# rasd3/TODA

Hardware: NVIDIA B200
Metric: frames/s voxelize+VoxelResBackBone8x fwd+bwd (higher is better)
Workload: dtype bf16

## Files before the change

include/toda_b200.h:

```cpp
#ifndef TODA_B200_H
#define TODA_B200_H

#include <stddef.h>
#include <stdint.h>

#ifdef __cplusplus
extern "C" {
#endif

#define TODA_OK 0
#define TODA_ERR_INVALID (-1)
#define TODA_ERR_CUDA (-2)
#define TODA_ERR_WORKSPACE (-3)
#define TODA_ERR_UNSUPPORTED (-4)

#define TODA_ORDER_FIRST_APPEARANCE 0
#define TODA_ORDER_CANONICAL 1

const char *toda_last_error(void);
int toda_version(void);
long long toda_launch_count(void);
int toda_device_info(int *sm_count_host, int *cc_major_host, int *cc_minor_host);

size_t toda_index_bytes(int batch, int D, int H, int W);
int toda_index_insert(void *index, int batch, int D, int H, int W, const int32_t *coords, int n, void *stream);
int toda_index_insert_strided(void *index_out, int batch, int oD, int oH, int oW, const int32_t *in_coords, int n_in,
                              const int *ksize_host, const int *stride_host, const int *pad_host, void *stream);
int toda_index_build(void *index, int batch, int D, int H, int W, int32_t *out_coords, int cap, int32_t *n_out,
                     void *stream);
int toda_index_rows(const void *index, int batch, int D, int H, int W, const int32_t *coords, int n, int32_t *rows,
                    void *stream);
int toda_index_release(void *index, int batch, int D, int H, int W, const int32_t *coords, int n, void *stream);

#define TODA_SELECT_RANGE_XY 0
#define TODA_SELECT_RECT_XY 1
#define TODA_SELECT_SECTOR 2
#define TODA_SELECT_BOXES 3
size_t toda_points_select_workspace_bytes(int n);
int toda_points_select(const float *points, int n, int stride, int x_col, const int32_t *frame_offsets, int batch, int mode,
                       const double *params_host, int invert, int add_batch_col, float *out, int32_t *out_offsets,
                       void *workspace, size_t workspace_bytes, void *stream);

size_t toda_voxelize_workspace_bytes(int64_t n_points, int batch, const int *grid_host, int max_points,
                                     int max_voxels);
int toda_voxelize_hard(const float *points, int64_t n_points, int point_stride, int xyz_col, int feat_col,
                       int num_features, const int32_t *frame_offsets, int batch, const float *range_host,
                       const float *vsize_host, const int *grid_host, int max_points, int max_voxels, int order,
                       float *voxels, int32_t *coords, int32_t *num_points, int32_t *voxel_counts, void *workspace,
                       size_t workspace_bytes, void *stream);

int toda_mean_vfe_fwd(const float *voxels, const void *num_points, int num_is_float, int n_voxels, int max_points,
                      int num_features, float *voxel_features, void *stream);
int toda_mean_vfe_bwd(const float *d_voxel_features, const void *num_points, int num_is_float, int n_voxels,
                      int max_points, int num_features, float *d_voxels, void *stream);

int toda_rulebook_subm(const void *index, int batch, int D, int H, int W, const int32_t *coords, int n,
                       const int *ksize_host, int32_t *nbr, void *stream);
int toda_rulebook_sparse(const void *index_in, int iD, int iH, int iW, const void *index_out, int oD, int oH, int oW,
                         int batch, const int32_t *in_coords, int n_in, const int32_t *out_coords, int n_out,
                         const int *ksize_host, const int *stride_host, const int *pad_host, int32_t *nbr_fwd,
                         int32_t *nbr_bwd, void *stream);

size_t toda_parity_order_workspace_bytes(int n);
int toda_parity_order(const int32_t *coords, int n, const int *stride_host, const int *pad_host, int32_t *order,
                      int32_t *pos_of_row, void *workspace, size_t workspace_bytes, void *stream);

#define TODA_CONV_FP32 0
#define TODA_CONV_BF16 1
#define TODA_CONV_BF16X3 2
int toda_weight_repack(const float *w_param, int kvol, int cin, int cout, int transpose, int mirror_k, float *w_out,
                       void *stream);
size_t toda_spconv_fwd_workspace_bytes(int n_in, int cin, int cout, int kvol, int precision);
int toda_table_tile_masks(const int32_t *nbr, int n_out, int kvol, uint32_t *masks, void *stream);
int toda_spconv_uses_tensor_cores(int cin, int cout, int kvol, int precision);
int toda_spconv_wgrad_uses_tensor_cores(int cin, int cout, int kvol, int precision);
int toda_spconv_fwd(const float *x, const void *x_bf16, int n_in, int cin, const int32_t *nbr, int n_out, int kvol,
                    const float *w, int cout, const float *bias, float *y, const int32_t *out_rows,
                    const uint32_t *tile_masks, double *bn_sums, int precision, void *workspace, size_t workspace_bytes,
                    void *stream);
int toda_tile_plan_capacity(int channels);
int toda_table_tile_plan(const int32_t *nbr, int n_out, int kvol, int ngroups, int cap, uint16_t *lidx, int32_t *rows,
                         int32_t *cnt, void *stream);
int toda_spconv_fwd_plan(const float *x, const void *x_bf16, int n_in, int cin, const int32_t *nbr, int n_out, int kvol,
                         const float *w, int cout, const float *bias, const float *addend, float *y,
                         const int32_t *out_rows, const uint32_t *tile_masks, const uint16_t *plan_lidx,
                         const int32_t *plan_rows, const int32_t *plan_cnt, int plan_groups, int plan_cap, double *bn_sums,
                         const void *w_bf16, int precision, void *workspace, size_t workspace_bytes, void *stream);
int toda_weight_kmajor_bf16(const float *w, int kvol, int cin, int cout, void *w_bf16, void *stream);
size_t toda_spconv_wgrad_workspace_bytes(int n_in, int n_out, int kvol, int cin, int cout, int precision);
int toda_spconv_wgrad(const float *x, const void *x_bf16, int n_in, int cin, const int32_t *nbr, int n_out, int kvol,
                      const float *dy, const void *dy_bf16, int cout, float *dw_param, void *workspace,
                      size_t workspace_bytes, int precision, void *stream);

size_t toda_bn_workspace_bytes(int channels);
int toda_bn_stats(const float *y, int n, int channels, const float *gamma, const float *beta, float eps,
                  float momentum, float *running_mean, float *running_var, float *scale, float *shift,
                  float *save_mean, float *save_rstd, void *workspace, size_t workspace_bytes, void *stream);
int toda_bn_finalize_sums(const double *sums, int n, int channels, const float *gamma, const float *beta, float eps,
                          float momentum, float *running_mean, float *running_var, float *scale, float *shift,
                          float *save_mean, float *save_rstd, void *stream);
int toda_bn_eval_coeffs(const float *gamma, const float *beta, const float *running_mean, const float *running_var,
                        float eps, int channels, float *scale, float *shift, void *stream);
int toda_bn_apply(const float *y, int n, int channels, const float *scale, const float *shift, const float *residual,
                  int relu, float *a, void *a_bf16, void *stream);
int toda_bn_apply_sums(const float *y, int n, int channels, const double *sums, const float *gamma, const float *beta,
                       float eps, float momentum, float *running_mean, float *running_var, float *scale, float *shift,
                       float *save_mean, float *save_rstd, const float *residual, int relu, float *a, void *a_bf16,
                       void *stream);
int toda_bn_bwd(const float *da, const float *a, const float *y, int n, int channels, const float *gamma,
                const float *save_mean, const float *save_rstd, int relu, int training, float *dy, void *dy_bf16,
                float *dresidual, float *dgamma, float *dbeta, void *workspace, size_t workspace_bytes, void *stream);
int toda_col_sum(const float *dy, int n, int channels, float *out, void *workspace, size_t workspace_bytes,
                 void *stream);

typedef struct {
    const float *x; const void *x_bf16; int n_in, cin; const int32_t *nbr; int n_out, kvol;
    const float *w; const void *w_bf16 ; int cout; const float *bias ;
    const uint32_t *tile_masks ;
    const uint16_t *plan_lidx ; const int32_t *plan_rows; const int32_t *plan_cnt; int plan_groups, plan_cap;
    int precision; void *conv_ws; size_t conv_ws_bytes;
    const float *gamma; const float *beta; float eps, momentum; float *running_mean; float *running_var; int training;
    const float *residual ; int relu;
    float *y; double *sums; float *stats; float *a; void *a_bf16 ;
    void *bn_ws; size_t bn_ws_bytes;
} toda_layer_fwd_args;
typedef struct {
    const float *da; const float *a_mask; const float *y; int n_out, cout; const float *gamma; const float *mean; const float *rstd;
    int relu, training; float *dy; void *dy_bf16 ; float *dres ; float *dgamma; float *dbeta;
    void *bn_ws; size_t bn_ws_bytes;
    const float *x; const void *x_bf16 ; int n_in, cin, kvol;
    int need_dx; const int32_t *dgrad_nbr; const float *wt; const void *wt_bf16 ;
    const int32_t *dgrad_out_rows ; const uint32_t *dgrad_masks ;
    const uint16_t *dplan_lidx ; const int32_t *dplan_rows; const int32_t *dplan_cnt; int dplan_groups, dplan_cap;
    const float *addend ; float *dx;
    int need_dw; const int32_t *nbr_fwd; float *dw; void *wgrad_ws; size_t wgrad_ws_bytes;
    int need_db; float *db;
    int precision; void *conv_ws; size_t conv_ws_bytes;
} toda_layer_bwd_args;
int toda_layer_fwd(const toda_layer_fwd_args *args, void *stream);
int toda_layer_bwd(const toda_layer_bwd_args *args, void *stream);

int toda_bev_scatter_fwd(const float *features, const int32_t *coords, int n, int channels, int batch, int D, int H,
                         int W, float *out, void *stream);
int toda_bev_scatter_bwd(const float *d_out, const int32_t *coords, int n, int channels, int batch, int D, int H,
                         int W, float *d_features, void *stream);

int toda_gather_rows(const float *in, const int32_t *rows, int n, int channels, float *out, void *stream);

#ifdef __cplusplus
}
#endif
#endif
```

toda_b200/_C.py:

```python
import ctypes
import os

_HERE = os.path.dirname(os.path.abspath(__file__))
LIB_PATH = os.path.join(_HERE, "lib", "libtoda_b200.so")

c_int, c_i64, c_f32, c_vp, c_sz = ctypes.c_int, ctypes.c_int64, ctypes.c_float, ctypes.c_void_p, ctypes.c_size_t
_IP = ctypes.POINTER(ctypes.c_int)
_FP = ctypes.POINTER(ctypes.c_float)

SIGNATURES = {
    "toda_last_error": (ctypes.c_char_p, []),
    "toda_version": (c_int, []),
    "toda_launch_count": (ctypes.c_longlong, []),
    "toda_device_info": (c_int, [_IP, _IP, _IP]),
    "toda_index_bytes": (c_sz, [c_int] * 4),
    "toda_index_insert": (c_int, [c_vp, c_int, c_int, c_int, c_int, c_vp, c_int, c_vp]),
    "toda_index_insert_strided": (c_int, [c_vp, c_int, c_int, c_int, c_int, c_vp, c_int, _IP, _IP, _IP, c_vp]),
    "toda_index_build": (c_int, [c_vp, c_int, c_int, c_int, c_int, c_vp, c_int, c_vp, c_vp]),
    "toda_index_rows": (c_int, [c_vp, c_int, c_int, c_int, c_int, c_vp, c_int, c_vp, c_vp]),
    "toda_index_release": (c_int, [c_vp, c_int, c_int, c_int, c_int, c_vp, c_int, c_vp]),
    "toda_points_select_workspace_bytes": (c_sz, [c_int]),
    "toda_points_select": (c_int, [c_vp, c_int, c_int, c_int, c_vp, c_int, c_int, ctypes.POINTER(ctypes.c_double), c_int, c_int,
                                   c_vp, c_vp, c_vp, c_sz, c_vp]),
    "toda_voxelize_workspace_bytes": (c_sz, [c_i64, c_int, _IP, c_int, c_int]),
    "toda_voxelize_hard": (c_int, [c_vp, c_i64, c_int, c_int, c_int, c_int, c_vp, c_int, _FP, _FP, _IP, c_int, c_int,
                                   c_int, c_vp, c_vp, c_vp, c_vp, c_vp, c_sz, c_vp]),
    "toda_mean_vfe_fwd": (c_int, [c_vp, c_vp, c_int, c_int, c_int, c_int, c_vp, c_vp]),
    "toda_mean_vfe_bwd": (c_int, [c_vp, c_vp, c_int, c_int, c_int, c_int, c_vp, c_vp]),
    "toda_rulebook_subm": (c_int, [c_vp, c_int, c_int, c_int, c_int, c_vp, c_int, _IP, c_vp, c_vp]),
    "toda_rulebook_sparse": (c_int, [c_vp, c_int, c_int, c_int, c_vp, c_int, c_int, c_int, c_int, c_vp, c_int, c_vp,
                                     c_int, _IP, _IP, _IP, c_vp, c_vp, c_vp]),
    "toda_weight_repack": (c_int, [c_vp, c_int, c_int, c_int, c_int, c_int, c_vp, c_vp]),
    "toda_spconv_fwd_workspace_bytes": (c_sz, [c_int] * 5),
    "toda_spconv_uses_tensor_cores": (c_int, [c_int] * 4),
    "toda_spconv_wgrad_uses_tensor_cores": (c_int, [c_int] * 4),
    "toda_parity_order_workspace_bytes": (c_sz, [c_int]),
    "toda_parity_order": (c_int, [c_vp, c_int, _IP, _IP, c_vp, c_vp, c_vp, c_sz, c_vp]),
    "toda_table_tile_masks": (c_int, [c_vp, c_int, c_int, c_vp, c_vp]),
    "toda_spconv_fwd": (c_int, [c_vp, c_vp, c_int, c_int, c_vp, c_int, c_int, c_vp, c_int, c_vp, c_vp, c_vp, c_vp, c_vp, c_int, c_vp,
                                c_sz, c_vp]),
    "toda_tile_plan_capacity": (c_int, [c_int]),
    "toda_table_tile_plan": (c_int, [c_vp, c_int, c_int, c_int, c_int, c_vp, c_vp, c_vp, c_vp]),
    "toda_spconv_fwd_plan": (c_int, [c_vp, c_vp, c_int, c_int, c_vp, c_int, c_int, c_vp, c_int, c_vp, c_vp, c_vp, c_vp, c_vp, c_vp,
                                     c_vp, c_vp, c_int, c_int, c_vp, c_vp, c_int, c_vp, c_sz, c_vp]),
    "toda_weight_kmajor_bf16": (c_int, [c_vp, c_int, c_int, c_int, c_vp, c_vp]),
    "toda_layer_fwd": (c_int, [c_vp, c_vp]),
    "toda_layer_bwd": (c_int, [c_vp, c_vp]),
    "toda_spconv_wgrad_workspace_bytes": (c_sz, [c_int] * 6),
    "toda_spconv_wgrad": (c_int, [c_vp, c_vp, c_int, c_int, c_vp, c_int, c_int, c_vp, c_vp, c_int, c_vp, c_vp, c_sz, c_int, c_vp]),
    "toda_bn_workspace_bytes": (c_sz, [c_int]),
    "toda_bn_stats": (c_int, [c_vp, c_int, c_int, c_vp, c_vp, c_f32, c_f32, c_vp, c_vp, c_vp, c_vp, c_vp, c_vp, c_vp,
                              c_sz, c_vp]),
    "toda_bn_finalize_sums": (c_int, [c_vp, c_int, c_int, c_vp, c_vp, c_f32, c_f32, c_vp, c_vp, c_vp, c_vp, c_vp, c_vp, c_vp]),
    "toda_bn_eval_coeffs": (c_int, [c_vp, c_vp, c_vp, c_vp, c_f32, c_int, c_vp, c_vp, c_vp]),
    "toda_bn_apply": (c_int, [c_vp, c_int, c_int, c_vp, c_vp, c_vp, c_int, c_vp, c_vp, c_vp]),
    "toda_bn_apply_sums": (c_int, [c_vp, c_int, c_int, c_vp, c_vp, c_vp, c_f32, c_f32, c_vp, c_vp, c_vp, c_vp, c_vp, c_vp, c_vp,
                                   c_int, c_vp, c_vp, c_vp]),
    "toda_bn_bwd": (c_int, [c_vp, c_vp, c_vp, c_int, c_int, c_vp, c_vp, c_vp, c_int, c_int, c_vp, c_vp, c_vp, c_vp, c_vp,
                            c_vp, c_sz, c_vp]),
    "toda_col_sum": (c_int, [c_vp, c_int, c_int, c_vp, c_vp, c_sz, c_vp]),
    "toda_bev_scatter_fwd": (c_int, [c_vp, c_vp, c_int, c_int, c_int, c_int, c_int, c_int, c_vp, c_vp]),
    "toda_bev_scatter_bwd": (c_int, [c_vp, c_vp, c_int, c_int, c_int, c_int, c_int, c_int, c_vp, c_vp]),
    "toda_gather_rows": (c_int, [c_vp, c_vp, c_int, c_int, c_vp, c_vp]),
}



class LayerFwdArgs(ctypes.Structure):
    _fields_ = [("x", c_vp), ("x_bf16", c_vp), ("n_in", c_int), ("cin", c_int), ("nbr", c_vp), ("n_out", c_int), ("kvol", c_int),
                ("w", c_vp), ("w_bf16", c_vp), ("cout", c_int), ("bias", c_vp), ("tile_masks", c_vp),
                ("plan_lidx", c_vp), ("plan_rows", c_vp), ("plan_cnt", c_vp), ("plan_groups", c_int), ("plan_cap", c_int),
                ("precision", c_int), ("conv_ws", c_vp), ("conv_ws_bytes", c_sz),
                ("gamma", c_vp), ("beta", c_vp), ("eps", c_f32), ("momentum", c_f32), ("running_mean", c_vp), ("running_var", c_vp),
                ("training", c_int), ("residual", c_vp), ("relu", c_int),
                ("y", c_vp), ("sums", c_vp), ("stats", c_vp), ("a", c_vp), ("a_bf16", c_vp), ("bn_ws", c_vp), ("bn_ws_bytes", c_sz)]


class LayerBwdArgs(ctypes.Structure):
    _fields_ = [("da", c_vp), ("a_mask", c_vp), ("y", c_vp), ("n_out", c_int), ("cout", c_int), ("gamma", c_vp), ("mean", c_vp),
                ("rstd", c_vp), ("relu", c_int), ("training", c_int), ("dy", c_vp), ("dy_bf16", c_vp), ("dres", c_vp), ("dgamma", c_vp),
                ("dbeta", c_vp), ("bn_ws", c_vp), ("bn_ws_bytes", c_sz),
                ("x", c_vp), ("x_bf16", c_vp), ("n_in", c_int), ("cin", c_int), ("kvol", c_int),
                ("need_dx", c_int), ("dgrad_nbr", c_vp), ("wt", c_vp), ("wt_bf16", c_vp), ("dgrad_out_rows", c_vp), ("dgrad_masks", c_vp),
                ("dplan_lidx", c_vp), ("dplan_rows", c_vp), ("dplan_cnt", c_vp), ("dplan_groups", c_int), ("dplan_cap", c_int),
                ("addend", c_vp), ("dx", c_vp),
                ("need_dw", c_int), ("nbr_fwd", c_vp), ("dw", c_vp), ("wgrad_ws", c_vp), ("wgrad_ws_bytes", c_sz),
                ("need_db", c_int), ("db", c_vp),
                ("precision", c_int), ("conv_ws", c_vp), ("conv_ws_bytes", c_sz)]


_lib = None


def lib():
    global _lib
    if _lib is None:
        if not os.path.exists(LIB_PATH):
            raise RuntimeError(
                f"{LIB_PATH} is missing: build it with `python -c 'import __graft_entry__ as g; g.build()'` "
                "(nvcc, sm_100a).  toda_b200 has no CPU fallback.")
        L = ctypes.CDLL(LIB_PATH)
        for name, (res, args) in SIGNATURES.items():
            fn = getattr(L, name)
            fn.restype = res
            fn.argtypes = args
        _lib = L
    return _lib


def check(rc, what=""):
    if rc != 0:
        msg = lib().toda_last_error().decode("utf-8", "replace")
        raise RuntimeError(f"libtoda_b200 {what} failed (code {rc}): {msg}")


def ints(vals):
    return (ctypes.c_int * len(vals))(*[int(v) for v in vals])


def doubles(vals):
    return (ctypes.c_double * len(vals))(*[float(v) for v in vals])


def floats(vals):
    return (ctypes.c_float * len(vals))(*[float(v) for v in vals])
```

toda_b200/csrc/conv_simt.cu:

```cuda
#include "common.cuh"
#include "conv_ts.cuh"

int conv_tc_fwd(const float *x, const void *x_bf16, int n_in, int cin, const int32_t *nbr, int n_out, int kvol, const float *w,
                int cout, const float *bias, float *y, const int32_t *out_rows, const uint32_t *tile_masks, double *bn_sums,
                void *workspace, size_t workspace_bytes,
                cudaStream_t st, const TilePlan *plan, const float *addend, const void *w_bf16);
size_t conv_tc_fwd_workspace_bytes(int n_in, int cin, int cout, int kvol);
int conv_tc_wgrad(const float *x, const void *x_bf16, int n_in, int cin, const int32_t *nbr, int n_out, int kvol,
                  const float *dy, const void *dy_bf16, int cout, float *dw_param, void *workspace, size_t workspace_bytes,
                  cudaStream_t st);
bool conv_tc_supported(int cin, int cout, int kvol);
size_t conv_x3_fwd_workspace_bytes(int n_in, int cin, int cout, int kvol);
int conv_x3_fwd(const float *x, int n_in, int cin, const int32_t *nbr, int n_out, int kvol, const float *w, int cout, const float *bias,
                float *y, const int32_t *out_rows, const uint32_t *tile_masks, double *bn_sums, void *workspace, size_t workspace_bytes,
                cudaStream_t st, const TilePlan *plan, const float *addend);
size_t conv_x3_wgrad_workspace_bytes(int n_in, int n_out, int kvol, int cin, int cout);
int conv_x3_wgrad(const float *x, int n_in, int cin, const int32_t *nbr, int n_out, int kvol, const float *dy, int cout, float *dw_param,
                  void *workspace, size_t workspace_bytes, cudaStream_t st);
bool conv_tc_wgrad_supported(int cin, int cout, int kvol);
size_t conv_tc_wgrad_workspace_bytes(int n_in, int n_out, int kvol, int cin, int cout);

namespace {

constexpr int kThreads = 256;
constexpr int BK = 16;

template <int BM, int BN>
__global__ void __launch_bounds__(kThreads) conv_fwd_f32_kernel(const float *__restrict__ x, int cin,
                                                                const int *__restrict__ nbr, int n_out, int kvol,
                                                                const float *__restrict__ w, int cout,
                                                                const float *__restrict__ bias, float *__restrict__ y,
                                                                const int *__restrict__ out_rows ,
                                                                const float *__restrict__ addend ) {
    static_assert((BM / 4) * (BN / 4) == kThreads, "4x4 micro-tiles must cover the CTA tile");
    __shared__ __align__(16) float As[BK][BM + 4];
    __shared__ __align__(16) float Bs[BK][BN + 4];
    __shared__ int rows[BM];
    const int tid = threadIdx.x;
    const int tx = tid % (BN / 4), ty = tid / (BN / 4);
    const int row0 = blockIdx.x * BM, col0 = blockIdx.y * BN;
    const bool vec = (cin % 4) == 0;
    float acc[4][4];
#pragma unroll
    for (int i = 0; i < 4; ++i)
#pragma unroll
        for (int j = 0; j < 4; ++j) acc[i][j] = 0.f;

    for (int k = 0; k < kvol; ++k) {
        int any = 0;
        for (int m = tid; m < BM; m += kThreads) {
            int r = row0 + m;
            int src = (r < n_out) ? __ldg(nbr + (size_t)k * n_out + r) : -1;
            rows[m] = src;
            any |= (src >= 0);
        }
        any = __syncthreads_or(any);
        if (!any) continue;
        for (int c0 = 0; c0 < cin; c0 += BK) {
            if (vec) {
                for (int e = tid; e < BM * (BK / 4); e += kThreads) {
                    int m = e / (BK / 4), q = e % (BK / 4);
                    int src = rows[m];
                    float4 v = make_float4(0.f, 0.f, 0.f, 0.f);
                    if (src >= 0 && c0 + q * 4 < cin) v = __ldg((const float4 *)(x + (size_t)src * cin + c0 + q * 4));
                    As[q * 4 + 0][m] = v.x; As[q * 4 + 1][m] = v.y; As[q * 4 + 2][m] = v.z; As[q * 4 + 3][m] = v.w;
                }
            } else {
                for (int e = tid; e < BM * BK; e += kThreads) {
                    int m = e / BK, kk = e % BK;
                    int src = rows[m];
                    As[kk][m] = (src >= 0 && c0 + kk < cin) ? __ldg(x + (size_t)src * cin + c0 + kk) : 0.f;
                }
            }
            for (int e = tid; e < BK * BN; e += kThreads) {
                int kk = e / BN, nn = e % BN;
                Bs[kk][nn] = (c0 + kk < cin && col0 + nn < cout) ? __ldg(w + ((size_t)k * cin + c0 + kk) * cout + col0 + nn) : 0.f;
            }
            __syncthreads();
#pragma unroll
            for (int kk = 0; kk < BK; ++kk) {
                float4 a = *(const float4 *)&As[kk][ty * 4];
                float4 b = *(const float4 *)&Bs[kk][tx * 4];
                float av[4] = {a.x, a.y, a.z, a.w}, bv[4] = {b.x, b.y, b.z, b.w};
#pragma unroll
                for (int i = 0; i < 4; ++i)
#pragma unroll
                    for (int j = 0; j < 4; ++j) acc[i][j] = fmaf(av[i], bv[j], acc[i][j]);
            }
            __syncthreads();
        }
    }
#pragma unroll
    for (int i = 0; i < 4; ++i) {
        int r = row0 + ty * 4 + i;
        if (r >= n_out) continue;
        const int orow = out_rows ? __ldg(out_rows + r) : r;
#pragma unroll
        for (int j = 0; j < 4; ++j) {
            int c = col0 + tx * 4 + j;
            if (c < cout) y[(size_t)orow * cout + c] = acc[i][j] + (bias ? __ldg(bias + c) : 0.f) + (addend ? __ldg(addend + (size_t)orow * cout + c) : 0.f);
        }
    }
}

constexpr int WT = 64;
__global__ void __launch_bounds__(kThreads) conv_wgrad_f32_kernel(const float *__restrict__ x, int cin,
                                                                  const int *__restrict__ nbr, int n_out, int kvol,
                                                                  const float *__restrict__ dy, int cout, int rows_per_split,
                                                                  float *__restrict__ partial) {
    __shared__ __align__(16) float As[BK][WT + 4];
    __shared__ __align__(16) float Bs[BK][WT + 4];
    __shared__ int pin[kThreads], pout[kThreads];
    __shared__ int warp_cnt[kThreads / 32];
    const int tid = threadIdx.x, lane = tid & 31, warp = tid >> 5;
    const int tx = tid % (WT / 4), ty = tid / (WT / 4);
    const int ci_tiles = (cin + WT - 1) / WT, co_tiles = (cout + WT - 1) / WT;
    int bx = blockIdx.x;
    const int co_t = bx % co_tiles; bx /= co_tiles;
    const int ci_t = bx % ci_tiles; bx /= ci_tiles;
    const int k = bx;
    const int split = blockIdx.y;
    const int ci0 = ci_t * WT, co0 = co_t * WT;
    const int r_begin = split * rows_per_split;
    const int r_end = min(n_out, r_begin + rows_per_split);
    float acc[4][4];
#pragma unroll
    for (int i = 0; i < 4; ++i)
#pragma unroll
        for (int j = 0; j < 4; ++j) acc[i][j] = 0.f;

    for (int r0 = r_begin; r0 < r_end; r0 += kThreads) {
        int r = r0 + tid;
        int src = (r < r_end) ? __ldg(nbr + (size_t)k * n_out + r) : -1;
        unsigned bal = __ballot_sync(0xffffffffu, src >= 0);
        if (lane == 0) warp_cnt[warp] = __popc(bal);
        __syncthreads();
        int woff = 0, total = 0;
#pragma unroll
        for (int wi = 0; wi < kThreads / 32; ++wi) {
            int c = warp_cnt[wi];
            if (wi < warp) woff += c;
            total += c;
        }
        if (src >= 0) {
            int pos = woff + __popc(bal & ((1u << lane) - 1u));
            pin[pos] = src;
            pout[pos] = r;
        }
        __syncthreads();
        for (int g0 = 0; g0 < total; g0 += BK) {
            for (int e = tid; e < BK * WT; e += kThreads) {
                int kk = e / WT, c = e % WT;
                bool ok = g0 + kk < total;
                As[kk][c] = (ok && ci0 + c < cin) ? __ldg(x + (size_t)pin[ok ? g0 + kk : 0] * cin + ci0 + c) : 0.f;
                Bs[kk][c] = (ok && co0 + c < cout) ? __ldg(dy + (size_t)pout[ok ? g0 + kk : 0] * cout + co0 + c) : 0.f;
            }
            __syncthreads();
#pragma unroll
            for (int kk = 0; kk < BK; ++kk) {
                float4 a = *(const float4 *)&As[kk][ty * 4];
                float4 b = *(const float4 *)&Bs[kk][tx * 4];
                float av[4] = {a.x, a.y, a.z, a.w}, bv[4] = {b.x, b.y, b.z, b.w};
#pragma unroll
                for (int i = 0; i < 4; ++i)
#pragma unroll
                    for (int j = 0; j < 4; ++j) acc[i][j] = fmaf(av[i], bv[j], acc[i][j]);
            }
            __syncthreads();
        }
    }
    float *dst = partial + ((size_t)split * kvol + k) * cin * cout;
#pragma unroll
    for (int i = 0; i < 4; ++i) {
        int ci = ci0 + ty * 4 + i;
        if (ci >= cin) continue;
#pragma unroll
        for (int j = 0; j < 4; ++j) {
            int co = co0 + tx * 4 + j;
            if (co < cout) dst[(size_t)ci * cout + co] = acc[i][j];
        }
    }
}

__global__ void wgrad_reduce_kernel(const float *__restrict__ partial, int splits, int kvol, int cin, int cout,
                                    float *__restrict__ dw_param) {
    size_t per = (size_t)kvol * cin * cout;
    const int sub = threadIdx.x & 7;
    for (size_t e = (blockIdx.x * (size_t)blockDim.x + threadIdx.x) >> 3; e < ((per + 31) & ~(size_t)31);
         e += ((size_t)gridDim.x * blockDim.x) >> 3) {
        float s = 0.f;
        if (e < per) {
            int ci = (int)(e % cin);
            size_t t = e / cin;
            int k = (int)(t % kvol);
            int co = (int)(t / kvol);
            size_t src = ((size_t)k * cin + ci) * cout + co;
            for (int sp = sub; sp < splits; sp += 8) s += partial[sp * per + src];
        }
        s += __shfl_xor_sync(0xffffffffu, s, 1);
        s += __shfl_xor_sync(0xffffffffu, s, 2);
        s += __shfl_xor_sync(0xffffffffu, s, 4);
        if (e < per && sub == 0) dw_param[e] = s;
    }
}

__global__ void weight_repack_kernel(const float *__restrict__ w_param, int kvol, int cin, int cout, int transpose,
                                     int mirror, float *__restrict__ w_out) {
    size_t per = (size_t)kvol * cin * cout;
    for (size_t e = blockIdx.x * (size_t)blockDim.x + threadIdx.x; e < per; e += (size_t)gridDim.x * blockDim.x) {
        int inner = (int)(e % (transpose ? cin : cout));
        size_t t = e / (transpose ? cin : cout);
        int mid = (int)(t % (transpose ? cout : cin));
        int k = (int)(t / (transpose ? cout : cin));
        int ci = transpose ? inner : mid, co = transpose ? mid : inner;
        int ks = mirror ? kvol - 1 - k : k;
        w_out[e] = __ldg(w_param + ((size_t)co * kvol + ks) * cin + ci);
    }
}

__global__ void gather_rows_kernel(const float *__restrict__ in, const int *__restrict__ rows, long long total, int c,
                                   float *__restrict__ out) {
    for (long long e = blockIdx.x * (long long)blockDim.x + threadIdx.x; e < total; e += (long long)gridDim.x * blockDim.x) {
        long long i = e / c;
        int r = __ldg(rows + i);
        out[e] = r >= 0 ? __ldg(in + (long long)r * c + (e - i * c)) : 0.f;
    }
}

int wgrad_splits(int n_out, int kvol, int cin, int cout) {
    int tiles = kvol * ((cin + WT - 1) / WT) * ((cout + WT - 1) / WT);
    int want = (4 * kNumSMs + tiles - 1) / tiles;
    int max_by_rows = (n_out + 4 * kThreads - 1) / (4 * kThreads);
    int s = want < max_by_rows ? want : max_by_rows;
    return s < 1 ? 1 : s;
}

}

extern "C" int toda_weight_repack(const float *w_param, int kvol, int cin, int cout, int transpose, int mirror_k,
                                  float *w_out, void *stream) {
    TODA_CHECK_ARG(w_param && w_out && kvol > 0 && cin > 0 && cout > 0, "weight_repack: bad args");
    size_t per = (size_t)kvol * cin * cout;
    weight_repack_kernel<<<wave_grid(per, 256), 256, 0, (cudaStream_t)stream>>>(w_param, kvol, cin, cout, transpose,
                                                                              mirror_k, w_out);
    TODA_LAUNCH_OK();
    return TODA_OK;
}

extern "C" int toda_spconv_uses_tensor_cores(int cin, int cout, int kvol, int precision) {
    return (precision == TODA_CONV_BF16 || precision == TODA_CONV_BF16X3) && conv_tc_supported(cin, cout, kvol) ? 1 : 0;
}

extern "C" int toda_spconv_wgrad_uses_tensor_cores(int cin, int cout, int kvol, int precision) {
    return (precision == TODA_CONV_BF16 || precision == TODA_CONV_BF16X3) && conv_tc_wgrad_supported(cin, cout, kvol) ? 1 : 0;
}

extern "C" size_t toda_spconv_fwd_workspace_bytes(int n_in, int cin, int cout, int kvol, int precision) {
    if (precision == TODA_CONV_BF16 && n_in >= 0 && cin > 0 && cout > 0 && kvol > 0 && conv_tc_supported(cin, cout, kvol))
        return conv_tc_fwd_workspace_bytes(n_in, cin, cout, kvol);
    if (precision == TODA_CONV_BF16X3 && n_in >= 0 && cin > 0 && cout > 0 && kvol > 0 && conv_tc_supported(cin, cout, kvol))
        return conv_x3_fwd_workspace_bytes(n_in, cin, cout, kvol);
    return 0;
}

static int spconv_fwd_impl(const float *x, const void *x_bf16, int n_in, int cin, const int32_t *nbr, int n_out, int kvol,
                           const float *w, int cout, const float *bias, float *y, const int32_t *out_rows,
                           const uint32_t *tile_masks, double *bn_sums, int precision, void *workspace, size_t workspace_bytes,
                           void *stream, const TilePlan *plan, const float *addend, const void *w_bf16);

extern "C" int toda_spconv_fwd(const float *x, const void *x_bf16, int n_in, int cin, const int32_t *nbr, int n_out, int kvol,
                               const float *w, int cout, const float *bias, float *y, const int32_t *out_rows,
                               const uint32_t *tile_masks, double *bn_sums, int precision,
                               void *workspace, size_t workspace_bytes, void *stream) {
    return spconv_fwd_impl(x, x_bf16, n_in, cin, nbr, n_out, kvol, w, cout, bias, y, out_rows, tile_masks, bn_sums, precision, workspace,
                           workspace_bytes, stream, nullptr, nullptr, nullptr);
}

extern "C" int toda_spconv_fwd_plan(const float *x, const void *x_bf16, int n_in, int cin, const int32_t *nbr, int n_out, int kvol,
                                    const float *w, int cout, const float *bias, const float *addend, float *y,
                                    const int32_t *out_rows, const uint32_t *tile_masks, const uint16_t *plan_lidx,
                                    const int32_t *plan_rows, const int32_t *plan_cnt, int plan_groups, int plan_cap, double *bn_sums,
                                    const void *w_bf16, int precision, void *workspace, size_t workspace_bytes, void *stream) {
    TilePlan plan{plan_lidx, plan_rows, plan_cnt, plan_groups, plan_cap};
    return spconv_fwd_impl(x, x_bf16, n_in, cin, nbr, n_out, kvol, w, cout, bias, y, out_rows, tile_masks, bn_sums, precision, workspace,
                           workspace_bytes, stream, plan_lidx ? &plan : nullptr, addend, w_bf16);
}

static int spconv_fwd_impl(const float *x, const void *x_bf16, int n_in, int cin, const int32_t *nbr, int n_out, int kvol,
                           const float *w, int cout, const float *bias, float *y, const int32_t *out_rows,
                           const uint32_t *tile_masks, double *bn_sums, int precision, void *workspace, size_t workspace_bytes,
                           void *stream, const TilePlan *plan, const float *addend, const void *w_bf16) {
    TODA_CHECK_ARG(n_in >= 0 && n_out >= 0 && cin > 0 && cout > 0 && kvol > 0, "spconv_fwd: bad sizes");
    if (n_out == 0) return TODA_OK;
    TODA_CHECK_ARG(x && nbr && w && y, "spconv_fwd: null pointer");
    cudaStream_t st = (cudaStream_t)stream;
    TODA_CHECK_ARG(precision == TODA_CONV_FP32 || precision == TODA_CONV_BF16 || precision == TODA_CONV_BF16X3,
                   "spconv_fwd: unknown precision %d", precision);
    if (precision == TODA_CONV_BF16X3 && conv_tc_supported(cin, cout, kvol))
        return conv_x3_fwd(x, n_in, cin, nbr, n_out, kvol, w, cout, bias, y, out_rows, tile_masks, bn_sums, workspace, workspace_bytes, st,
                           plan, addend);
    if (precision == TODA_CONV_BF16 && conv_tc_supported(cin, cout, kvol))
        return conv_tc_fwd(x, x_bf16, n_in, cin, nbr, n_out, kvol, w, cout, bias, y, out_rows, tile_masks, bn_sums, workspace,
                           workspace_bytes, st, plan, addend, w_bf16);
    TODA_CHECK_ARG(!bn_sums, "spconv_fwd: fused BatchNorm statistics need the tensor-core kernel for this shape");
    if (cout <= 16) {
        dim3 grid(ceil_div(n_out, 256), ceil_div(cout, 16));
        conv_fwd_f32_kernel<256, 16><<<grid, kThreads, 0, st>>>(x, cin, nbr, n_out, kvol, w, cout, bias, y, out_rows, addend);
    } else if (cout <= 32) {
        dim3 grid(ceil_div(n_out, 128), ceil_div(cout, 32));
        conv_fwd_f32_kernel<128, 32><<<grid, kThreads, 0, st>>>(x, cin, nbr, n_out, kvol, w, cout, bias, y, out_rows, addend);
    } else {
        dim3 grid(ceil_div(n_out, 64), ceil_div(cout, 64));
        conv_fwd_f32_kernel<64, 64><<<grid, kThreads, 0, st>>>(x, cin, nbr, n_out, kvol, w, cout, bias, y, out_rows, addend);
    }
    TODA_LAUNCH_OK();
    return TODA_OK;
}

extern "C" size_t toda_spconv_wgrad_workspace_bytes(int n_in, int n_out, int kvol, int cin, int cout, int precision) {
    if (n_in < 0 || n_out < 0 || kvol <= 0 || cin <= 0 || cout <= 0) return 0;
    if (precision == TODA_CONV_BF16 && conv_tc_wgrad_supported(cin, cout, kvol))
        return conv_tc_wgrad_workspace_bytes(n_in, n_out, kvol, cin, cout);
    if (precision == TODA_CONV_BF16X3 && conv_tc_wgrad_supported(cin, cout, kvol))
        return conv_x3_wgrad_workspace_bytes(n_in, n_out, kvol, cin, cout);
    int splits = wgrad_splits(n_out, kvol, cin, cout);
    return align_up((size_t)splits * kvol * cin * cout * sizeof(float), 256);
}

extern "C" int toda_spconv_wgrad(const float *x, const void *x_bf16, int n_in, int cin, const int32_t *nbr, int n_out,
                                 int kvol, const float *dy, const void *dy_bf16, int cout, float *dw_param, void *workspace,
                                 size_t workspace_bytes, int precision, void *stream) {
    TODA_CHECK_ARG(n_in >= 0 && n_out >= 0 && cin > 0 && cout > 0 && kvol > 0, "spconv_wgrad: bad sizes");
    TODA_CHECK_ARG(dw_param, "spconv_wgrad: null dw");
    cudaStream_t st = (cudaStream_t)stream;
    if (n_out == 0) {
        TODA_CUDA_OK(cudaMemsetAsync(dw_param, 0, (size_t)kvol * cin * cout * sizeof(float), st));
        return TODA_OK;
    }
    TODA_CHECK_ARG(x && nbr && dy && workspace, "spconv_wgrad: null pointer");
    TODA_CHECK_ARG(precision == TODA_CONV_FP32 || precision == TODA_CONV_BF16 || precision == TODA_CONV_BF16X3,
                   "spconv_wgrad: unknown precision %d", precision);
    if (precision == TODA_CONV_BF16X3 && conv_tc_wgrad_supported(cin, cout, kvol))
        return conv_x3_wgrad(x, n_in, cin, nbr, n_out, kvol, dy, cout, dw_param, workspace, workspace_bytes, st);
    if (precision == TODA_CONV_BF16 && conv_tc_wgrad_supported(cin, cout, kvol))
        return conv_tc_wgrad(x, x_bf16, n_in, cin, nbr, n_out, kvol, dy, dy_bf16, cout, dw_param, workspace, workspace_bytes, st);
    int splits = wgrad_splits(n_out, kvol, cin, cout);
    size_t need = (size_t)splits * kvol * cin * cout * sizeof(float);
    if (workspace_bytes < need) {
        toda_set_error("spconv_wgrad: workspace %zu < required %zu bytes", workspace_bytes, need);
        return TODA_ERR_WORKSPACE;
    }
    int rows_per_split = ceil_div(n_out, splits);
    rows_per_split = ceil_div(rows_per_split, kThreads) * kThreads;
    int tiles = kvol * ((cin + WT - 1) / WT) * ((cout + WT - 1) / WT);
    dim3 grid(tiles, splits);
    conv_wgrad_f32_kernel<<<grid, kThreads, 0, st>>>(x, cin, nbr, n_out, kvol, dy, cout, rows_per_split, (float *)workspace);
    TODA_LAUNCH_OK();
    size_t per = (size_t)kvol * cin * cout;
    wgrad_reduce_kernel<<<wave_grid(per * 8, 256), 256, 0, st>>>((const float *)workspace, splits, kvol, cin, cout, dw_param);
    TODA_LAUNCH_OK();
    return TODA_OK;
}

extern "C" int toda_gather_rows(const float *in, const int32_t *rows, int n, int channels, float *out, void *stream) {
    TODA_CHECK_ARG(n >= 0 && channels > 0, "gather_rows: bad sizes");
    if (n == 0) return TODA_OK;
    TODA_CHECK_ARG(in && rows && out, "gather_rows: null pointer");
    long long total = (long long)n * channels;
    gather_rows_kernel<<<wave_grid(total, 256), 256, 0, (cudaStream_t)stream>>>(in, rows, total, channels, out);
    TODA_LAUNCH_OK();
    return TODA_OK;
}
```

toda_b200/csrc/conv_tc.cu:

```cuda
#include <cuda.h>
#include <cuda_bf16.h>
#include <stdlib.h>

#include "common.cuh"
#include "conv_ts.cuh"
#include "epilogue.cuh"
#include "table_slice.cuh"

namespace {

constexpr int kTileM = 128;
constexpr int kChunkK = 64;
constexpr int kStages = 3;
constexpr int kProducers = 128;
constexpr int kThreadsTC = kProducers + 32;
constexpr int kABytes = kTileM * kChunkK * 2;
constexpr int kBBytesMax = 128 * kChunkK * 2;
constexpr int kStageBytes = kABytes + kBBytesMax;
constexpr int kMaxKvol = 27;
constexpr int kIdxBytes = kMaxKvol * kTileM * 4;

__device__ __forceinline__ uint32_t smem_u32(const void *p) { return (uint32_t)__cvta_generic_to_shared(p); }

__device__ __forceinline__ void mbar_init(uint32_t bar, uint32_t count) {
    asm volatile("mbarrier.init.shared::cta.b64 [%0], %1;" ::"r"(bar), "r"(count) : "memory");
}
__device__ __forceinline__ void mbar_wait(uint32_t bar, uint32_t parity) {
    uint32_t done = 0;
    uint32_t spins = 0;
    while (!done) {
        asm volatile(
            "{\n\t.reg .pred p;\n\t"
            "mbarrier.try_wait.parity.shared::cta.b64 p, [%1], %2;\n\t"
            "selp.u32 %0, 1, 0, p;\n\t}"
            : "=r"(done)
            : "r"(bar), "r"(parity)
            : "memory");
        if (!done && ++spins > (1u << 24)) __trap();
    }
}
__device__ __forceinline__ uint32_t mbar_test(uint32_t bar, uint32_t parity) {
    uint32_t done;
    asm volatile(
        "{\n\t.reg .pred p;\n\t"
        "mbarrier.test_wait.parity.shared::cta.b64 p, [%1], %2;\n\t"
        "selp.u32 %0, 1, 0, p;\n\t}"
        : "=r"(done)
        : "r"(bar), "r"(parity)
        : "memory");
    return done;
}
__device__ __forceinline__ bool elect_one() {
    uint32_t pred;
    asm volatile(
        "{\n\t.reg .pred p;\n\t"
        "elect.sync _|p, 0xffffffff;\n\t"
        "selp.u32 %0, 1, 0, p;\n\t}"
        : "=r"(pred));
    return pred != 0;
}
__device__ __forceinline__ void cp_async_16(uint32_t dst, const void *src, uint32_t src_bytes) {
    asm volatile("cp.async.cg.shared.global [%0], [%1], 16, %2;" ::"r"(dst), "l"(src), "r"(src_bytes) : "memory");
}
__device__ __forceinline__ void mbar_arrive_expect_tx(uint32_t bar, uint32_t bytes) {
    asm volatile("mbarrier.arrive.expect_tx.shared::cta.b64 _, [%0], %1;" ::"r"(bar), "r"(bytes) : "memory");
}
__device__ __forceinline__ void tma_load_2d(uint32_t dst, const CUtensorMap *map, int c0, int c1, uint32_t bar) {
    asm volatile(
        "cp.async.bulk.tensor.2d.shared::cluster.global.mbarrier::complete_tx::bytes [%0], [%1, {%2, %3}], [%4];"
        ::"r"(dst), "l"(map), "r"(c0), "r"(c1), "r"(bar)
        : "memory");
}
__device__ __forceinline__ void st_shared_zero16(uint32_t dst) {
    asm volatile("st.shared.v4.b32 [%0], {%1, %1, %1, %1};" ::"r"(dst), "r"(0u) : "memory");
}
__device__ __forceinline__ void cp_async_arrive_noinc(uint32_t bar) {
    asm volatile("cp.async.mbarrier.arrive.noinc.shared::cta.b64 [%0];" ::"r"(bar) : "memory");
}
__device__ __forceinline__ void umma_commit(uint32_t bar) {
    asm volatile("tcgen05.commit.cta_group::1.mbarrier::arrive::one.shared::cluster.b64 [%0];" ::"r"(bar) : "memory");
}
__device__ __forceinline__ void umma_bf16(uint32_t tmem_d, uint64_t adesc, uint64_t bdesc, uint32_t idesc, uint32_t accumulate) {
    asm volatile(
        "{\n\t.reg .pred p;\n\t"
        "setp.ne.b32 p, %4, 0;\n\t"
        "tcgen05.mma.cta_group::1.kind::f16 [%0], %1, %2, %3, p;\n\t}"
        ::"r"(tmem_d), "l"(adesc), "l"(bdesc), "r"(idesc), "r"(accumulate)
        : "memory");
}

__device__ __forceinline__ uint64_t make_desc_k_sw128(uint32_t smem_addr) {
    uint64_t d = 0;
    d |= (uint64_t)((smem_addr >> 4) & 0x3fff);
    d |= (uint64_t)1 << 16;
    d |= (uint64_t)(1024 >> 4) << 32;
    d |= (uint64_t)1 << 46;
    d |= (uint64_t)2 << 61;
    return d;
}

__host__ __device__ constexpr uint32_t make_idesc_bf16(int m, int n) {
    return (1u << 4) | (1u << 7) | (1u << 10) | ((uint32_t)(n >> 3) << 17) | ((uint32_t)(m >> 4) << 24);
}

__device__ __forceinline__ uint32_t sw128_offset(int r, int p) { return (uint32_t)(r * 128 + ((p ^ (r & 7)) << 4)); }

constexpr int kProdThreads = 256;
constexpr int kFwdThreads = kProdThreads + 32 + 128 + 32;
constexpr int kFwdSmemBudget = 200 * 1024;
template <int COUT, int KB> struct FwdCfg {
    static constexpr int kABlock = kTileM * kChunkK * 2;
    static constexpr int kBBlock = COUT * kChunkK * 2;
    static constexpr int kATile = KB * kABlock, kBTile = KB * kBBlock;
    static constexpr int kStage = kATile + kBTile;
    static constexpr int kStagesRaw = (kFwdSmemBudget - 2 * kIdxBytes) / kStage;
    static constexpr int kStages = kStagesRaw > 8 ? 8 : kStagesRaw;
    static constexpr int kSmem = kStages * kStage + 1024 + 256 + 2 * kIdxBytes;
    static constexpr int kTmemCols = 2 * COUT < 32 ? 32 : 2 * COUT;
    static_assert(kStages >= 3, "need at least 3 stages");
};

__device__ __forceinline__ void mbar_arrive(uint32_t bar) {
    asm volatile("mbarrier.arrive.shared::cta.b64 _, [%0];" ::"r"(bar) : "memory");
}
__device__ __forceinline__ void cp_async_4(uint32_t dst, const void *src) {
    asm volatile("cp.async.ca.shared.global [%0], [%1], 4;" ::"r"(dst), "l"(src) : "memory");
}

template <int CIN, int COUT, int KB>
__global__ void __launch_bounds__(kFwdThreads, 1) conv_tc_fwd_kernel(const __nv_bfloat16 *__restrict__ xb,
                                                                     const int *__restrict__ nbr, int n_out, int kvol,
                                                                     const __grid_constant__ CUtensorMap map_w ,
                                                                     const float *__restrict__ bias, const float *__restrict__ addend ,
                                                                     float *__restrict__ y,
                                                                     const int *__restrict__ out_rows ,
                                                                     const uint32_t *__restrict__ tile_masks ,
                                                                     double *__restrict__ bn_sums, int num_tiles,
                                                                     long long *__restrict__ dbg) {
    static_assert(COUT % 16 == 0 && COUT >= 16 && COUT <= 128, "UMMA N");
    static_assert(CIN == 16 || CIN == 32 || CIN == 64 || CIN == 128, "row = 32..256 bytes of bf16");
    using C = FwdCfg<COUT, KB>;
    constexpr int S = C::kStages;
    constexpr int kChunkElems = KB * kChunkK;
    extern __shared__ uint8_t smem_raw[];
    const uint32_t raw = smem_u32(smem_raw);
    const uint32_t base = (raw + 1023u) & ~1023u;
    const uint32_t bar_base = base + S * C::kStage;
    const uint32_t full_bar = bar_base, empty_bar = bar_base + 8 * S;
    const uint32_t acc_full = bar_base + 16 * S, acc_empty = acc_full + 16;
    const uint32_t idx_full = acc_full + 32, idx_empty = acc_full + 48;
    const uint32_t tmem_slot = acc_full + 64;
    const uint32_t idx_base = bar_base + 256;
    volatile uint32_t *tmem_slot_ptr = (volatile uint32_t *)(smem_raw + (tmem_slot - raw));

    const int tid = threadIdx.x, warp = tid >> 5, lane = tid & 31;
    const int ktot = kvol * CIN;
    const int nchunks = (ktot + kChunkElems - 1) / kChunkElems;
    auto chunk_mask_of = [&](int t) -> unsigned long long {
        if (!tile_masks) return nchunks >= 64 ? ~0ull : ((1ull << nchunks) - 1ull);
        const uint32_t om = __ldg(tile_masks + t);
        unsigned long long cm = 0ull;
        if (CIN <= kChunkElems) {
            constexpr int kOpc = CIN <= kChunkElems ? kChunkElems / CIN : 1;
            for (int c = 0; c < nchunks; ++c)
                if ((om >> (c * kOpc)) & ((1u << kOpc) - 1u)) cm |= 1ull << c;
        } else {
            constexpr int kCpo = CIN > kChunkElems ? CIN / kChunkElems : 1;
            for (int c = 0; c < nchunks; ++c)
                if ((om >> (c / kCpo)) & 1u) cm |= 1ull << c;
        }
        return cm ? cm : 1ull;
    };

    if (tid == 0) {
        for (int s = 0; s < S; ++s) {
            mbar_init(full_bar + 8 * s, kProdThreads / 32 + 1);
            mbar_init(empty_bar + 8 * s, 1);
        }
        for (int b = 0; b < 2; ++b) {
            mbar_init(acc_full + 8 * b, 1);
            mbar_init(acc_empty + 8 * b, 128);
            mbar_init(idx_full + 8 * b, 64);
            mbar_init(idx_empty + 8 * b, kProdThreads);
        }
        asm volatile("fence.mbarrier_init.release.cluster;" ::: "memory");
    }
    if (warp == 8) {
        asm volatile("tcgen05.alloc.cta_group::1.sync.aligned.shared::cta.b32 [%0], %1;" ::"r"(tmem_slot), "n"(C::kTmemCols) : "memory");
        asm volatile("tcgen05.relinquish_alloc_permit.cta_group::1.sync.aligned;" ::: "memory");
    }
    asm volatile("tcgen05.fence::before_thread_sync;" ::: "memory");
    __syncthreads();
    asm volatile("tcgen05.fence::after_thread_sync;" ::: "memory");
    const uint32_t tmem_base = *tmem_slot_ptr;

    if (warp < 8) {
        const int p = tid & 7;
        const int rbase = tid >> 3;
        const uint32_t piece_off = (uint32_t)(rbase * 128 + ((p ^ (rbase & 7)) << 4));
        constexpr int kOffsPerChunk = CIN >= 64 ? 1 : 64 / CIN;
        const int k_sub = CIN >= 64 ? 0 : p / (CIN / 8);
        const int ci_lo = CIN >= 64 ? p * 8 : (p % (CIN / 8)) * 8;
        const char *xbytes = (const char *)xb + ci_lo * 2;
        const uint32_t idx_lane = idx_base + 4 * rbase;
        constexpr int kLag = S - 2;
        int g = 0, it = 0;
        for (int t = blockIdx.x; t < num_tiles; t += gridDim.x, ++it) {
            const int ib = it & 1;
            if (dbg && blockIdx.x == 0 && tid == 0 && it < 256) dbg[0 * 256 + it] = clock64();
            mbar_wait(idx_full + 8 * ib, (it >> 1) & 1);
            if (dbg && blockIdx.x == 0 && tid == 0 && it < 256) dbg[1 * 256 + it] = clock64();
            if (dbg && blockIdx.x == 0 && tid == 0 && it < 255) dbg[7 * 256 + it] = g;
            const uint32_t idx_tile = idx_lane + ib * kIdxBytes;
            for (unsigned long long cm = chunk_mask_of(t); cm; cm &= cm - 1, ++g) {
                const int c = __ffsll((long long)cm) - 1;
                const int s = g % S, use = g / S;
                if (use > 0) mbar_wait(empty_bar + 8 * s, (use - 1) & 1);
                const uint32_t a_dst0 = base + s * C::kStage + piece_off;
#pragma unroll
                for (int kb = 0; kb < KB; ++kb) {
                    const int cb = c * KB + kb;
                    const uint32_t a_dst = a_dst0 + kb * C::kABlock;
                    const int k = CIN == 128 ? (cb >> 1) : cb * kOffsPerChunk + k_sub;
                    const bool k_ok = k < kvol;
                    const int ci_hi = CIN == 128 ? (cb & 1) * 64 : 0;
                    int src[4];
#pragma unroll
                    for (int i = 0; i < 4; ++i) {
                        src[i] = -1;
                        if (k_ok) asm volatile("ld.shared.b32 %0, [%1];" : "=r"(src[i]) : "r"(idx_tile + 4 * (k * kTileM + 32 * i)));
                    }
#pragma unroll
                    for (int i = 0; i < 4; ++i) {
                        if (src[i] >= 0) cp_async_16(a_dst + i * 4096, xbytes + ((size_t)(unsigned)src[i] * CIN + ci_hi) * 2, 16u);
                        else st_shared_zero16(a_dst + i * 4096);
                    }
                }
                if (tid == 0) {
                    const int left = ktot - c * kChunkElems;
                    const int nblk = left >= kChunkElems ? KB : (left + kChunkK - 1) / kChunkK;
                    mbar_arrive_expect_tx(full_bar + 8 * s, nblk * C::kBBlock);
                    const uint32_t b_tile = base + s * C::kStage + C::kATile;
                    for (int kb = 0; kb < nblk; ++kb)
                        tma_load_2d(b_tile + kb * C::kBBlock, &map_w, (c * KB + kb) * kChunkK, 0, full_bar + 8 * s);
                }
                asm volatile("cp.async.commit_group;" ::: "memory");
                if (g >= kLag) {
                    asm volatile("cp.async.wait_group %0;" ::"n"(kLag) : "memory");
                    asm volatile("fence.proxy.async.shared::cta;" ::: "memory");
                    __syncwarp();
                    if (lane == 0) mbar_arrive(full_bar + 8 * ((g - kLag) % S));
                }
                if (dbg && blockIdx.x == 0 && tid == 0 && g < 256) dbg[3 * 256 + g] = clock64();
            }
            mbar_arrive(idx_empty + 8 * ib);
        }
        asm volatile("cp.async.wait_group 0;" ::: "memory");
        asm volatile("fence.proxy.async.shared::cta;" ::: "memory");
        __syncwarp();
        if (lane == 0)
            for (int j = (g > kLag ? g - kLag : 0); j < g; ++j) mbar_arrive(full_bar + 8 * (j % S));
    } else if (warp == 8) {
        {
            constexpr uint32_t idesc = make_idesc_bf16(kTileM, COUT);
            int g = 0, it = 0;
            uint32_t ready = 0;
            for (int t = blockIdx.x; t < num_tiles; t += gridDim.x, ++it) {
                const int ab = it & 1, ause = it >> 1;
                if (ause > 0) mbar_wait(acc_empty + 8 * ab, (ause - 1) & 1);
                const uint32_t d_tmem = tmem_base + ab * COUT;
                uint32_t accumulate = 0;
                for (unsigned long long cm = chunk_mask_of(t); cm; cm &= cm - 1, ++g) {
                    const int c = __ffsll((long long)cm) - 1;
                    const int s = g % S, use = g / S;
                    if (dbg && blockIdx.x == 0 && lane == 0 && g < 256) dbg[4 * 256 + g] = clock64();
                    if (!ready) mbar_wait(full_bar + 8 * s, use & 1);
                    if (dbg && blockIdx.x == 0 && lane == 0 && g < 256) dbg[5 * 256 + g] = clock64();
                    const int sn = (g + 1) % S, usen = (g + 1) / S;
                    ready = mbar_test(full_bar + 8 * sn, usen & 1);
                    asm volatile("tcgen05.fence::after_thread_sync;" ::: "memory");
                    const uint32_t a_tile = base + s * C::kStage, b_tile = a_tile + C::kATile;
                    const int ksteps = min(kChunkElems, ktot - c * kChunkElems) / 16;
                    if (elect_one()) {
                        const uint64_t ad0 = make_desc_k_sw128(a_tile), bd0 = make_desc_k_sw128(b_tile);
                        umma_bf16(d_tmem, ad0, bd0, idesc, accumulate);
                        for (int j = 1; j < ksteps; ++j) {
                            const uint32_t blk = j >> 2, st = j & 3;
                            umma_bf16(d_tmem, ad0 + blk * (C::kABlock >> 4) + 2 * st, bd0 + blk * (C::kBBlock >> 4) + 2 * st, idesc, 1u);
                        }
                        umma_commit(empty_bar + 8 * s);
                    }
                    accumulate = 1u;
                    __syncwarp();
                    if (dbg && blockIdx.x == 0 && lane == 0 && g < 256) dbg[6 * 256 + g] = clock64();
                }
                if (elect_one()) umma_commit(acc_full + 8 * ab);
                __syncwarp();
            }
        }
    } else if (warp < 13) {
        const int q = warp & 3;
        float acc_s[COUT / 16], acc_q[COUT / 16];
#pragma unroll
        for (int i = 0; i < COUT / 16; ++i) acc_s[i] = acc_q[i] = 0.f;
        int it = 0;
        for (int t = blockIdx.x; t < num_tiles; t += gridDim.x, ++it) {
            const int ab = it & 1;
            mbar_wait(acc_full + 8 * ab, (it >> 1) & 1);
            asm volatile("tcgen05.fence::after_thread_sync;" ::: "memory");
            const int row = t * kTileM + q * 32 + lane;
            const int orow = (out_rows && row < n_out) ? __ldg(out_rows + row) : row;
            const uint32_t taddr = tmem_base + ((uint32_t)(q * 32) << 16) + ab * COUT;
#pragma unroll
            for (int n0 = 0; n0 < COUT; n0 += 16) {
                uint32_t v[16];
                asm volatile(
                    "tcgen05.ld.sync.aligned.32x32b.x16.b32 {%0,%1,%2,%3,%4,%5,%6,%7,%8,%9,%10,%11,%12,%13,%14,%15}, [%16];"
                    : "=r"(v[0]), "=r"(v[1]), "=r"(v[2]), "=r"(v[3]), "=r"(v[4]), "=r"(v[5]), "=r"(v[6]), "=r"(v[7]), "=r"(v[8]),
                      "=r"(v[9]), "=r"(v[10]), "=r"(v[11]), "=r"(v[12]), "=r"(v[13]), "=r"(v[14]), "=r"(v[15])
                    : "r"(taddr + n0));
                asm volatile("tcgen05.wait::ld.sync.aligned;" ::: "memory");
                float o[16];
#pragma unroll
                for (int j = 0; j < 16; ++j) o[j] = __uint_as_float(v[j]) + (bias ? __ldg(bias + n0 + j) : 0.f);
                if (row < n_out) {
                    if (addend) {
                        const float4 *ad = (const float4 *)(addend + (size_t)orow * COUT + n0);
#pragma unroll
                        for (int qq = 0; qq < 4; ++qq) {
                            const float4 a4 = __ldg(ad + qq);
                            o[4 * qq] += a4.x; o[4 * qq + 1] += a4.y; o[4 * qq + 2] += a4.z; o[4 * qq + 3] += a4.w;
                        }
                    }
                    float4 *dst = (float4 *)(y + (size_t)orow * COUT + n0);
#pragma unroll
                    for (int qq = 0; qq < 4; ++qq) dst[qq] = make_float4(o[4 * qq], o[4 * qq + 1], o[4 * qq + 2], o[4 * qq + 3]);
                }
                if (bn_sums) {
                    float sq[16];
#pragma unroll
                    for (int j = 0; j < 16; ++j) {
                        o[j] = row < n_out ? o[j] : 0.f;
                        sq[j] = o[j] * o[j];
                    }
                    acc_s[n0 / 16] += warp_colsum16(o, lane);
                    acc_q[n0 / 16] += warp_colsum16(sq, lane);
                }
            }
            asm volatile("tcgen05.fence::before_thread_sync;" ::: "memory");
            mbar_arrive(acc_empty + 8 * ab);
            if (dbg && blockIdx.x == 0 && q == 1 && lane == 0 && it < 256) dbg[2 * 256 + it] = clock64();
        }
        if (bn_sums && !(lane & 1)) {
            const int col = (lane >> 1) & 15;
#pragma unroll
            for (int i = 0; i < COUT / 16; ++i) {
                atomicAdd(bn_sums + i * 16 + col, (double)acc_s[i]);
                atomicAdd(bn_sums + COUT + i * 16 + col, (double)acc_q[i]);
            }
        }
    } else {
        int it = 0;
        for (int t = blockIdx.x; t < num_tiles; t += gridDim.x, ++it) {
            const int ib = it & 1, use = it >> 1;
            if (use > 0) mbar_wait(idx_empty + 8 * ib, (use - 1) & 1);
            const uint32_t dst0 = idx_base + ib * kIdxBytes;
            const int row0 = t * kTileM;
            load_table_slice<kTileM>(dst0, nbr, n_out, row0, n_out, kvol, lane);
            cp_async_arrive_noinc(idx_full + 8 * ib);
            mbar_arrive(idx_full + 8 * ib);
        }
    }
    __syncthreads();
    if (warp == 8) {
        asm volatile("tcgen05.fence::after_thread_sync;" ::: "memory");
        asm volatile("tcgen05.dealloc.cta_group::1.sync.aligned.b32 %0, %1;" ::"r"(tmem_base), "n"(C::kTmemCols) : "memory");
    }
}

__global__ void f32_to_bf16_kernel(const float *__restrict__ in, long long n4, __nv_bfloat16 *__restrict__ out) {
    for (long long i = blockIdx.x * (long long)blockDim.x + threadIdx.x; i < n4; i += (long long)gridDim.x * blockDim.x) {
        float4 v = __ldg((const float4 *)in + i);
        __nv_bfloat162 lo = __floats2bfloat162_rn(v.x, v.y), hi = __floats2bfloat162_rn(v.z, v.w);
        uint2 o;
        o.x = *(uint32_t *)&lo;
        o.y = *(uint32_t *)&hi;
        ((uint2 *)out)[i] = o;
    }
}

__global__ void f32_to_bf16_pad_kernel(const float *__restrict__ in, long long n, int cin, int cpad,
                                       __nv_bfloat16 *__restrict__ out) {
    long long total = n * cpad;
    for (long long e = blockIdx.x * (long long)blockDim.x + threadIdx.x; e < total; e += (long long)gridDim.x * blockDim.x) {
        long long r = e / cpad;
        int c = (int)(e - r * cpad);
        out[e] = __float2bfloat16_rn(c < cin ? __ldg(in + r * cin + c) : 0.f);
    }
}

__global__ void weight_to_kmajor_bf16_kernel(const float *__restrict__ w, int kvol, int cin, int cpad, int cout,
                                             __nv_bfloat16 *__restrict__ wb) {
    size_t per = (size_t)kvol * cpad * cout;
    for (size_t e = blockIdx.x * (size_t)blockDim.x + threadIdx.x; e < per; e += (size_t)gridDim.x * blockDim.x) {
        size_t kc = e % ((size_t)kvol * cpad);
        int co = (int)(e / ((size_t)kvol * cpad));
        int k = (int)(kc / cpad), ci = (int)(kc % cpad);
        wb[e] = __float2bfloat16_rn(ci < cin ? __ldg(w + ((size_t)k * cin + ci) * cout + co) : 0.f);
    }
}

__global__ void table_tile_masks_kernel(const int *__restrict__ nbr, int n_out, int kvol, int num_tiles, uint32_t *__restrict__ masks) {
    const int t = (blockIdx.x * blockDim.x + threadIdx.x) >> 5, lane = threadIdx.x & 31;
    if (t >= num_tiles) return;
    const int row0 = t * kTileM;
    uint32_t m = 0;
    for (int k = 0; k < kvol; ++k) {
        const int *src = nbr + (size_t)k * n_out + row0;
        int any = 0;
#pragma unroll
        for (int j = 0; j < kTileM / 32; ++j) {
            const int r = lane + 32 * j;
            if (row0 + r < n_out) any |= (__ldg(src + r) >= 0);
        }
        if (__any_sync(0xffffffffu, any)) m |= 1u << k;
    }
    if (lane == 0) masks[t] = m;
}

}

extern "C" int toda_table_tile_masks(const int32_t *nbr, int n_out, int kvol, uint32_t *masks, void *stream) {
    TODA_CHECK_ARG(n_out >= 0 && kvol > 0 && kvol <= 32, "table_tile_masks: bad sizes n_out=%d kvol=%d", n_out, kvol);
    if (n_out == 0) return TODA_OK;
    TODA_CHECK_ARG(nbr && masks, "table_tile_masks: null pointer");
    const int num_tiles = ceil_div(n_out, kTileM);
    table_tile_masks_kernel<<<ceil_div(num_tiles * 32, 256), 256, 0, (cudaStream_t)stream>>>(nbr, n_out, kvol, num_tiles, masks);
    TODA_LAUNCH_OK();
    return TODA_OK;
}

static inline int pad16(int c) { return c < 16 ? 16 : c; }

int conv_tma_fwd(const void *xb, int n_in, int cin, const int32_t *nbr, int n_out, int kvol, const void *wb, int cout,
                 const float *bias, const float *addend, float *y, const int32_t *out_rows, const uint32_t *tile_masks, double *bn_sums,
                 cudaStream_t st);

static long long *g_dbg_timeline = nullptr;
extern "C" void toda_debug_set_timeline(long long *buf) { g_dbg_timeline = buf; }
long long *conv_tc_debug_timeline() { return g_dbg_timeline; }
static int g_dbg_mode = 0;
extern "C" void toda_debug_set_mode(int m) { g_dbg_mode = m; }
int conv_tc_debug_mode() { return g_dbg_mode; }

extern "C" int toda_weight_kmajor_bf16(const float *w, int kvol, int cin, int cout, void *w_bf16, void *stream) {
    TODA_CHECK_ARG(w && w_bf16 && kvol > 0 && cin > 0 && cout > 0, "weight_kmajor_bf16: bad args");
    const int cp = cin < 16 ? 16 : cin;
    weight_to_kmajor_bf16_kernel<<<wave_grid((int64_t)kvol * cp * cout, 256), 256, 0, (cudaStream_t)stream>>>(w, kvol, cin, cp, cout,
                                                                                                            (__nv_bfloat16 *)w_bf16);
    TODA_LAUNCH_OK();
    return TODA_OK;
}

bool conv_tc_supported(int cin, int cout, int kvol) {
    bool cin_ok = (cin >= 1 && cin < 16) || cin == 16 || cin == 32 || cin == 64 || cin == 128;
    return cin_ok && kvol <= kMaxKvol && (cout == 16 || cout == 32 || cout == 64 || cout == 128);
}

size_t conv_tc_fwd_workspace_bytes(int n_in, int cin, int cout, int kvol) {
    int cp = pad16(cin);
    return align_up((size_t)n_in * cp * 2 + 16, 256) + align_up((size_t)kvol * cp * cout * 2, 256) + 256;
}

int conv_tc_fwd(const float *x, const void *x_bf16, int n_in, int cin, const int32_t *nbr, int n_out, int kvol, const float *w,
                int cout, const float *bias, float *y, const int32_t *out_rows, const uint32_t *tile_masks, double *bn_sums,
                void *workspace, size_t workspace_bytes,
                cudaStream_t st, const TilePlan *plan, const float *addend, const void *w_bf16) {
    size_t need = conv_tc_fwd_workspace_bytes(n_in, cin, cout, kvol);
    if (!workspace || workspace_bytes < need) {
        toda_set_error("spconv_fwd(bf16): workspace %zu < required %zu bytes", workspace_bytes, need);
        return TODA_ERR_WORKSPACE;
    }
    const int cp = pad16(cin);
    __nv_bfloat16 *xb = (__nv_bfloat16 *)workspace;
    __nv_bfloat16 *wb = (__nv_bfloat16 *)((char *)workspace + align_up((size_t)n_in * cp * 2 + 16, 256));
    if (cp == cin && x_bf16) {
        xb = (__nv_bfloat16 *)x_bf16;
    } else if (cp == cin) {
        long long n4 = (long long)n_in * cin / 4;
        if (n4 > 0) {
            f32_to_bf16_kernel<<<wave_grid(n4, 256), 256, 0, st>>>(x, n4, xb);
            TODA_LAUNCH_OK();
        }
    } else if (n_in > 0) {
        f32_to_bf16_pad_kernel<<<wave_grid((int64_t)n_in * cp, 256), 256, 0, st>>>(x, n_in, cin, cp, xb);
        TODA_LAUNCH_OK();
    }
    if (w_bf16) {
        wb = (__nv_bfloat16 *)w_bf16;
    } else {
        weight_to_kmajor_bf16_kernel<<<wave_grid((int64_t)kvol * cp * cout, 256), 256, 0, st>>>(w, kvol, cin, cp, cout, wb);
        TODA_LAUNCH_OK();
    }
    cin = cp;
    if (bn_sums) TODA_CUDA_OK(cudaMemsetAsync(bn_sums, 0, 2 * (size_t)cout * sizeof(double), st));
    static int feed = -1;
    if (feed < 0) { const char *e = getenv("TODA_TC_FEED"); feed = !e ? 2 : (e[0] == 'c' ? 0 : (e[0] == 't' && e[1] == 'm' ? 1 : 2)); }
    if (feed == 2 && conv_ts_supported(cin, cout, kvol, plan))
        return conv_ts_fwd(xb, n_in, cin, nbr, n_out, kvol, *plan, wb, cout, bias, addend, y, out_rows, tile_masks, bn_sums, st);
    if (feed == 1 || (feed == 2 && cin == 128 && cout == 128))
        {
        return conv_tma_fwd(xb, n_in, cin, nbr, n_out, kvol, wb, cout, bias, addend, y, out_rows, out_rows ? tile_masks : nullptr, bn_sums, st);
    }
    int num_tiles = ceil_div(n_out, kTileM);
    int grid = num_tiles < kNumSMs ? num_tiles : kNumSMs;
    CUtensorMap map_w;
    if (int rc = conv_tma_make_map(&map_w, wb, (uint64_t)cout, (uint64_t)kvol * cin, (uint32_t)cout, kChunkK)) return rc;
#define LAUNCH_TC(CI, CO)                                                                                                    \
    do {                                                                                                                     \
        constexpr int KB_ = (CO) <= 64 ? 2 : 1;                                                                              \
        constexpr int smem = FwdCfg<CO, KB_>::kSmem;                                                                         \
        static bool attr_set = false;                                                                                        \
        if (!attr_set) {                                                                                                     \
            TODA_CUDA_OK(cudaFuncSetAttribute(conv_tc_fwd_kernel<CI, CO, KB_>, cudaFuncAttributeMaxDynamicSharedMemorySize, smem)); \
            attr_set = true;                                                                                                 \
        }                                                                                                                    \
        conv_tc_fwd_kernel<CI, CO, KB_><<<grid, kFwdThreads, smem, st>>>(xb, nbr, n_out, kvol, map_w, bias, addend, y, out_rows, tile_masks, bn_sums, num_tiles, g_dbg_timeline); \
    } while (0)
#define LAUNCH_TC_CO(CI)                                                                                 \
    switch (cout) {                                                                                      \
        case 16: LAUNCH_TC(CI, 16); break;                                                               \
        case 32: LAUNCH_TC(CI, 32); break;                                                               \
        case 64: LAUNCH_TC(CI, 64); break;                                                               \
        case 128: LAUNCH_TC(CI, 128); break;                                                             \
        default: toda_set_error("conv_tc_fwd: unsupported cout %d", cout); return TODA_ERR_UNSUPPORTED;  \
    }
    switch (cin) {
        case 16: LAUNCH_TC_CO(16); break;
        case 32: LAUNCH_TC_CO(32); break;
        case 64: LAUNCH_TC_CO(64); break;
        case 128: LAUNCH_TC_CO(128); break;
        default: toda_set_error("conv_tc_fwd: unsupported cin %d", cin); return TODA_ERR_UNSUPPORTED;
    }
#undef LAUNCH_TC_CO
#undef LAUNCH_TC
    TODA_LAUNCH_OK();
    return TODA_OK;
}

namespace {

template <int NPAD, int ROWS> struct WCfg {
    static constexpr int kATile = 2 * ROWS * 128;
    static constexpr int kBTile = (NPAD / 64) * ROWS * 128;
    static constexpr int kIdx = 32 * ROWS * 4;
    static constexpr int kBBufs = ROWS == 128 ? 2 : 3;
    static constexpr int kStages = ROWS == 128 ? 4 : 8;
    static constexpr int kLag = ROWS == 128 ? 2 : 3;
    static constexpr int kSmem = kStages * kATile + kBBufs * kBTile + 2 * kIdx + 1024 + 256;
};
constexpr int kWgradThreads = kProdThreads + 32 + 128 + 32;

__device__ __forceinline__ uint64_t make_desc_mn_sw128(uint32_t smem_addr, uint32_t lbo_bytes) {
    uint64_t d = 0;
    d |= (uint64_t)((smem_addr >> 4) & 0x3fff);
    d |= (uint64_t)((lbo_bytes >> 4) & 0x3fff) << 16;
    d |= (uint64_t)(1024 >> 4) << 32;
    d |= (uint64_t)1 << 46;
    d |= (uint64_t)2 << 61;
    return d;
}

template <int CIN, int NPAD, int ROWS>
__global__ void __launch_bounds__(kWgradThreads, 1) conv_tc_wgrad_kernel(const __nv_bfloat16 *__restrict__ xb,
                                                                         const int *__restrict__ nbr, int n_out, int kvol,
                                                                         const __nv_bfloat16 *__restrict__ dyb, int cout,
                                                                         int rows_per_split, int passes_per_cta,
                                                                         float *__restrict__ partial) {
    using W = WCfg<NPAD, ROWS>;
    constexpr int kOffsPerPass = 128 / CIN;
    constexpr int S = W::kStages;
    constexpr int kRowsW = ROWS, kATileW = W::kATile, kBTileW = W::kBTile, kIdxW = W::kIdx, kBBufsW = W::kBBufs;
    constexpr int kRowIters = ROWS / 32;
    extern __shared__ uint8_t smem_raw[];
    const uint32_t raw = smem_u32(smem_raw);
    const uint32_t base = (raw + 1023u) & ~1023u;
    const uint32_t b_base = base + S * kATileW;
    const uint32_t idx_base = b_base + kBBufsW * kBTileW;
    const uint32_t bar_base = idx_base + 2 * kIdxW;
    const uint32_t a_full = bar_base, a_empty = bar_base + 8 * S;
    const uint32_t b_full = bar_base + 16 * S, b_empty = b_full + 32;
    const uint32_t idx_full = b_full + 64, idx_empty = b_full + 80;
    const uint32_t accum_bar = b_full + 96, tmem_slot = b_full + 104;
    volatile uint32_t *tmem_slot_ptr = (volatile uint32_t *)(smem_raw + (tmem_slot - raw));

    const int tid = threadIdx.x, warp = tid >> 5, lane = tid & 31;
    const int split = blockIdx.x, group = blockIdx.y;
    const int total_passes = (kvol + kOffsPerPass - 1) / kOffsPerPass;
    const int pass0 = group * passes_per_cta;
    const int npass = min(passes_per_cta, total_passes - pass0);
    const int k0 = pass0 * kOffsPerPass;
    const int noffs = min(npass * kOffsPerPass, kvol - k0);
    const int r_begin = split * rows_per_split;
    const int r_end = min(n_out, r_begin + rows_per_split);
    const int nchunks = r_end > r_begin ? (r_end - r_begin + kRowsW - 1) / kRowsW : 0;

    if (tid == 0) {
        for (int s = 0; s < S; ++s) {
            mbar_init(a_full + 8 * s, kProdThreads / 32);
            mbar_init(a_empty + 8 * s, 1);
        }
        for (int b = 0; b < kBBufsW; ++b) {
            mbar_init(b_full + 8 * b, kProdThreads / 32);
            mbar_init(b_empty + 8 * b, 1);
        }
        for (int b = 0; b < 2; ++b) {
            mbar_init(idx_full + 8 * b, 64);
            mbar_init(idx_empty + 8 * b, kProdThreads);
        }
        mbar_init(accum_bar, 1);
        asm volatile("fence.mbarrier_init.release.cluster;" ::: "memory");
    }
    uint32_t tmem_cols = 32;
    while ((int)tmem_cols < passes_per_cta * NPAD) tmem_cols <<= 1;
    if (warp == 8) {
        asm volatile("tcgen05.alloc.cta_group::1.sync.aligned.shared::cta.b32 [%0], %1;" ::"r"(tmem_slot), "r"(tmem_cols) : "memory");
        asm volatile("tcgen05.relinquish_alloc_permit.cta_group::1.sync.aligned;" ::: "memory");
    }
    asm volatile("tcgen05.fence::before_thread_sync;" ::: "memory");
    __syncthreads();
    asm volatile("tcgen05.fence::after_thread_sync;" ::: "memory");
    const uint32_t tmem_base = *tmem_slot_ptr;

    if (warp < 8) {
        const int p = tid & 7, rbase = tid >> 3;
        const uint32_t piece_off = (uint32_t)(rbase * 128 + ((p ^ (rbase & 7)) << 4));
        const int off_lo = CIN >= 64 ? 0 : p / (CIN / 8);
        const int ci_lo = CIN >= 64 ? p * 8 : (p % (CIN / 8)) * 8;
        constexpr int kLagW = W::kLag;
        int g = 0, signalled = 0;
        for (int rc = 0; rc < nchunks; ++rc) {
            const int ib = rc & 1, use_i = rc >> 1;
            const int bb = rc % kBBufsW, use_b = rc / kBBufsW;
            const int row_base = r_begin + rc * kRowsW;
            if (npass < kLagW) {
                asm volatile("cp.async.wait_group 0;" ::: "memory");
                asm volatile("fence.proxy.async.shared::cta;" ::: "memory");
                __syncwarp();
                if (lane == 0)
                    for (; signalled < g; ++signalled) {
                        if (signalled % npass == 0) mbar_arrive(b_full + 8 * ((signalled / npass) % kBBufsW));
                        mbar_arrive(a_full + 8 * (signalled % S));
                    }
                signalled = g;
            }
            if (use_b > 0) mbar_wait(b_empty + 8 * bb, (use_b - 1) & 1);
            {
                const uint32_t b_dst = b_base + bb * kBTileW + piece_off;
#pragma unroll
                for (int nb = 0; nb < NPAD / 64; ++nb) {
                    const int co = nb * 64 + p * 8;
#pragma unroll
                    for (int i = 0; i < kRowIters; ++i) {
                        const int row = row_base + rbase + 32 * i;
                        const uint32_t dst = b_dst + nb * (kRowsW * 128) + i * 4096;
                        if (row < r_end && co < cout) cp_async_16(dst, dyb + (size_t)row * cout + co, 16u);
                        else st_shared_zero16(dst);
                    }
                }
            }
            mbar_wait(idx_full + 8 * ib, use_i & 1);
            const uint32_t idx_tile = idx_base + ib * kIdxW + 4 * rbase;
            for (int ps = 0; ps < npass; ++ps, ++g) {
                const int s = g % S, use = g / S;
                if (use > 0) mbar_wait(a_empty + 8 * s, (use - 1) & 1);
                const uint32_t a_dst = base + s * kATileW + piece_off;
#pragma unroll
                for (int mb = 0; mb < 2; ++mb) {
                    const int koff = ps * kOffsPerPass + (CIN == 128 ? 0 : (CIN == 64 ? mb : mb * (kOffsPerPass / 2) + off_lo));
                    const int ci = CIN == 128 ? mb * 64 + ci_lo : ci_lo;
                    const bool k_ok = koff < noffs;
                    int src[kRowIters];
#pragma unroll
                    for (int i = 0; i < kRowIters; ++i) {
                        src[i] = -1;
                        if (k_ok) asm volatile("ld.shared.b32 %0, [%1];" : "=r"(src[i]) : "r"(idx_tile + 4 * (koff * kRowsW + 32 * i)));
                    }
#pragma unroll
                    for (int i = 0; i < kRowIters; ++i) {
                        const uint32_t dst = a_dst + mb * (kRowsW * 128) + i * 4096;
                        if (src[i] >= 0) cp_async_16(dst, xb + (size_t)(unsigned)src[i] * CIN + ci, 16u);
                        else st_shared_zero16(dst);
                    }
                }
                asm volatile("cp.async.commit_group;" ::: "memory");
                if (g - signalled >= kLagW) {
                    asm volatile("cp.async.wait_group %0;" ::"n"(kLagW) : "memory");
                    asm volatile("fence.proxy.async.shared::cta;" ::: "memory");
                    __syncwarp();
                    const int j = signalled;
                    if (lane == 0) {
                        if (j % npass == 0) mbar_arrive(b_full + 8 * ((j / npass) % kBBufsW));
                        mbar_arrive(a_full + 8 * (j % S));
                    }
                    ++signalled;
                }
            }
            mbar_arrive(idx_empty + 8 * ib);
        }
        asm volatile("cp.async.wait_group 0;" ::: "memory");
        asm volatile("fence.proxy.async.shared::cta;" ::: "memory");
        __syncwarp();
        if (lane == 0)
            for (int j = signalled; j < g; ++j) {
                if (j % npass == 0) mbar_arrive(b_full + 8 * ((j / npass) % kBBufsW));
                mbar_arrive(a_full + 8 * (j % S));
            }
    } else if (warp == 8) {
        if (nchunks > 0) {
            constexpr uint32_t idesc = make_idesc_bf16(128, NPAD) | (1u << 15) | (1u << 16);
            int g = 0;
            uint32_t ready = 0;
            for (int rc = 0; rc < nchunks; ++rc) {
                const int ib = rc % kBBufsW;
                mbar_wait(b_full + 8 * ib, (rc / kBBufsW) & 1);
                const uint32_t b_tile = b_base + ib * kBTileW;
                for (int ps = 0; ps < npass; ++ps, ++g) {
                    const int s = g % S, use = g / S;
                    if (!ready) mbar_wait(a_full + 8 * s, use & 1);
                    ready = mbar_test(a_full + 8 * ((g + 1) % S), ((g + 1) / S) & 1);
                    asm volatile("tcgen05.fence::after_thread_sync;" ::: "memory");
                    const uint32_t a_tile = base + s * kATileW;
                    if (elect_one()) {
#pragma unroll
                        const uint64_t ad0 = make_desc_mn_sw128(a_tile, kRowsW * 128), bd0 = make_desc_mn_sw128(b_tile, kRowsW * 128);
                        umma_bf16(tmem_base + ps * NPAD, ad0, bd0, idesc, rc != 0);
                        for (int j = 1; j < kRowsW / 16; ++j)
                            umma_bf16(tmem_base + ps * NPAD, ad0 + 128 * j, bd0 + 128 * j, idesc, 1u);
                        umma_commit(a_empty + 8 * s);
                    }
                    __syncwarp();
                }
                if (elect_one()) umma_commit(b_empty + 8 * ib);
                __syncwarp();
            }
            if (elect_one()) umma_commit(accum_bar);
            __syncwarp();
        }
    } else if (warp < 13) {
        const int q = warp & 3;
        if (nchunks > 0) {
            mbar_wait(accum_bar, 0);
            asm volatile("tcgen05.fence::after_thread_sync;" ::: "memory");
        }
        const int m = q * 32 + lane;
        for (int ps = 0; ps < npass; ++ps) {
            const int k = (pass0 + ps) * kOffsPerPass + m / CIN, ci = m % CIN;
            float *dst = partial + (((size_t)split * kvol + k) * CIN + ci) * cout;
            const uint32_t taddr = tmem_base + ((uint32_t)(q * 32) << 16) + ps * NPAD;
            for (int n0 = 0; n0 < cout; n0 += 16) {
                uint32_t v[16];
                if (nchunks > 0) {
                    asm volatile(
                        "tcgen05.ld.sync.aligned.32x32b.x16.b32 {%0,%1,%2,%3,%4,%5,%6,%7,%8,%9,%10,%11,%12,%13,%14,%15}, [%16];"
                        : "=r"(v[0]), "=r"(v[1]), "=r"(v[2]), "=r"(v[3]), "=r"(v[4]), "=r"(v[5]), "=r"(v[6]), "=r"(v[7]),
                          "=r"(v[8]), "=r"(v[9]), "=r"(v[10]), "=r"(v[11]), "=r"(v[12]), "=r"(v[13]), "=r"(v[14]), "=r"(v[15])
                        : "r"(taddr + n0));
                    asm volatile("tcgen05.wait::ld.sync.aligned;" ::: "memory");
                } else {
#pragma unroll
                    for (int qq = 0; qq < 16; ++qq) v[qq] = 0u;
                }
                if (k < kvol) {
#pragma unroll
                    for (int qq = 0; qq < 4; ++qq)
                        *(float4 *)(dst + n0 + 4 * qq) = make_float4(__uint_as_float(v[4 * qq]), __uint_as_float(v[4 * qq + 1]),
                                                                     __uint_as_float(v[4 * qq + 2]), __uint_as_float(v[4 * qq + 3]));
                }
            }
        }
        asm volatile("tcgen05.fence::before_thread_sync;" ::: "memory");
    } else {
        for (int rc = 0; rc < nchunks; ++rc) {
            const int ib = rc & 1, use = rc >> 1;
            if (use > 0) mbar_wait(idx_empty + 8 * ib, (use - 1) & 1);
            const uint32_t dst0 = idx_base + ib * kIdxW;
            const int row_base = r_begin + rc * kRowsW;
            load_table_slice<ROWS>(dst0, nbr + (size_t)k0 * n_out, n_out, row_base, r_end, noffs, lane);
            cp_async_arrive_noinc(idx_full + 8 * ib);
            mbar_arrive(idx_full + 8 * ib);
        }
    }
    __syncthreads();
    if (warp == 8) {
        asm volatile("tcgen05.fence::after_thread_sync;" ::: "memory");
        asm volatile("tcgen05.dealloc.cta_group::1.sync.aligned.b32 %0, %1;" ::"r"(tmem_base), "r"(tmem_cols) : "memory");
    }
}

__global__ void __launch_bounds__(256) wgrad_tc_reduce_kernel(const float *__restrict__ partial, int splits, int kvol, int cin,
                                                              int cpad, int cout, float *__restrict__ dw_param) {
    __shared__ float red[8][33];
    const size_t per_pad = (size_t)kvol * cpad * cout;
    const int x = threadIdx.x & 31, y = threadIdx.x >> 5;
    for (size_t e0 = (size_t)blockIdx.x * 32; e0 < per_pad; e0 += (size_t)gridDim.x * 32) {
        const size_t e = e0 + x;
        float s = 0.f;
        if (e < per_pad) {
#pragma unroll 4
            for (int sp = y; sp < splits; sp += 8) s += __ldg(partial + sp * per_pad + e);
        }
        red[y][x] = s;
        __syncthreads();
        if (y == 0 && e < per_pad) {
            s = ((red[0][x] + red[1][x]) + (red[2][x] + red[3][x])) + ((red[4][x] + red[5][x]) + (red[6][x] + red[7][x]));
            const int co = (int)(e % cout);
            const size_t t = e / cout;
            const int ci = (int)(t % cpad), k = (int)(t / cpad);
            if (ci < cin) dw_param[((size_t)co * kvol + k) * cin + ci] = s;
        }
        __syncthreads();
    }
}

struct WgradPlan {
    int passes_per_cta, groups, splits, rows_per_split;
    size_t xb_bytes, dyb_bytes, partial_bytes;
};

WgradPlan wgrad_plan(int n_in, int n_out, int kvol, int cin, int cout) {
    WgradPlan p;
    int npad = cout <= 64 ? 64 : 128;
    const int kRowsW = npad == 64 ? 128 : 64;
    int offs = 128 / cin;
    int total_passes = (kvol + offs - 1) / offs;
    p.passes_per_cta = total_passes < 512 / npad ? total_passes : 512 / npad;
    p.groups = (total_passes + p.passes_per_cta - 1) / p.passes_per_cta;
    int want = kNumSMs / p.groups;
    if (want < 1) want = 1;
    int max_by_rows = (n_out + 4 * kRowsW - 1) / (4 * kRowsW);
    p.splits = want < max_by_rows ? want : max_by_rows;
    if (p.splits < 1) p.splits = 1;
    int rps = (n_out + p.splits - 1) / p.splits;
    p.rows_per_split = (rps + kRowsW - 1) / kRowsW * kRowsW;
    if (p.rows_per_split < kRowsW) p.rows_per_split = kRowsW;
    p.xb_bytes = align_up((size_t)n_in * cin * 2 + 16, 256);
    p.dyb_bytes = align_up((size_t)n_out * cout * 2 + 16, 256);
    p.partial_bytes = align_up((size_t)p.splits * kvol * cin * cout * 4, 256);
    return p;
}

}

bool conv_tc_wgrad_supported(int cin, int cout, int kvol) {
    return kvol <= kMaxKvol && ((cin >= 1 && cin <= 16) || cin == 32 || cin == 64 || cin == 128) && (cout == 16 || cout == 32 || cout == 64 || cout == 128);
}

size_t conv_tc_wgrad_workspace_bytes(int n_in, int n_out, int kvol, int cin, int cout) {
    WgradPlan p = wgrad_plan(n_in, n_out, kvol, pad16(cin), cout);
    return p.xb_bytes + p.dyb_bytes + p.partial_bytes + 256;
}

int conv_tc_wgrad(const float *x, const void *x_bf16, int n_in, int cin, const int32_t *nbr, int n_out, int kvol,
                  const float *dy, const void *dy_bf16, int cout, float *dw_param, void *workspace, size_t workspace_bytes,
                  cudaStream_t st) {
    const int cin_real = cin;
    cin = pad16(cin);
    WgradPlan p = wgrad_plan(n_in, n_out, kvol, cin, cout);
    size_t need = p.xb_bytes + p.dyb_bytes + p.partial_bytes;
    if (!workspace || workspace_bytes < need) {
        toda_set_error("spconv_wgrad(bf16): workspace %zu < required %zu bytes", workspace_bytes, need);
        return TODA_ERR_WORKSPACE;
    }
    __nv_bfloat16 *xb = (__nv_bfloat16 *)workspace;
    __nv_bfloat16 *dyb = (__nv_bfloat16 *)((char *)workspace + p.xb_bytes);
    float *partial = (float *)((char *)workspace + p.xb_bytes + p.dyb_bytes);
    long long n4 = (long long)n_in * cin / 4;
    if (cin_real != cin) {
        if (n_in > 0) {
            f32_to_bf16_pad_kernel<<<wave_grid((int64_t)n_in * cin, 256), 256, 0, st>>>(x, n_in, cin_real, cin, xb);
            TODA_LAUNCH_OK();
        }
    } else if (x_bf16) {
        xb = (__nv_bfloat16 *)x_bf16;
    } else if (n4 > 0) {
        f32_to_bf16_kernel<<<wave_grid(n4, 256), 256, 0, st>>>(x, n4, xb);
        TODA_LAUNCH_OK();
    }
    if (dy_bf16) {
        dyb = (__nv_bfloat16 *)dy_bf16;
    } else {
        n4 = (long long)n_out * cout / 4;
        f32_to_bf16_kernel<<<wave_grid(n4, 256), 256, 0, st>>>(dy, n4, dyb);
        TODA_LAUNCH_OK();
    }
    dim3 grid(p.splits, p.groups);
#define LAUNCH_W(CI, NP, RW)                                                                                              \
    do {                                                                                                                   \
        constexpr int smem = WCfg<NP, RW>::kSmem;                                                                          \
        static bool attr_set = false;                                                                                      \
        if (!attr_set) {                                                                                                   \
            TODA_CUDA_OK(cudaFuncSetAttribute(conv_tc_wgrad_kernel<CI, NP, RW>, cudaFuncAttributeMaxDynamicSharedMemorySize, smem)); \
            attr_set = true;                                                                                               \
        }                                                                                                                  \
        conv_tc_wgrad_kernel<CI, NP, RW><<<grid, kWgradThreads, smem, st>>>(xb, nbr, n_out, kvol, dyb, cout, p.rows_per_split,  \
                                                                           p.passes_per_cta, partial);                      \
    } while (0)
    const bool wide = cout > 64;
    switch (cin) {
        case 16: if (wide) LAUNCH_W(16, 128, 64); else LAUNCH_W(16, 64, 128); break;
        case 32: if (wide) LAUNCH_W(32, 128, 64); else LAUNCH_W(32, 64, 128); break;
        case 64: if (wide) LAUNCH_W(64, 128, 64); else LAUNCH_W(64, 64, 128); break;
        case 128: if (wide) LAUNCH_W(128, 128, 64); else LAUNCH_W(128, 64, 128); break;
        default: toda_set_error("conv_tc_wgrad: unsupported cin %d", cin); return TODA_ERR_UNSUPPORTED;
    }
#undef LAUNCH_W
    TODA_LAUNCH_OK();
    size_t per_pad = (size_t)kvol * cin * cout;
    wgrad_tc_reduce_kernel<<<wave_grid(per_pad * 8, 256), 256, 0, st>>>(partial, p.splits, kvol, cin_real, cin, cout, dw_param);
    TODA_LAUNCH_OK();
    return TODA_OK;
}
```

toda_b200/csrc/conv_x3.cu:

```cuda
#include <cuda_bf16.h>

#include "common.cuh"
#include "conv_ts.cuh"

int conv_tc_fwd(const float *x, const void *x_bf16, int n_in, int cin, const int32_t *nbr, int n_out, int kvol, const float *w,
                int cout, const float *bias, float *y, const int32_t *out_rows, const uint32_t *tile_masks, double *bn_sums,
                void *workspace, size_t workspace_bytes,
                cudaStream_t st, const TilePlan *plan, const float *addend, const void *w_bf16);
size_t conv_tc_fwd_workspace_bytes(int n_in, int cin, int cout, int kvol);
int conv_tc_wgrad(const float *x, const void *x_bf16, int n_in, int cin, const int32_t *nbr, int n_out, int kvol,
                  const float *dy, const void *dy_bf16, int cout, float *dw_param, void *workspace, size_t workspace_bytes,
                  cudaStream_t st);
size_t conv_tc_wgrad_workspace_bytes(int n_in, int n_out, int kvol, int cin, int cout);

namespace {

static inline int pad16(int c) { return c < 16 ? 16 : c; }

__device__ __forceinline__ void split_bf16(float v, __nv_bfloat16 &hi, __nv_bfloat16 &lo) {
    hi = __float2bfloat16_rn(v);
    lo = __float2bfloat16_rn(v - __bfloat162float(hi));
}

__global__ void split_rows_kernel(const float *__restrict__ in, long long n, int cin, int cpad, __nv_bfloat16 *__restrict__ hi,
                                  __nv_bfloat16 *__restrict__ lo) {
    const long long total = n * cpad;
    for (long long e = blockIdx.x * (long long)blockDim.x + threadIdx.x; e < total; e += (long long)gridDim.x * blockDim.x) {
        const long long r = e / cpad;
        const int c = (int)(e - r * cpad);
        __nv_bfloat16 h, l;
        split_bf16(c < cin ? __ldg(in + r * cin + c) : 0.f, h, l);
        hi[e] = h;
        lo[e] = l;
    }
}

__global__ void split_weights_kernel(const float *__restrict__ w, int kvol, int cin, int cpad, int cout, __nv_bfloat16 *__restrict__ hi,
                                     __nv_bfloat16 *__restrict__ lo) {
    const size_t per = (size_t)kvol * cpad * cout;
    for (size_t e = blockIdx.x * (size_t)blockDim.x + threadIdx.x; e < per; e += (size_t)gridDim.x * blockDim.x) {
        const size_t kc = e % ((size_t)kvol * cpad);
        const int co = (int)(e / ((size_t)kvol * cpad));
        const int k = (int)(kc / cpad), ci = (int)(kc % cpad);
        __nv_bfloat16 h, l;
        split_bf16(ci < cin ? __ldg(w + ((size_t)k * cin + ci) * cout + co) : 0.f, h, l);
        hi[e] = h;
        lo[e] = l;
    }
}

__global__ void sum3_unpad_kernel(const float *__restrict__ t1, const float *__restrict__ t2, const float *__restrict__ t3, size_t rows,
                                  int cpad, int cin, float *__restrict__ dw) {
    const size_t total = rows * cin;
    for (size_t e = blockIdx.x * (size_t)blockDim.x + threadIdx.x; e < total; e += (size_t)gridDim.x * blockDim.x) {
        const size_t r = e / cin;
        const int c = (int)(e - r * cin);
        const size_t s = r * cpad + c;
        dw[e] = (t1[s] + t2[s]) + t3[s];
    }
}

struct X3Fwd { size_t x_bytes, w_bytes, inner; };
X3Fwd x3_fwd_layout(int n_in, int cin, int cout, int kvol) {
    const int cp = pad16(cin);
    X3Fwd l;
    l.x_bytes = align_up((size_t)(n_in > 0 ? n_in : 1) * cp * 2 + 16, 256);
    l.w_bytes = align_up((size_t)kvol * cp * cout * 2, 256);
    l.inner = conv_tc_fwd_workspace_bytes(n_in, cp, cout, kvol);
    return l;
}

struct X3Wgrad { size_t x_bytes, dy_bytes, t_bytes, inner; };
X3Wgrad x3_wgrad_layout(int n_in, int n_out, int kvol, int cin, int cout) {
    const int cp = pad16(cin);
    X3Wgrad l;
    l.x_bytes = align_up((size_t)(n_in > 0 ? n_in : 1) * cp * 2 + 16, 256);
    l.dy_bytes = align_up((size_t)(n_out > 0 ? n_out : 1) * cout * 2 + 16, 256);
    l.t_bytes = align_up((size_t)kvol * cp * cout * 4, 256);
    l.inner = conv_tc_wgrad_workspace_bytes(n_in, n_out, kvol, cp, cout);
    return l;
}

}

size_t conv_x3_fwd_workspace_bytes(int n_in, int cin, int cout, int kvol) {
    X3Fwd l = x3_fwd_layout(n_in, cin, cout, kvol);
    return 2 * l.x_bytes + 2 * l.w_bytes + l.inner + 256;
}

int conv_x3_fwd(const float *x, int n_in, int cin, const int32_t *nbr, int n_out, int kvol, const float *w, int cout, const float *bias,
                float *y, const int32_t *out_rows, const uint32_t *tile_masks, double *bn_sums, void *workspace, size_t workspace_bytes,
                cudaStream_t st, const TilePlan *plan, const float *addend) {
    const size_t need = conv_x3_fwd_workspace_bytes(n_in, cin, cout, kvol);
    if (!workspace || workspace_bytes < need) {
        toda_set_error("spconv_fwd(bf16x3): workspace %zu < required %zu bytes", workspace_bytes, need);
        return TODA_ERR_WORKSPACE;
    }
    const int cp = pad16(cin);
    X3Fwd l = x3_fwd_layout(n_in, cin, cout, kvol);
    char *p = (char *)workspace;
    __nv_bfloat16 *xh = (__nv_bfloat16 *)p, *xl = (__nv_bfloat16 *)(p + l.x_bytes);
    __nv_bfloat16 *wh = (__nv_bfloat16 *)(p + 2 * l.x_bytes), *wl = (__nv_bfloat16 *)(p + 2 * l.x_bytes + l.w_bytes);
    void *inner = p + 2 * l.x_bytes + 2 * l.w_bytes;
    if (n_in > 0) {
        split_rows_kernel<<<wave_grid((int64_t)n_in * cp, 256), 256, 0, st>>>(x, n_in, cin, cp, xh, xl);
        TODA_LAUNCH_OK();
    }
    split_weights_kernel<<<wave_grid((int64_t)kvol * cp * cout, 256), 256, 0, st>>>(w, kvol, cin, cp, cout, wh, wl);
    TODA_LAUNCH_OK();
    int rc = conv_tc_fwd(x, xh, n_in, cp, nbr, n_out, kvol, w, cout, bias, y, out_rows, tile_masks, nullptr, inner, l.inner, st, plan, addend, wh);
    if (rc) return rc;
    rc = conv_tc_fwd(x, xh, n_in, cp, nbr, n_out, kvol, w, cout, nullptr, y, out_rows, tile_masks, nullptr, inner, l.inner, st, plan, y, wl);
    if (rc) return rc;
    return conv_tc_fwd(x, xl, n_in, cp, nbr, n_out, kvol, w, cout, nullptr, y, out_rows, tile_masks, bn_sums, inner, l.inner, st, plan, y, wh);
}

size_t conv_x3_wgrad_workspace_bytes(int n_in, int n_out, int kvol, int cin, int cout) {
    X3Wgrad l = x3_wgrad_layout(n_in, n_out, kvol, cin, cout);
    return 2 * l.x_bytes + 2 * l.dy_bytes + 3 * l.t_bytes + l.inner + 256;
}

int conv_x3_wgrad(const float *x, int n_in, int cin, const int32_t *nbr, int n_out, int kvol, const float *dy, int cout, float *dw_param,
                  void *workspace, size_t workspace_bytes, cudaStream_t st) {
    const size_t need = conv_x3_wgrad_workspace_bytes(n_in, n_out, kvol, cin, cout);
    if (!workspace || workspace_bytes < need) {
        toda_set_error("spconv_wgrad(bf16x3): workspace %zu < required %zu bytes", workspace_bytes, need);
        return TODA_ERR_WORKSPACE;
    }
    const int cp = pad16(cin);
    X3Wgrad l = x3_wgrad_layout(n_in, n_out, kvol, cin, cout);
    char *p = (char *)workspace;
    __nv_bfloat16 *xh = (__nv_bfloat16 *)p, *xl = (__nv_bfloat16 *)(p + l.x_bytes);
    __nv_bfloat16 *dh = (__nv_bfloat16 *)(p + 2 * l.x_bytes), *dl = (__nv_bfloat16 *)(p + 2 * l.x_bytes + l.dy_bytes);
    float *t1 = (float *)(p + 2 * l.x_bytes + 2 * l.dy_bytes), *t2 = (float *)((char *)t1 + l.t_bytes), *t3 = (float *)((char *)t2 + l.t_bytes);
    void *inner = (char *)t3 + l.t_bytes;
    split_rows_kernel<<<wave_grid((int64_t)n_in * cp, 256), 256, 0, st>>>(x, n_in, cin, cp, xh, xl);
    TODA_LAUNCH_OK();
    split_rows_kernel<<<wave_grid((int64_t)n_out * cout, 256), 256, 0, st>>>(dy, n_out, cout, cout, dh, dl);
    TODA_LAUNCH_OK();
    int rc = conv_tc_wgrad(x, xh, n_in, cp, nbr, n_out, kvol, dy, dh, cout, t1, inner, l.inner, st);
    if (rc) return rc;
    rc = conv_tc_wgrad(x, xh, n_in, cp, nbr, n_out, kvol, dy, dl, cout, t2, inner, l.inner, st);
    if (rc) return rc;
    rc = conv_tc_wgrad(x, xl, n_in, cp, nbr, n_out, kvol, dy, dh, cout, t3, inner, l.inner, st);
    if (rc) return rc;
    const size_t rows = (size_t)cout * kvol;
    sum3_unpad_kernel<<<wave_grid((int64_t)rows * cin, 256), 256, 0, st>>>(t1, t2, t3, rows, cp, cin, dw_param);
    TODA_LAUNCH_OK();
    return TODA_OK;
}
```

toda_b200/csrc/layer.cu:

```cuda
#include "common.cuh"

extern "C" int toda_layer_fwd(const toda_layer_fwd_args *p, void *stream) {
    TODA_CHECK_ARG(p, "layer_fwd: null args");
    const int c = p->cout, n = p->n_out;
    TODA_CHECK_ARG(c > 0 && n >= 0 && p->stats && (n == 0 || (p->y && p->a)), "layer_fwd: bad sizes / null outputs");
    float *scale = p->stats, *shift = p->stats + c, *mean = p->stats + 2 * c, *rstd = p->stats + 3 * c;
    const bool tc = p->training && n > 0 && p->sums && toda_spconv_uses_tensor_cores(p->cin, c, p->kvol, p->precision);
    int rc = toda_spconv_fwd_plan(p->x, p->x_bf16, p->n_in, p->cin, p->nbr, n, p->kvol, p->w, c, p->bias, nullptr, p->y, nullptr,
                                  p->tile_masks, p->plan_lidx, p->plan_rows, p->plan_cnt, p->plan_groups, p->plan_cap,
                                  tc ? p->sums : nullptr, p->w_bf16, p->precision, p->conv_ws, p->conv_ws_bytes, stream);
    if (rc) return rc;
    if (n == 0) return TODA_OK;
    if (tc)
        return toda_bn_apply_sums(p->y, n, c, p->sums, p->gamma, p->beta, p->eps, p->momentum, p->running_mean, p->running_var, scale,
                                  shift, mean, rstd, p->residual, p->relu, p->a, p->a_bf16, stream);
    if (p->training)
        rc = toda_bn_stats(p->y, n, c, p->gamma, p->beta, p->eps, p->momentum, p->running_mean, p->running_var, scale, shift, mean, rstd,
                           p->bn_ws, p->bn_ws_bytes, stream);
    else
        rc = toda_bn_eval_coeffs(p->gamma, p->beta, p->running_mean, p->running_var, p->eps, c, scale, shift, stream);
    if (rc) return rc;
    return toda_bn_apply(p->y, n, c, scale, shift, p->residual, p->relu, p->a, p->a_bf16, stream);
}

extern "C" int toda_layer_bwd(const toda_layer_bwd_args *p, void *stream) {
    TODA_CHECK_ARG(p, "layer_bwd: null args");
    const int c = p->cout, n = p->n_out;
    TODA_CHECK_ARG(c > 0 && n >= 0, "layer_bwd: bad sizes");
    if (n == 0) {
        cudaStream_t st = (cudaStream_t)stream;
        if (p->dgamma) TODA_CUDA_OK(cudaMemsetAsync(p->dgamma, 0, sizeof(float) * c, st));
        if (p->dbeta) TODA_CUDA_OK(cudaMemsetAsync(p->dbeta, 0, sizeof(float) * c, st));
        if (p->need_db && p->db) TODA_CUDA_OK(cudaMemsetAsync(p->db, 0, sizeof(float) * c, st));
        if (p->need_dw && p->dw) TODA_CUDA_OK(cudaMemsetAsync(p->dw, 0, sizeof(float) * (size_t)p->kvol * p->cin * c, st));
        if (p->need_dx && p->dx && p->n_in > 0) {
            if (p->addend) TODA_CUDA_OK(cudaMemcpyAsync(p->dx, p->addend, sizeof(float) * (size_t)p->n_in * p->cin, cudaMemcpyDeviceToDevice, st));
            else TODA_CUDA_OK(cudaMemsetAsync(p->dx, 0, sizeof(float) * (size_t)p->n_in * p->cin, st));
        }
        return TODA_OK;
    }
    const bool dy_f32_read = p->need_db || !p->dy_bf16 || p->precision != TODA_CONV_BF16 ||
                             (p->need_dx && !toda_spconv_uses_tensor_cores(c, p->cin, p->kvol, p->precision)) ||
                             (p->need_dw && !toda_spconv_wgrad_uses_tensor_cores(p->cin, c, p->kvol, p->precision));
    int rc = toda_bn_bwd(p->da, p->a_mask, p->y, n, c, p->gamma, p->mean, p->rstd, p->relu, p->training, dy_f32_read ? p->dy : nullptr,
                         p->dy_bf16, p->dres, p->dgamma, p->dbeta, p->bn_ws, p->bn_ws_bytes, stream);
    if (rc) return rc;
    if (p->need_dx) {
        rc = toda_spconv_fwd_plan(p->dy, p->dy_bf16, n, c, p->dgrad_nbr, p->n_in, p->kvol, p->wt, p->cin, nullptr, p->addend, p->dx,
                                  p->dgrad_out_rows, p->dgrad_masks, p->dplan_lidx, p->dplan_rows, p->dplan_cnt, p->dplan_groups,
                                  p->dplan_cap, nullptr, p->wt_bf16, p->precision, p->conv_ws, p->conv_ws_bytes, stream);
        if (rc) return rc;
    }
    if (p->need_dw) {
        rc = toda_spconv_wgrad(p->x, p->x_bf16, p->n_in, p->cin, p->nbr_fwd, n, p->kvol, p->dy, p->dy_bf16, c, p->dw, p->wgrad_ws,
                               p->wgrad_ws_bytes, p->precision, stream);
        if (rc) return rc;
    }
    if (p->need_db) {
        rc = toda_col_sum(p->dy, n, c, p->db, p->bn_ws, p->bn_ws_bytes, stream);
        if (rc) return rc;
    }
    return TODA_OK;
}
```

toda_b200/csrc/table_slice.cuh:

```cuda
#pragma once
#include <cstdint>

template <int ROWS>
__device__ __forceinline__ void load_table_slice(uint32_t dst0, const int *__restrict__ nbr_k0, int n_out, int row_base, int r_end,
                                                 int noffs, int lane) {
    const int *src = nbr_k0 + row_base + lane;
    uint32_t dst = dst0 + 4u * lane;
    if (row_base + ROWS <= r_end) {
#pragma unroll 3
        for (int k = 0; k < noffs; ++k, src += n_out, dst += 4u * ROWS) {
#pragma unroll
            for (int j = 0; j < ROWS / 32; ++j)
                asm volatile("cp.async.ca.shared.global [%0], [%1], 4;" ::"r"(dst + 128u * j), "l"(src + 32 * j) : "memory");
        }
    } else {
        for (int k = 0; k < noffs; ++k, src += n_out, dst += 4u * ROWS) {
#pragma unroll
            for (int j = 0; j < ROWS / 32; ++j) {
                if (row_base + lane + 32 * j < r_end)
                    asm volatile("cp.async.ca.shared.global [%0], [%1], 4;" ::"r"(dst + 128u * j), "l"(src + 32 * j) : "memory");
                else
                    asm volatile("st.shared.b32 [%0], %1;" ::"r"(dst + 128u * j), "r"(-1) : "memory");
            }
        }
    }
}
```

toda_b200/ops.py:

```python
import ctypes
import weakref
from dataclasses import dataclass
from typing import List, Optional

import numpy as np
import torch

from . import _C

ORDER_FIRST_APPEARANCE = 0
ORDER_CANONICAL = 1
CONV_FP32 = 0
CONV_BF16 = 1
CONV_BF16X3 = 2
_TC_PRECISIONS = (CONV_BF16, CONV_BF16X3)

_launch_base = 0


def launches():
    return int(_C.lib().toda_launch_count()) - _launch_base


def reset_launches():
    global _launch_base
    _launch_base = int(_C.lib().toda_launch_count())


def _count(n):
    pass


_prof = None


def profile_begin():
    global _prof
    _prof = []


def profile_end():
    global _prof
    rec, _prof = _prof, None
    torch.cuda.synchronize()
    return [dict(name=n, ms=a.elapsed_time(b), **m) for (n, m, a, b) in rec]


class _Timed:
    def __init__(self, name, meta):
        self.name, self.meta = name, meta

    def __enter__(self):
        self.a = torch.cuda.Event(enable_timing=True)
        self.a.record()
        return self

    def __exit__(self, *exc):
        b = torch.cuda.Event(enable_timing=True)
        b.record()
        _prof.append((self.name, self.meta, self.a, b))
        return False


class _NoTimer:
    def __enter__(self):
        return self

    def __exit__(self, *exc):
        return False


_NO_TIMER = _NoTimer()


def _timed(name, **meta):
    return _Timed(name, meta) if _prof is not None else _NO_TIMER


_raw_stream = torch._C._cuda_getCurrentRawStream


def _stream_id(device=None):
    return _raw_stream(torch.cuda.current_device() if device is None or device.index is None else device.index)


def _stream():
    return ctypes.c_void_p(_raw_stream(torch.cuda.current_device()))


def _p(t: Optional[torch.Tensor]):
    return ctypes.c_void_p(t.data_ptr()) if t is not None else None


def _need(t, dtype, name):
    if not t.is_cuda:
        raise RuntimeError(f"{name} must be a CUDA tensor (toda_b200 has no CPU path)")
    if t.dtype != dtype:
        raise TypeError(f"{name} must be {dtype}, got {t.dtype}")
    if not t.is_contiguous():
        raise ValueError(f"{name} must be contiguous")
    return t


_workspaces = {}


def _workspace(tag, nbytes, device, zero=False):
    key = (tag, device.index, _stream_id(device))
    buf = _workspaces.get(key)
    if buf is None or buf.numel() < nbytes:
        buf = (torch.zeros if zero else torch.empty)(int(nbytes * 1.25) + 256, dtype=torch.uint8, device=device)
        _workspaces[key] = buf
    return buf


SELECT_RANGE_XY, SELECT_RECT_XY, SELECT_SECTOR, SELECT_BOXES = 0, 1, 2, 3
SELECT_MAX_BOXES = 96


def points_select(points, frame_offsets, mode, params, invert=False, add_batch_col=False, x_col=0, trim=True):
    points = _need(points, torch.float32, "points")
    assert points.dim() == 2
    n, stride = points.shape
    dev = points.device
    batch = 0
    if frame_offsets is not None:
        frame_offsets = _need(frame_offsets, torch.int32, "frame_offsets")
        batch = frame_offsets.numel() - 1
    L = _C.lib()
    ws = _workspace("select", L.toda_points_select_workspace_bytes(n), dev)
    out = torch.empty((n, stride + (1 if add_batch_col else 0)), dtype=torch.float32, device=dev)
    out_offsets = torch.empty((batch + 1,), dtype=torch.int32, device=dev)
    p = list(params) + [0.0] * (4 - len(params))
    with _timed("points_select", n=n, stride=stride, mode=int(mode)):
        _C.check(L.toda_points_select(_p(points), n, stride, int(x_col), _p(frame_offsets), batch, int(mode), _C.doubles(p),
                                      int(bool(invert)), int(bool(add_batch_col)), _p(out), _p(out_offsets), _p(ws),
                                      ws.numel(), _stream()), "toda_points_select")
    _count(2)
    if trim:
        return out[:int(out_offsets[-1].item())], out_offsets
    return out, out_offsets


def gather_point_rows(points, rows):
    points = _need(points, torch.float32, "points")
    rows = _need(rows, torch.int32, "rows")
    n, c = rows.shape[0], points.shape[1]
    out = torch.empty((n, c), dtype=torch.float32, device=points.device)
    _C.check(_C.lib().toda_gather_rows(_p(points), _p(rows), n, c, _p(out), _stream()), "toda_gather_rows")
    _count(1)
    return out


def grid_size_xyz(pc_range, voxel_size):
    r = np.asarray(pc_range, dtype=np.float64)
    return np.round((r[3:6] - r[0:3]) / np.asarray(voxel_size, dtype=np.float64)).astype(np.int64)


def voxelize(points, frame_offsets, pc_range, voxel_size, max_points, max_voxels, num_features=None, xyz_col=0,
             feat_col=0, order=ORDER_FIRST_APPEARANCE, grid=None, trim=True):
    points = _need(points, torch.float32, "points")
    assert points.dim() == 2
    n, stride = points.shape
    dev = points.device
    if not torch.is_tensor(frame_offsets):
        frame_offsets = torch.tensor(list(frame_offsets), dtype=torch.int32, device=dev)
    frame_offsets = _need(frame_offsets, torch.int32, "frame_offsets")
    batch = frame_offsets.numel() - 1
    f = int(num_features) if num_features is not None else stride - feat_col
    grid = grid_size_xyz(pc_range, voxel_size) if grid is None else np.asarray(grid)
    grid_c = _C.ints(grid)
    L = _C.lib()
    ws_bytes = L.toda_voxelize_workspace_bytes(n, batch, grid_c, max_points, max_voxels)
    if ws_bytes == 0:
        raise RuntimeError("toda_voxelize_workspace_bytes rejected the arguments")
    ws = _workspace("vox", ws_bytes, dev)
    cap = batch * max_voxels
    voxels = torch.empty((cap, max_points, f), dtype=torch.float32, device=dev)
    coords = torch.empty((cap, 4), dtype=torch.int32, device=dev)
    num = torch.empty((cap,), dtype=torch.int32, device=dev)
    counts = torch.empty((batch + 1,), dtype=torch.int32, device=dev)
    with _timed("voxelize", n_points=n, batch=batch, K=max_points, F=f):
        rc = L.toda_voxelize_hard(_p(points), n, stride, xyz_col, feat_col, f, _p(frame_offsets), batch,
                                  _C.floats(np.asarray(pc_range, dtype=np.float32)),
                                  _C.floats(np.asarray(voxel_size, dtype=np.float32)), grid_c, max_points, max_voxels,
                                  order, _p(voxels), _p(coords), _p(num), _p(counts), _p(ws), ws.numel(), _stream())
    _C.check(rc, "toda_voxelize_hard")
    _count(16 if order == ORDER_FIRST_APPEARANCE else 19)
    if trim:
        v = int(counts[batch].item())
        return voxels[:v], coords[:v], num[:v], counts
    return voxels, coords, num, counts


class _MeanVFE(torch.autograd.Function):
    @staticmethod
    def forward(ctx, voxels, num_points):
        voxels = _need(voxels, torch.float32, "voxels")
        v, k, f = voxels.shape
        is_float = num_points.dtype == torch.float32
        if not is_float:
            num_points = _need(num_points, torch.int32, "voxel_num_points")
        num_points = num_points.contiguous()
        out = torch.empty((v, f), dtype=torch.float32, device=voxels.device)
        with _timed("mean_vfe_fwd", V=v, K=k, F=f):
            _C.check(_C.lib().toda_mean_vfe_fwd(_p(voxels), _p(num_points), int(is_float), v, k, f, _p(out), _stream()),
                     "toda_mean_vfe_fwd")
        _count(1)
        ctx.save_for_backward(num_points)
        ctx.shape = (v, k, f, is_float)
        return out

    @staticmethod
    def backward(ctx, dout):
        (num_points,) = ctx.saved_tensors
        v, k, f, is_float = ctx.shape
        dout = dout.contiguous()
        dv = torch.empty((v, k, f), dtype=torch.float32, device=dout.device)
        _C.check(_C.lib().toda_mean_vfe_bwd(_p(dout), _p(num_points), int(is_float), v, k, f, _p(dv), _stream()),
                 "toda_mean_vfe_bwd")
        _count(1)
        return dv, None


def mean_vfe(voxels, num_points):
    return _MeanVFE.apply(voxels, num_points)


_index_occupant = {}


class OccupancyIndex:

    def __init__(self, batch, shape, device, tag):
        self.batch = int(batch)
        self.shape = [int(s) for s in shape]
        d, h, w = self.shape
        nbytes = _C.lib().toda_index_bytes(self.batch, d, h, w)
        if nbytes == 0:
            raise RuntimeError(f"bad index dims {batch} {shape}")
        self.key = (("index", tag, self.batch, d, h, w), device.index, _stream_id(device))
        self.buf = _workspace(self.key[0], nbytes, device, zero=True)
        self.coords = None
        self.frame_counts = None
        self.n = 0
        self._marked = False

    def _dims(self):
        return (self.batch, *self.shape)

    def _acquire(self):
        prev = _index_occupant.get(self.key)
        if prev is not None and prev is not self and prev.buf.data_ptr() == self.buf.data_ptr():
            prev._unmark()
        _index_occupant[self.key] = self

    def _unmark(self):
        if self.coords is not None and self.n > 0:
            _C.check(_C.lib().toda_index_release(_p(self.buf), *self._dims(), _p(self.coords), self.n, _stream()),
                     "toda_index_release")
            _count(1)
        if _index_occupant.get(self.key) is self:
            del _index_occupant[self.key]

    def insert(self, coords):
        self._acquire()
        coords = _need(coords, torch.int32, "coords")
        _C.check(_C.lib().toda_index_insert(_p(self.buf), *self._dims(), _p(coords), coords.shape[0], _stream()),
                 "toda_index_insert")
        _count(1)

    def insert_strided(self, in_coords, ksize, stride, padding):
        self._acquire()
        in_coords = _need(in_coords, torch.int32, "in_coords")
        _C.check(_C.lib().toda_index_insert_strided(_p(self.buf), *self._dims(), _p(in_coords), in_coords.shape[0],
                                                    _C.ints(ksize), _C.ints(stride), _C.ints(padding), _stream()),
                 "toda_index_insert_strided")
        _count(1)

    def build(self, cap, known_n=None):
        dev = self.buf.device
        coords = torch.empty((max(cap, 1), 4), dtype=torch.int32, device=dev)
        n_out = torch.empty((self.batch + 1,), dtype=torch.int32, device=dev)
        with _timed("index_build", cells=self.batch * self.shape[0] * self.shape[1] * self.shape[2]):
            _C.check(_C.lib().toda_index_build(_p(self.buf), *self._dims(), _p(coords), cap, _p(n_out), _stream()),
                     "toda_index_build")
        _count(5)
        self.n = int(n_out[0].item()) if known_n is None else int(known_n)
        self.coords = coords[:self.n]
        self.frame_counts = n_out
        return self.coords

    def ensure_live(self):
        if _index_occupant.get(self.key) is self:
            return
        if self.coords is None:
            raise RuntimeError("occupancy index was released")
        coords, n = self.coords, self.n
        self.insert(coords)
        self.build(n, known_n=n)

    def rows(self, coords):
        self.ensure_live()
        coords = _need(coords, torch.int32, "coords")
        rows = torch.empty((coords.shape[0],), dtype=torch.int32, device=coords.device)
        _C.check(_C.lib().toda_index_rows(_p(self.buf), *self._dims(), _p(coords), coords.shape[0], _p(rows), _stream()),
                 "toda_index_rows")
        _count(1)
        return rows

    def release(self):
        if _index_occupant.get(self.key) is self:
            self._unmark()
        self.coords = None
        self.n = 0


@dataclass
class Rulebook:
    subm: bool
    ksize: List[int]
    stride: List[int]
    padding: List[int]
    in_shape: List[int]
    out_shape: List[int]
    n_in: int
    n_out: int
    out_coords: torch.Tensor
    nbr_fwd: torch.Tensor
    nbr_bwd: Optional[torch.Tensor]
    dgrad_order: Optional[torch.Tensor] = None
    nbr_bwd_sorted: Optional[torch.Tensor] = None
    dgrad_tile_masks: Optional[torch.Tensor] = None
    tile_masks: Optional[torch.Tensor] = None
    plan: Optional["TilePlan"] = None
    dgrad_plan: Optional["TilePlan"] = None

    @property
    def kvol(self):
        return self.ksize[0] * self.ksize[1] * self.ksize[2]


@dataclass
class TilePlan:
    lidx: torch.Tensor
    rows: torch.Tensor
    cnt: torch.Tensor
    ngroups: int
    cap: int

    def tensors(self):
        return [self.lidx, self.rows, self.cnt]


def table_tile_plan(nbr, ksize, channels):
    kvol, n = nbr.shape
    ngroups = int(ksize[0])
    if n == 0 or kvol > 27 or ngroups > 3 or kvol % ngroups or kvol // ngroups > 9 or not channels:
        return None
    L = _C.lib()
    cap = L.toda_tile_plan_capacity(int(channels))
    if cap <= 0:
        return None
    tiles = (n + 127) // 128
    dev = nbr.device
    lidx = torch.empty((tiles, kvol, 128), dtype=torch.int16, device=dev)
    rows = torch.empty((tiles, ngroups, cap), dtype=torch.int32, device=dev)
    cnt = torch.empty((tiles, ngroups), dtype=torch.int32, device=dev)
    with _timed("tile_plan", n=n, kvol=kvol):
        _C.check(L.toda_table_tile_plan(_p(nbr), n, kvol, ngroups, cap, _p(lidx), _p(rows), _p(cnt), _stream()),
                 "toda_table_tile_plan")
    _count(1)
    return TilePlan(lidx, rows, cnt, ngroups, cap)


def conv_out_size(in_size, k, s, p):
    return (in_size + 2 * p - (k - 1) - 1) // s + 1


def rulebook_subm(index: OccupancyIndex, ksize, channels=None):
    index.ensure_live()
    n = index.n
    kvol = ksize[0] * ksize[1] * ksize[2]
    nbr = torch.empty((kvol, n), dtype=torch.int32, device=index.buf.device)
    with _timed("rulebook_subm", n=n, kvol=kvol):
        _C.check(_C.lib().toda_rulebook_subm(_p(index.buf), index.batch, *index.shape, _p(index.coords), n, _C.ints(ksize),
                                             _p(nbr), _stream()), "toda_rulebook_subm")
    _count(1)
    rb = Rulebook(True, list(ksize), [1, 1, 1], [k // 2 for k in ksize], index.shape, index.shape, n, n, index.coords,
                  nbr, None)
    rb.tile_masks = table_tile_masks(nbr) if (n > 0 and kvol <= 32) else None
    rb.plan = table_tile_plan(nbr, ksize, channels) if _TILE_PLANS else None
    return rb


def rulebook_sparse(index_in: OccupancyIndex, ksize, stride, padding, tag, cin=None, cout=None):
    index_in.ensure_live()
    out_shape = [conv_out_size(index_in.shape[a], ksize[a], stride[a], padding[a]) for a in range(3)]
    index_out = OccupancyIndex(index_in.batch, out_shape, index_in.buf.device, tag)
    if index_out.buf.data_ptr() == index_in.buf.data_ptr():
        index_out = OccupancyIndex(index_in.batch, out_shape, index_in.buf.device, (tag, "alt"))
    assert index_out.buf.data_ptr() != index_in.buf.data_ptr()
    index_out.insert_strided(index_in.coords, ksize, stride, padding)
    per_in = 1
    for a in range(3):
        per_in *= min(ksize[a], (ksize[a] + stride[a] - 1) // stride[a])
    cells = index_in.batch * out_shape[0] * out_shape[1] * out_shape[2]
    cap = int(min(index_in.n * per_in, cells))
    out_coords = index_out.build(cap)
    n_in, n_out = index_in.n, index_out.n
    kvol = ksize[0] * ksize[1] * ksize[2]
    dev = index_in.buf.device
    nbr_fwd = torch.empty((kvol, n_out), dtype=torch.int32, device=dev)
    nbr_bwd = torch.empty((kvol, n_in), dtype=torch.int32, device=dev)
    with _timed("rulebook_sparse", n_in=n_in, n_out=n_out, kvol=kvol):
        _C.check(_C.lib().toda_rulebook_sparse(_p(index_in.buf), *index_in.shape, _p(index_out.buf), *out_shape,
                                               index_in.batch, _p(index_in.coords), n_in, _p(out_coords), n_out,
                                               _C.ints(ksize), _C.ints(stride), _C.ints(padding), _p(nbr_fwd), _p(nbr_bwd),
                                               _stream()), "toda_rulebook_sparse")
    _count(2)
    rb = Rulebook(False, list(ksize), list(stride), list(padding), index_in.shape, out_shape, n_in, n_out, out_coords,
                  nbr_fwd, nbr_bwd)
    rb.tile_masks = table_tile_masks(nbr_fwd) if (n_out > 0 and kvol <= 32) else None
    rb.dgrad_order, rb.nbr_bwd_sorted = (_dgrad_parity_order(index_in.coords, nbr_bwd, stride, padding) if kvol <= 32
                                         else (None, None))
    if rb.dgrad_order is not None:
        rb.dgrad_tile_masks = table_tile_masks(rb.nbr_bwd_sorted)
    if _TILE_PLANS:
        rb.plan = table_tile_plan(nbr_fwd, ksize, cin)
        rb.dgrad_plan = table_tile_plan(rb.nbr_bwd_sorted if rb.dgrad_order is not None else nbr_bwd, ksize, cout)
    return rb, index_out


import os as _os
_TILE_PLANS = _os.environ.get("TODA_TILE_PLANS", "0") == "1"


def set_tile_plans(on):
    global _TILE_PLANS
    _TILE_PLANS = bool(on)


def tile_plans_enabled():
    return _TILE_PLANS


def table_tile_masks(nbr):
    kvol, n = nbr.shape
    masks = torch.empty(((n + 127) // 128,), dtype=torch.int32, device=nbr.device)
    _C.check(_C.lib().toda_table_tile_masks(_p(nbr), n, kvol, _p(masks), _stream()), "toda_table_tile_masks")
    _count(1)
    return masks


def _dgrad_parity_order(in_coords, nbr_bwd, stride, padding):
    if all(s == 1 for s in stride) or in_coords.shape[0] == 0:
        return None, None
    if stride[0] * stride[1] * stride[2] > 8:
        return None, None
    n = in_coords.shape[0]
    L = _C.lib()
    ws = _workspace("parity", L.toda_parity_order_workspace_bytes(n), in_coords.device)
    order = torch.empty((n,), dtype=torch.int32, device=in_coords.device)
    _C.check(L.toda_parity_order(_p(in_coords), n, _C.ints(stride), _C.ints(padding), _p(order), None, _p(ws), ws.numel(),
                                 _stream()), "toda_parity_order")
    _count(2)
    return order, nbr_bwd.index_select(1, order).contiguous()


_repack_cache = {}


def invalidate_weight_cache():
    _repack_cache.clear()


def _repack(weight, transpose, mirror, want_bf16=False):
    key = (id(weight), bool(transpose), bool(mirror))
    hit = _repack_cache.get(key)
    if hit is not None and hit[2]() is weight and hit[0] == weight._version and hit[3] == weight.data_ptr():
        out = hit[1]
    else:
        cout, kvol, cin = weight.shape[0], weight.shape[1] * weight.shape[2] * weight.shape[3], weight.shape[4]
        out = torch.empty((kvol, cout, cin) if transpose else (kvol, cin, cout), dtype=torch.float32, device=weight.device)
        _C.check(_C.lib().toda_weight_repack(_p(weight), kvol, cin, cout, int(transpose), int(mirror), _p(out), _stream()),
                 "toda_weight_repack")
        _count(1)
        if len(_repack_cache) > 512:
            _repack_cache.clear()
        hit = [weight._version, out, weakref.ref(weight), weight.data_ptr(), None]
        _repack_cache[key] = hit
    if not want_bf16:
        return out
    if hit[4] is None:
        kvol, ci, co = out.shape
        wb = torch.empty((co, kvol * max(ci, 16)), dtype=torch.bfloat16, device=out.device)
        _C.check(_C.lib().toda_weight_kmajor_bf16(_p(out), kvol, ci, co, _p(wb), _stream()), "toda_weight_kmajor_bf16")
        _count(1)
        hit[4] = wb
    return out, hit[4]


def _bf16_shadow_of(t):
    tag = getattr(t, "_toda_bf16", None)
    if tag is not None and tag[1] == t._version and tag[0].shape == t.shape:
        return tag[0]
    return None


def _conv_call(x, xb, cin, nbr, n_out, kvol, w, cout, bias, precision, what="conv_fwd", rb=None, bn_sums=None, y=None,
               out_rows=None, tile_masks=None, plan=None, addend=None, w_bf16=None):
    if y is None:
        y = torch.empty((n_out, cout), dtype=torch.float32, device=x.device)
    L = _C.lib()
    ws_bytes = L.toda_spconv_fwd_workspace_bytes(x.shape[0], cin, cout, kvol, precision)
    ws = _workspace("conv", ws_bytes, x.device) if ws_bytes else None
    if precision not in _TC_PRECISIONS:
        plan = None
    with _timed(what, n_in=x.shape[0], n_out=n_out, cin=cin, cout=cout, kvol=kvol, precision=precision, rb=id(rb)):
        if plan is None and addend is None and w_bf16 is None:
            _C.check(L.toda_spconv_fwd(_p(x), _p(xb), x.shape[0], cin, _p(nbr), n_out, kvol, _p(w), cout, _p(bias), _p(y),
                                       _p(out_rows), _p(tile_masks), _p(bn_sums), precision, _p(ws), ws.numel() if ws is not None else 0,
                                       _stream()), "toda_spconv_fwd")
        else:
            pl = plan
            _C.check(L.toda_spconv_fwd_plan(_p(x), _p(xb), x.shape[0], cin, _p(nbr), n_out, kvol, _p(w), cout, _p(bias),
                                            _p(addend), _p(y), _p(out_rows), _p(tile_masks), _p(pl.lidx) if pl else None,
                                            _p(pl.rows) if pl else None, _p(pl.cnt) if pl else None, pl.ngroups if pl else 0,
                                            pl.cap if pl else 0, _p(bn_sums), _p(w_bf16), precision, _p(ws),
                                            ws.numel() if ws is not None else 0, _stream()), "toda_spconv_fwd_plan")
    _count(1)
    return y


def conv_plan_usable(plan, cin, cout, kvol, precision):
    if plan is None or precision not in _TC_PRECISIONS or _os.environ.get("TODA_TC_FEED", "ts")[:1] in ("c",) or \
            _os.environ.get("TODA_TC_FEED", "ts")[:2] == "tm":
        return False
    cp = max(16, cin)
    return (cp in (16, 32, 64, 128) and cout in (16, 32, 64, 128) and kvol <= 27
            and plan.cap <= _C.lib().toda_tile_plan_capacity(cp))


def _conv_forward_impl(x, x_bf16, weight, bias, rb, precision, want_stats):
    x = _need(x.contiguous(), torch.float32, "features")
    weight = _need(weight.contiguous(), torch.float32, "weight")
    cout, cin = weight.shape[0], weight.shape[4]
    assert x.shape == (rb.n_in, cin), (x.shape, rb.n_in, cin)
    if x_bf16 is not None and (precision != CONV_BF16 or x_bf16.shape != x.shape or x_bf16.dtype != torch.bfloat16
                               or not x_bf16.is_contiguous()):
        x_bf16 = None
    w = _repack(weight, False, False)
    b = bias.contiguous() if bias is not None else None
    sums = None
    if want_stats and rb.n_out > 0 and _C.lib().toda_spconv_uses_tensor_cores(cin, cout, rb.kvol, precision):
        sums = torch.empty((2 * cout,), dtype=torch.float64, device=x.device)
    y = _conv_call(x, x_bf16, cin, rb.nbr_fwd, rb.n_out, rb.kvol, w, cout, b, precision, "conv_fwd", rb, sums,
                   tile_masks=rb.tile_masks, plan=rb.plan)
    return y, sums, x, weight, x_bf16


def _conv_backward_impl(dy, dyb, x, weight, xb, rb, precision, need_dx, need_dw, need_db):
    cout, cin = weight.shape[0], weight.shape[4]
    L = _C.lib()
    dx = dw = db = None
    if need_dx:
        wt = _repack(weight, True, rb.subm)
        if rb.subm:
            dx = _conv_call(dy, dyb, cout, rb.nbr_fwd, rb.n_in, rb.kvol, wt, cin, None, precision, "conv_dgrad", rb,
                            tile_masks=rb.tile_masks, plan=rb.plan)
        elif rb.dgrad_order is None:
            dx = _conv_call(dy, dyb, cout, rb.nbr_bwd, rb.n_in, rb.kvol, wt, cin, None, precision, "conv_dgrad", rb,
                            plan=rb.dgrad_plan)
        else:
            dx = _conv_call(dy, dyb, cout, rb.nbr_bwd_sorted, rb.n_in, rb.kvol, wt, cin, None, precision, "conv_dgrad",
                            rb, out_rows=rb.dgrad_order, tile_masks=rb.dgrad_tile_masks, plan=rb.dgrad_plan)
    if need_dw:
        dw = torch.empty_like(weight)
        ws_bytes = L.toda_spconv_wgrad_workspace_bytes(rb.n_in, rb.n_out, rb.kvol, cin, cout, precision)
        ws = _workspace("wgrad", ws_bytes, dy.device)
        with _timed("conv_wgrad", n_in=rb.n_in, n_out=rb.n_out, cin=cin, cout=cout, kvol=rb.kvol, precision=precision,
                    rb=id(rb)):
            _C.check(L.toda_spconv_wgrad(_p(x), _p(xb), rb.n_in, cin, _p(rb.nbr_fwd), rb.n_out, rb.kvol, _p(dy), _p(dyb),
                                         cout, _p(dw), _p(ws), ws.numel(), precision, _stream()), "toda_spconv_wgrad")
        _count(2)
    if need_db:
        db = col_sum(dy)
    return dx, dw, db


class _SparseConv(torch.autograd.Function):
    @staticmethod
    def forward(ctx, x, x_bf16, weight, bias, rb: Rulebook, precision, want_stats):
        y, sums, x, weight, x_bf16 = _conv_forward_impl(x, x_bf16, weight, bias, rb, precision, want_stats)
        ctx.save_for_backward(x, weight, x_bf16)
        ctx.set_materialize_grads(False)
        ctx.rb, ctx.precision, ctx.has_bias = rb, precision, bias is not None
        if sums is not None:
            ctx.mark_non_differentiable(sums)
        return y, sums

    @staticmethod
    def backward(ctx, dy, _dsums=None):
        if dy is None:
            return (None,) * 7
        x, weight, xb = ctx.saved_tensors
        dyb = _bf16_shadow_of(dy) if (ctx.precision == CONV_BF16 and dy.is_contiguous()) else None
        dx, dw, db = _conv_backward_impl(dy.contiguous(), dyb, x, weight, xb, ctx.rb, ctx.precision, ctx.needs_input_grad[0],
                                         ctx.needs_input_grad[2], ctx.has_bias and ctx.needs_input_grad[3])
        return dx, None, dw, db, None, None, None


def sparse_conv(x, weight, bias, rb, precision=CONV_FP32, x_bf16=None, want_stats=False):
    y, sums = _SparseConv.apply(x, x_bf16, weight, bias, rb, precision, want_stats)
    return (y, sums) if want_stats else y


def col_sum(t):
    n, c = t.shape
    out = torch.empty((c,), dtype=torch.float32, device=t.device)
    L = _C.lib()
    ws = _workspace("bn", L.toda_bn_workspace_bytes(c), t.device)
    _C.check(L.toda_col_sum(_p(t), n, c, _p(out), _p(ws), ws.numel(), _stream()), "toda_col_sum")
    _count(2)
    return out


class ReluMaskTape:

    def __init__(self, mode):
        assert mode in ("record", "replay")
        self.mode, self.masks, self.i = mode, [], 0

    def replay(self):
        self.mode, self.i = "replay", 0
        return self


_relu_tape = None


def set_relu_mask_tape(tape):
    global _relu_tape
    _relu_tape = tape


def _bn_forward_impl(y, gamma, beta, running_mean, running_var, eps, momentum, training, residual, relu, want_bf16, sums,
                     need_grad):
    y = _need(y.contiguous(), torch.float32, "bn input")
    n, c = y.shape
    dev = y.device
    L = _C.lib()
    scale = torch.empty((c,), dtype=torch.float32, device=dev)
    shift = torch.empty_like(scale)
    if training and sums is not None:
        mean = torch.empty_like(scale)
        rstd = torch.empty_like(scale)
        _C.check(L.toda_bn_finalize_sums(_p(sums), n, c, _p(gamma), _p(beta), float(eps), float(momentum),
                                         _p(running_mean), _p(running_var), _p(scale), _p(shift), _p(mean), _p(rstd),
                                         _stream()), "toda_bn_finalize_sums")
        _count(1)
    elif training:
        mean = torch.empty_like(scale)
        rstd = torch.empty_like(scale)
        ws = _workspace("bn", L.toda_bn_workspace_bytes(c), dev)
        with _timed("bn_stats", n=n, c=c):
            _C.check(L.toda_bn_stats(_p(y), n, c, _p(gamma), _p(beta), float(eps), float(momentum), _p(running_mean),
                                     _p(running_var), _p(scale), _p(shift), _p(mean), _p(rstd), _p(ws), ws.numel(),
                                     _stream()), "toda_bn_stats")
        _count(2)
    else:
        _C.check(L.toda_bn_eval_coeffs(_p(gamma), _p(beta), _p(running_mean), _p(running_var), float(eps), c, _p(scale),
                                       _p(shift), _stream()), "toda_bn_eval_coeffs")
        _count(1)
        mean = running_mean
        rstd = torch.rsqrt(running_var + eps) if need_grad else None
    res = residual.contiguous() if residual is not None else None
    a = torch.empty_like(y)
    ab = torch.empty(y.shape, dtype=torch.bfloat16, device=dev) if want_bf16 else None
    if _relu_tape is not None and relu:
        _C.check(L.toda_bn_apply(_p(y), n, c, _p(scale), _p(shift), _p(res), 0, _p(a), None, _stream()), "toda_bn_apply")
        _count(1)
        if _relu_tape.mode == "record":
            mask = a > 0
            _relu_tape.masks.append(mask)
        else:
            mask = _relu_tape.masks[_relu_tape.i]
            _relu_tape.i += 1
        a = a * mask
        if want_bf16:
            ab = a.to(torch.bfloat16)
        return a, ab, y, mean, rstd, mask.to(torch.float32)
    with _timed("bn_apply", n=n, c=c, residual=res is not None):
        _C.check(L.toda_bn_apply(_p(y), n, c, _p(scale), _p(shift), _p(res), int(relu), _p(a), _p(ab), _stream()),
                 "toda_bn_apply")
    _count(1)
    return a, ab, y, mean, rstd, a


def _bn_backward_impl(da, y, a, gamma, mean, rstd, training, relu, has_res, want_bf16):
    n, c = y.shape
    da = da.contiguous()
    L = _C.lib()
    dy = torch.empty_like(y)
    dyb = torch.empty(y.shape, dtype=torch.bfloat16, device=y.device) if want_bf16 else None
    dres = torch.empty_like(y) if has_res else None
    dgamma = torch.empty((c,), dtype=torch.float32, device=y.device)
    dbeta = torch.empty_like(dgamma)
    ws = _workspace("bn", L.toda_bn_workspace_bytes(c), y.device)
    with _timed("bn_bwd", n=n, c=c, residual=has_res):
        _C.check(L.toda_bn_bwd(_p(da), _p(a), _p(y), n, c, _p(gamma), _p(mean), _p(rstd), int(relu), int(training),
                               _p(dy), _p(dyb), _p(dres), _p(dgamma), _p(dbeta), _p(ws), ws.numel(), _stream()),
                 "toda_bn_bwd")
    _count(3)
    return dy, dyb, dres, dgamma, dbeta


class _BNAct(torch.autograd.Function):
    @staticmethod
    def forward(ctx, y, gamma, beta, running_mean, running_var, eps, momentum, training, residual, relu, want_bf16, sums):
        a, ab, y, mean, rstd, a_mask = _bn_forward_impl(y, gamma, beta, running_mean, running_var, eps, momentum, training,
                                                        residual, relu, want_bf16, sums, y.requires_grad or gamma.requires_grad)
        ctx.save_for_backward(y, a_mask, gamma, mean, rstd)
        ctx.set_materialize_grads(False)
        ctx.cfg = (bool(training), bool(relu), residual is not None, bool(want_bf16))
        if ab is not None:
            ctx.mark_non_differentiable(ab)
        return a, ab

    @staticmethod
    def backward(ctx, da, _dab=None):
        if da is None:
            return (None,) * 12
        y, a, gamma, mean, rstd = ctx.saved_tensors
        training, relu, has_res, want_bf16 = ctx.cfg
        dy, dyb, dres, dgamma, dbeta = _bn_backward_impl(da, y, a, gamma, mean, rstd, training, relu, has_res, want_bf16)
        if dyb is not None:
            dy._toda_bf16 = (dyb, dy._version)
        return dy, dgamma, dbeta, None, None, None, None, None, dres, None, None, None


def _vp(t):
    return t.data_ptr() if t is not None else None


def _fused_ok(training, need_grad):
    return _prof is None and _relu_tape is None and (training or not need_grad)


def _layer_forward(x, x_bf16, weight, bias, rb, precision, gamma, beta, running_mean, running_var, eps, momentum, training,
                   residual, relu, want_bf16, need_grad=True):
    if not _fused_ok(training, need_grad):
        y, sums, x, weight, x_bf16 = _conv_forward_impl(x, x_bf16, weight, bias, rb, precision, bool(training))
        a, ab, y, mean, rstd, a_mask = _bn_forward_impl(y, gamma, beta, running_mean, running_var, eps, momentum, training,
                                                        residual, relu, want_bf16, sums, need_grad)
        return a, ab, (x, x_bf16, weight, y, a_mask, gamma, mean, rstd)
    x = _need(x.contiguous(), torch.float32, "features")
    weight = _need(weight.contiguous(), torch.float32, "weight")
    cout, cin = weight.shape[0], weight.shape[4]
    assert x.shape == (rb.n_in, cin), (x.shape, rb.n_in, cin)
    if x_bf16 is not None and (precision != CONV_BF16 or x_bf16.shape != x.shape or x_bf16.dtype != torch.bfloat16
                               or not x_bf16.is_contiguous()):
        x_bf16 = None
    L = _C.lib()
    kvol, n_out, dev = rb.kvol, rb.n_out, x.device
    tc = bool(L.toda_spconv_uses_tensor_cores(cin, cout, kvol, precision))
    if tc and precision == CONV_BF16:
        w, wb = _repack(weight, False, False, True)
    else:
        w, wb = _repack(weight, False, False), None
    y = torch.empty((n_out, cout), dtype=torch.float32, device=dev)
    a = torch.empty_like(y)
    ab = torch.empty((n_out, cout), dtype=torch.bfloat16, device=dev) if want_bf16 else None
    small = torch.empty((8 * cout,), dtype=torch.float32, device=dev)
    ws_bytes = L.toda_spconv_fwd_workspace_bytes(x.shape[0], cin, cout, kvol, precision)
    ws = _workspace("conv", ws_bytes, dev) if ws_bytes else None
    bws = _workspace("bn", L.toda_bn_workspace_bytes(cout), dev)
    res = residual.contiguous() if residual is not None else None
    b = bias.contiguous() if bias is not None else None
    pl = rb.plan if precision in _TC_PRECISIONS else None
    sp = small.data_ptr()
    args = _C.LayerFwdArgs(
        x.data_ptr(), _vp(x_bf16), x.shape[0], cin, rb.nbr_fwd.data_ptr(), n_out, kvol, w.data_ptr(), _vp(wb), cout, _vp(b),
        _vp(rb.tile_masks), _vp(pl.lidx) if pl else None, _vp(pl.rows) if pl else None, _vp(pl.cnt) if pl else None,
        pl.ngroups if pl else 0, pl.cap if pl else 0, precision, _vp(ws), ws.numel() if ws is not None else 0,
        gamma.data_ptr(), beta.data_ptr(), float(eps), float(momentum), _vp(running_mean), _vp(running_var), int(bool(training)),
        _vp(res), int(bool(relu)), y.data_ptr(), sp + 16 * cout, sp, a.data_ptr(), _vp(ab), bws.data_ptr(), bws.numel())
    _C.check(L.toda_layer_fwd(ctypes.byref(args), _stream()), "toda_layer_fwd")
    _count(2 if (tc and training and n_out > 0) else (3 if tc else 4))
    mean = small[2 * cout:3 * cout] if training else running_mean
    rstd = small[3 * cout:4 * cout] if training else None
    return a, ab, (x, x_bf16, weight, y, a, gamma, mean, rstd)


def _layer_backward(da, saved, rb, precision, training, relu, has_res, has_bias, need_dx, need_dw, addend=None):
    x, xb, weight, y, a_mask, gamma, mean, rstd = saved
    if not _fused_ok(training, True):
        dy, dyb, dres, dgamma, dbeta = _bn_backward_impl(da, y, a_mask, gamma, mean, rstd, training, relu, has_res,
                                                         precision == CONV_BF16)
        dx, dw, db = _conv_backward_impl(dy, dyb, x, weight, xb, rb, precision, need_dx, need_dw, has_bias)
        if addend is not None and dx is not None:
            dx = dx + addend
        return dx, dw, db, dgamma, dbeta, dres
    L = _C.lib()
    da = da.contiguous()
    n_out, cout = y.shape
    cin, kvol, dev = weight.shape[4], rb.kvol, y.device
    bf16 = precision == CONV_BF16
    dy = torch.empty_like(y)
    dyb = torch.empty(y.shape, dtype=torch.bfloat16, device=dev) if bf16 else None
    dres = torch.empty_like(y) if has_res else None
    small = torch.empty((3 * cout,), dtype=torch.float32, device=dev)
    bws = _workspace("bn", L.toda_bn_workspace_bytes(cout), dev)
    dx = dw = None
    wt = wtb = None
    nbr = out_rows = masks = pl = None
    if need_dx:
        tc = bool(L.toda_spconv_uses_tensor_cores(cout, cin, kvol, precision))
        if tc and precision == CONV_BF16:
            wt, wtb = _repack(weight, True, rb.subm, True)
        else:
            wt = _repack(weight, True, rb.subm)
        if rb.subm:
            nbr, masks, pl = rb.nbr_fwd, rb.tile_masks, rb.plan
        elif rb.dgrad_order is None:
            nbr, pl = rb.nbr_bwd, rb.dgrad_plan
        else:
            nbr, out_rows, masks, pl = rb.nbr_bwd_sorted, rb.dgrad_order, rb.dgrad_tile_masks, rb.dgrad_plan
        if precision not in _TC_PRECISIONS:
            pl = None
        dx = torch.empty((rb.n_in, cin), dtype=torch.float32, device=dev)
        if addend is not None:
            addend = addend.contiguous()
    ws_bytes = L.toda_spconv_fwd_workspace_bytes(n_out, cout, cin, kvol, precision) if need_dx else 0
    ws = _workspace("conv", ws_bytes, dev) if ws_bytes else None
    wws = None
    if need_dw:
        dw = torch.empty_like(weight)
        wws = _workspace("wgrad", L.toda_spconv_wgrad_workspace_bytes(rb.n_in, n_out, kvol, cin, cout, precision), dev)
    sp = small.data_ptr()
    args = _C.LayerBwdArgs(
        da.data_ptr(), a_mask.data_ptr(), y.data_ptr(), n_out, cout, gamma.data_ptr(), _vp(mean), _vp(rstd), int(relu), int(training),
        dy.data_ptr(), _vp(dyb), _vp(dres), sp, sp + 4 * cout, bws.data_ptr(), bws.numel(),
        x.data_ptr(), _vp(xb), rb.n_in, cin, kvol,
        int(bool(need_dx)), _vp(nbr), _vp(wt), _vp(wtb), _vp(out_rows), _vp(masks),
        _vp(pl.lidx) if pl else None, _vp(pl.rows) if pl else None, _vp(pl.cnt) if pl else None, pl.ngroups if pl else 0,
        pl.cap if pl else 0, _vp(addend) if need_dx else None, _vp(dx),
        int(bool(need_dw)), rb.nbr_fwd.data_ptr(), _vp(dw), _vp(wws), wws.numel() if wws is not None else 0,
        int(bool(has_bias)), sp + 8 * cout, precision, _vp(ws), ws.numel() if ws is not None else 0)
    _C.check(L.toda_layer_bwd(ctypes.byref(args), _stream()), "toda_layer_bwd")
    _count(3 + (1 if need_dx else 0) + (2 if need_dw else 0) + (2 if has_bias else 0))
    return dx, dw, (small[2 * cout:] if has_bias else None), small[:cout], small[cout:2 * cout], dres


class _ConvBNAct(torch.autograd.Function):

    @staticmethod
    def forward(ctx, x, x_bf16, weight, bias, rb, precision, gamma, beta, running_mean, running_var, eps, momentum, training,
                residual, relu, want_bf16):
        need_grad = any(ctx.needs_input_grad)
        a, ab, saved = _layer_forward(x, x_bf16, weight, bias, rb, precision, gamma, beta, running_mean, running_var, eps, momentum,
                                      training, residual, relu, want_bf16, need_grad)
        if need_grad:
            ctx.save_for_backward(*saved)
        ctx.set_materialize_grads(False)
        ctx.rb, ctx.precision, ctx.has_bias = rb, precision, bias is not None
        ctx.cfg = (bool(training), bool(relu), residual is not None, bool(want_bf16))
        if ab is not None:
            ctx.mark_non_differentiable(ab)
        return a, ab

    @staticmethod
    def backward(ctx, da, _dab=None):
        if da is None:
            return (None,) * 16
        training, relu, has_res, want_bf16 = ctx.cfg
        dx, dw, db, dgamma, dbeta, dres = _layer_backward(da, ctx.saved_tensors, ctx.rb, ctx.precision, training, relu, has_res,
                                                          ctx.has_bias and ctx.needs_input_grad[3], ctx.needs_input_grad[0],
                                                          ctx.needs_input_grad[2])
        return dx, None, dw, db, None, None, dgamma, dbeta, None, None, None, None, None, dres, None, None


class _ResBlock(torch.autograd.Function):

    @staticmethod
    def forward(ctx, x, x_bf16, w1, b1, g1, be1, rm1, rv1, w2, b2, g2, be2, rm2, rv2, rb, precision, eps, momentum, training, want_bf16):
        need_grad = any(ctx.needs_input_grad)
        h, hb, s1 = _layer_forward(x, x_bf16, w1, b1, rb, precision, g1, be1, rm1, rv1, eps, momentum, training, None, True,
                                   want_bf16, need_grad)
        out, outb, s2 = _layer_forward(h, hb, w2, b2, rb, precision, g2, be2, rm2, rv2, eps, momentum, training, s1[0], True,
                                       want_bf16, need_grad)
        if need_grad:
            ctx.save_for_backward(*s1, *s2)
        ctx.set_materialize_grads(False)
        ctx.rb, ctx.precision, ctx.training = rb, precision, bool(training)
        ctx.has_bias = (b1 is not None, b2 is not None)
        if outb is not None:
            ctx.mark_non_differentiable(outb)
        return out, outb

    @staticmethod
    def backward(ctx, dout, _db=None):
        if dout is None:
            return (None,) * 20
        sv = ctx.saved_tensors
        s1, s2 = sv[:8], sv[8:]
        ng = ctx.needs_input_grad
        dh, dw2, db2, dg2, dbe2, dres = _layer_backward(dout, s2, ctx.rb, ctx.precision, ctx.training, True, True,
                                                        ctx.has_bias[1] and ng[9], True, ng[8])
        dx, dw1, db1, dg1, dbe1, _ = _layer_backward(dh, s1, ctx.rb, ctx.precision, ctx.training, True, False,
                                                     ctx.has_bias[0] and ng[3], ng[0], ng[2], addend=dres if ng[0] else None)
        return (dx, None, dw1, db1, dg1, dbe1, None, None, dw2, db2, dg2, dbe2, None, None, None, None, None, None, None, None)


def res_block(x, x_bf16, conv1_w, conv1_b, bn1, conv2_w, conv2_b, bn2, rb, precision, want_bf16=False):
    training = bn1.training or bn1.running_mean is None
    if training:
        for bn in (bn1, bn2):
            if bn.running_mean is not None and bn.num_batches_tracked is not None:
                bn.num_batches_tracked += 1
    assert bn1.eps == bn2.eps and bn1.momentum == bn2.momentum
    return _ResBlock.apply(x, x_bf16, conv1_w, conv1_b, bn1.weight, bn1.bias, bn1.running_mean, bn1.running_var, conv2_w, conv2_b,
                           bn2.weight, bn2.bias, bn2.running_mean, bn2.running_var, rb, precision, bn1.eps, bn1.momentum, training,
                           want_bf16)


def conv_bn_act(x, weight, bias, rb, precision, bn: torch.nn.BatchNorm1d, residual=None, relu=True, x_bf16=None, want_bf16=False):
    training = bn.training or bn.running_mean is None
    if training and bn.running_mean is not None and bn.num_batches_tracked is not None:
        bn.num_batches_tracked += 1
    return _ConvBNAct.apply(x, x_bf16, weight, bias, rb, precision, bn.weight, bn.bias, bn.running_mean, bn.running_var, bn.eps,
                            bn.momentum, training, residual, relu, want_bf16)


def bn_act(y, bn: torch.nn.BatchNorm1d, residual=None, relu=True, want_bf16=False, sums=None):
    training = bn.training or bn.running_mean is None
    if training and bn.running_mean is not None and bn.num_batches_tracked is not None:
        bn.num_batches_tracked += 1
    a, ab = _BNAct.apply(y, bn.weight, bn.bias, bn.running_mean, bn.running_var, bn.eps, bn.momentum, training, residual,
                         relu, want_bf16, sums if training else None)
    return (a, ab) if want_bf16 else a


class _BEVScatter(torch.autograd.Function):
    @staticmethod
    def forward(ctx, features, coords, batch, d, h, w):
        features = _need(features.contiguous(), torch.float32, "features")
        coords = _need(coords, torch.int32, "indices")
        n, c = features.shape
        out = torch.empty((batch, c * d, h, w), dtype=torch.float32, device=features.device)
        with _timed("bev_scatter_fwd", n=n, c=c, out_elems=out.numel()):
            _C.check(_C.lib().toda_bev_scatter_fwd(_p(features), _p(coords), n, c, batch, d, h, w, _p(out), _stream()),
                     "toda_bev_scatter_fwd")
        _count(2)
        ctx.save_for_backward(coords)
        ctx.dims = (n, c, batch, d, h, w)
        return out

    @staticmethod
    def backward(ctx, dout):
        (coords,) = ctx.saved_tensors
        n, c, batch, d, h, w = ctx.dims
        dout = dout.contiguous()
        df = torch.empty((n, c), dtype=torch.float32, device=dout.device)
        with _timed("bev_scatter_bwd", n=n, c=c):
            _C.check(_C.lib().toda_bev_scatter_bwd(_p(dout), _p(coords), n, c, batch, d, h, w, _p(df), _stream()),
                     "toda_bev_scatter_bwd")
        _count(1)
        return df, None, None, None, None, None


def bev_scatter(features, coords, batch, d, h, w):
    return _BEVScatter.apply(features, coords, batch, d, h, w)


class _GatherRows(torch.autograd.Function):
    @staticmethod
    def forward(ctx, x, rows, inverse_rows):
        x = _need(x.contiguous(), torch.float32, "features")
        n, c = rows.shape[0], x.shape[1]
        out = torch.empty((n, c), dtype=torch.float32, device=x.device)
        _C.check(_C.lib().toda_gather_rows(_p(x), _p(rows), n, c, _p(out), _stream()), "toda_gather_rows")
        _count(1)
        ctx.save_for_backward(inverse_rows)
        return out

    @staticmethod
    def backward(ctx, dout):
        (inv,) = ctx.saved_tensors
        dout = dout.contiguous()
        n, c = inv.shape[0], dout.shape[1]
        dx = torch.empty((n, c), dtype=torch.float32, device=dout.device)
        _C.check(_C.lib().toda_gather_rows(_p(dout), _p(inv), n, c, _p(dx), _stream()), "toda_gather_rows")
        _count(1)
        return dx, None, None


def permute_rows(x, rows, inverse_rows):
    return _GatherRows.apply(x, rows, inverse_rows)
```

Measured before the change: 398.3.

## Skip empty row-chunk/offset passes in tensor-core wgrad using tile masks

The tcgen05 weight-gradient kernel now reads per-tile neighbour occupancy masks and only schedules (row chunk, pass) items that have at least one live offset. Work is balanced across splits by counting live items with a block-wide prefix scan instead of splitting rows evenly. Table-slice loads also skip offsets that are absent from the mask. This removes MMA and gather work on empty tiles, which are common in sparse convolution. The cost is extra scheduling logic, a warp-ballot walk and more complex barrier signalling, with some risk of pipeline stalls or correctness bugs.

```diff
diff --git a/include/toda_b200.h b/include/toda_b200.h
--- a/include/toda_b200.h
+++ b/include/toda_b200.h
@@ -89,8 +89,10 @@
 int toda_weight_kmajor_bf16(const float *w, int kvol, int cin, int cout, void *w_bf16, void *stream);
 size_t toda_spconv_wgrad_workspace_bytes(int n_in, int n_out, int kvol, int cin, int cout, int precision);
 int toda_spconv_wgrad(const float *x, const void *x_bf16, int n_in, int cin, const int32_t *nbr, int n_out, int kvol,
-                      const float *dy, const void *dy_bf16, int cout, float *dw_param, void *workspace,
-                      size_t workspace_bytes, int precision, void *stream);
+                      const uint32_t *tile_masks, const float *dy, const void *dy_bf16, int cout, float *dw_param,
+                      void *workspace, size_t workspace_bytes, int precision, void *stream);
+int toda_wgrad_schedule(const uint32_t *masks, int n_out, int kvol, int cin, int cout, int split, int group,
+                        int32_t *geometry, int32_t *items, int cap);
 
 size_t toda_bn_workspace_bytes(int channels);
 int toda_bn_stats(const float *y, int n, int channels, const float *gamma, const float *beta, float eps,
@@ -133,7 +135,7 @@
     const int32_t *dgrad_out_rows ; const uint32_t *dgrad_masks ;
     const uint16_t *dplan_lidx ; const int32_t *dplan_rows; const int32_t *dplan_cnt; int dplan_groups, dplan_cap;
     const float *addend ; float *dx;
-    int need_dw; const int32_t *nbr_fwd; float *dw; void *wgrad_ws; size_t wgrad_ws_bytes;
+    int need_dw; const int32_t *nbr_fwd; const uint32_t *wgrad_masks ; float *dw; void *wgrad_ws; size_t wgrad_ws_bytes;
     int need_db; float *db;
     int precision; void *conv_ws; size_t conv_ws_bytes;
 } toda_layer_bwd_args;
diff --git a/toda_b200/_C.py b/toda_b200/_C.py
--- a/toda_b200/_C.py
+++ b/toda_b200/_C.py
@@ -47,7 +47,9 @@
     "toda_layer_fwd": (c_int, [c_vp, c_vp]),
     "toda_layer_bwd": (c_int, [c_vp, c_vp]),
     "toda_spconv_wgrad_workspace_bytes": (c_sz, [c_int] * 6),
-    "toda_spconv_wgrad": (c_int, [c_vp, c_vp, c_int, c_int, c_vp, c_int, c_int, c_vp, c_vp, c_int, c_vp, c_vp, c_sz, c_int, c_vp]),
+    "toda_spconv_wgrad": (c_int, [c_vp, c_vp, c_int, c_int, c_vp, c_int, c_int, c_vp, c_vp, c_vp, c_int, c_vp, c_vp, c_sz, c_int,
+                                  c_vp]),
+    "toda_wgrad_schedule": (c_int, [c_vp, c_int, c_int, c_int, c_int, c_int, c_int, c_vp, c_vp, c_int]),
     "toda_bn_workspace_bytes": (c_sz, [c_int]),
     "toda_bn_stats": (c_int, [c_vp, c_int, c_int, c_vp, c_vp, c_f32, c_f32, c_vp, c_vp, c_vp, c_vp, c_vp, c_vp, c_vp,
                               c_sz, c_vp]),
@@ -84,7 +86,7 @@
                 ("need_dx", c_int), ("dgrad_nbr", c_vp), ("wt", c_vp), ("wt_bf16", c_vp), ("dgrad_out_rows", c_vp), ("dgrad_masks", c_vp),
                 ("dplan_lidx", c_vp), ("dplan_rows", c_vp), ("dplan_cnt", c_vp), ("dplan_groups", c_int), ("dplan_cap", c_int),
                 ("addend", c_vp), ("dx", c_vp),
-                ("need_dw", c_int), ("nbr_fwd", c_vp), ("dw", c_vp), ("wgrad_ws", c_vp), ("wgrad_ws_bytes", c_sz),
+                ("need_dw", c_int), ("nbr_fwd", c_vp), ("wgrad_masks", c_vp), ("dw", c_vp), ("wgrad_ws", c_vp), ("wgrad_ws_bytes", c_sz),
                 ("need_db", c_int), ("db", c_vp),
                 ("precision", c_int), ("conv_ws", c_vp), ("conv_ws_bytes", c_sz)]
 
diff --git a/toda_b200/csrc/conv_simt.cu b/toda_b200/csrc/conv_simt.cu
--- a/toda_b200/csrc/conv_simt.cu
+++ b/toda_b200/csrc/conv_simt.cu
@@ -7,16 +7,16 @@
                 cudaStream_t st, const TilePlan *plan, const float *addend, const void *w_bf16);
 size_t conv_tc_fwd_workspace_bytes(int n_in, int cin, int cout, int kvol);
 int conv_tc_wgrad(const float *x, const void *x_bf16, int n_in, int cin, const int32_t *nbr, int n_out, int kvol,
-                  const float *dy, const void *dy_bf16, int cout, float *dw_param, void *workspace, size_t workspace_bytes,
-                  cudaStream_t st);
+                  const uint32_t *tile_masks, const float *dy, const void *dy_bf16, int cout, float *dw_param, void *workspace,
+                  size_t workspace_bytes, cudaStream_t st);
 bool conv_tc_supported(int cin, int cout, int kvol);
 size_t conv_x3_fwd_workspace_bytes(int n_in, int cin, int cout, int kvol);
 int conv_x3_fwd(const float *x, int n_in, int cin, const int32_t *nbr, int n_out, int kvol, const float *w, int cout, const float *bias,
                 float *y, const int32_t *out_rows, const uint32_t *tile_masks, double *bn_sums, void *workspace, size_t workspace_bytes,
                 cudaStream_t st, const TilePlan *plan, const float *addend);
 size_t conv_x3_wgrad_workspace_bytes(int n_in, int n_out, int kvol, int cin, int cout);
-int conv_x3_wgrad(const float *x, int n_in, int cin, const int32_t *nbr, int n_out, int kvol, const float *dy, int cout, float *dw_param,
-                  void *workspace, size_t workspace_bytes, cudaStream_t st);
+int conv_x3_wgrad(const float *x, int n_in, int cin, const int32_t *nbr, int n_out, int kvol, const uint32_t *tile_masks, const float *dy,
+                  int cout, float *dw_param, void *workspace, size_t workspace_bytes, cudaStream_t st);
 bool conv_tc_wgrad_supported(int cin, int cout, int kvol);
 size_t conv_tc_wgrad_workspace_bytes(int n_in, int n_out, int kvol, int cin, int cout);
 
@@ -328,7 +328,7 @@
 }
 
 extern "C" int toda_spconv_wgrad(const float *x, const void *x_bf16, int n_in, int cin, const int32_t *nbr, int n_out,
-                                 int kvol, const float *dy, const void *dy_bf16, int cout, float *dw_param, void *workspace,
+                                 int kvol, const uint32_t *tile_masks, const float *dy, const void *dy_bf16, int cout, float *dw_param, void *workspace,
                                  size_t workspace_bytes, int precision, void *stream) {
     TODA_CHECK_ARG(n_in >= 0 && n_out >= 0 && cin > 0 && cout > 0 && kvol > 0, "spconv_wgrad: bad sizes");
     TODA_CHECK_ARG(dw_param, "spconv_wgrad: null dw");
@@ -341,9 +341,9 @@
     TODA_CHECK_ARG(precision == TODA_CONV_FP32 || precision == TODA_CONV_BF16 || precision == TODA_CONV_BF16X3,
                    "spconv_wgrad: unknown precision %d", precision);
     if (precision == TODA_CONV_BF16X3 && conv_tc_wgrad_supported(cin, cout, kvol))
-        return conv_x3_wgrad(x, n_in, cin, nbr, n_out, kvol, dy, cout, dw_param, workspace, workspace_bytes, st);
+        return conv_x3_wgrad(x, n_in, cin, nbr, n_out, kvol, tile_masks, dy, cout, dw_param, workspace, workspace_bytes, st);
     if (precision == TODA_CONV_BF16 && conv_tc_wgrad_supported(cin, cout, kvol))
-        return conv_tc_wgrad(x, x_bf16, n_in, cin, nbr, n_out, kvol, dy, dy_bf16, cout, dw_param, workspace, workspace_bytes, st);
+        return conv_tc_wgrad(x, x_bf16, n_in, cin, nbr, n_out, kvol, tile_masks, dy, dy_bf16, cout, dw_param, workspace, workspace_bytes, st);
     int splits = wgrad_splits(n_out, kvol, cin, cout);
     size_t need = (size_t)splits * kvol * cin * cout * sizeof(float);
     if (workspace_bytes < need) {
diff --git a/toda_b200/csrc/conv_tc.cu b/toda_b200/csrc/conv_tc.cu
--- a/toda_b200/csrc/conv_tc.cu
+++ b/toda_b200/csrc/conv_tc.cu
@@ -558,8 +558,166 @@
     static constexpr int kStages = ROWS == 128 ? 4 : 8;
     static constexpr int kLag = ROWS == 128 ? 2 : 3;
     static constexpr int kSmem = kStages * kATile + kBBufs * kBTile + 2 * kIdx + 1024 + 256;
+    static_assert(kLag < kStages, "an A stage is reused only after its item has been signalled");
 };
 constexpr int kWgradThreads = kProdThreads + 32 + 128 + 32;
+
+__host__ __device__ inline int popc32(uint32_t v) {
+#ifdef __CUDA_ARCH__
+    return __popc(v);
+#else
+    return __builtin_popcount(v);
+#endif
+}
+
+struct WgradGeom {
+    const uint32_t *masks;
+    int rows, offs;
+    int pass0, npass;
+    int nchunks;
+    __host__ __device__ uint32_t offsets(int c) const {
+        if (!masks) return ~0u;
+#ifdef __CUDA_ARCH__
+        const uint32_t m = __ldg(masks + c / (128 / rows));
+#else
+        const uint32_t m = masks[c / (128 / rows)];
+#endif
+        return m >> (pass0 * offs);
+    }
+    __host__ __device__ uint32_t live_of(uint32_t m) const {
+        const uint32_t per_pass = (1u << offs) - 1u;
+        uint32_t l = 0;
+        for (int p = 0; p < npass; ++p)
+            if ((m >> (p * offs)) & per_pass) l |= 1u << p;
+        return l;
+    }
+    __host__ __device__ uint32_t live(int c) const { return live_of(offsets(c)); }
+};
+
+struct WgradRange { int c_begin, skip, count; };
+
+__host__ __device__ inline void wgrad_split_bounds(int total, int split, int splits, int &begin, int &end) {
+    begin = (int)((long long)split * total / splits);
+    end = (int)((long long)(split + 1) * total / splits);
+}
+
+__host__ __device__ inline uint32_t wgrad_take(uint32_t l, int &skip, int &left) {
+    for (; l && skip > 0; --skip) l &= l - 1;
+    uint32_t keep = 0;
+    for (; l && left > 0; --left) {
+        keep |= l & (0u - l);
+        l &= l - 1;
+    }
+    return keep;
+}
+
+struct WgradWalk {
+    WgradGeom geom;
+    int c, skip, left;
+    WgradWalk(const WgradGeom &g, const WgradRange &r) : geom(g), c(r.c_begin), skip(r.skip), left(r.count) {}
+    bool next(int &chunk, uint32_t &passes) {
+        while (left > 0) {
+            const uint32_t keep = wgrad_take(geom.live(c++), skip, left);
+            if (keep) {
+                chunk = c - 1;
+                passes = keep;
+                return true;
+            }
+        }
+        return false;
+    }
+};
+
+struct WgradWarpWalk {
+    WgradGeom geom;
+    int c, skip, left, base;
+    uint32_t pending = 0, win_m = 0, win_l = 0;
+    __device__ WgradWarpWalk(const WgradGeom &g, const WgradRange &r) : geom(g), c(r.c_begin), skip(r.skip), left(r.count), base(0) {}
+    __device__ bool next(int &chunk, uint32_t &passes, uint32_t &kbits) {
+        const int lane = threadIdx.x & 31;
+        while (left > 0) {
+            if (!pending) {
+                base = c;
+                c += 32;
+                const int cl = base + lane;
+                win_m = cl < geom.nchunks ? geom.offsets(cl) : 0u;
+                win_l = cl < geom.nchunks ? geom.live_of(win_m) : 0u;
+                pending = __ballot_sync(0xffffffffu, win_l != 0u);
+                continue;
+            }
+            const int j = __ffs(pending) - 1;
+            pending &= pending - 1;
+            const uint32_t keep = wgrad_take(__shfl_sync(0xffffffffu, win_l, j), skip, left);
+            kbits = __shfl_sync(0xffffffffu, win_m, j);
+            if (keep) {
+                chunk = base + j;
+                passes = keep;
+                return true;
+            }
+        }
+        return false;
+    }
+};
+
+WgradRange wgrad_host_range(const WgradGeom &geom, int split, int splits) {
+    int total = 0;
+    for (int c = 0; c < geom.nchunks; ++c) total += popc32(geom.live(c));
+    int begin, end;
+    wgrad_split_bounds(total, split, splits, begin, end);
+    WgradRange r{0, 0, end - begin};
+    for (int c = 0, run = 0; r.count > 0 && c < geom.nchunks; ++c) {
+        const int n = popc32(geom.live(c));
+        if (begin < run + n) {
+            r.c_begin = c;
+            r.skip = begin - run;
+            break;
+        }
+        run += n;
+    }
+    return r;
+}
+
+__device__ WgradRange wgrad_block_range(const WgradGeom &geom, int split, int splits, int *sched ) {
+    const int tid = threadIdx.x, lane = tid & 31, warp = tid >> 5, nwarps = blockDim.x >> 5;
+    const int per = (geom.nchunks + (int)blockDim.x - 1) / (int)blockDim.x;
+    const int c0 = min(tid * per, geom.nchunks), c1 = min(c0 + per, geom.nchunks);
+    int cnt = 0;
+#pragma unroll 4
+    for (int c = c0; c < c1; ++c) cnt += popc32(geom.live(c));
+    int inc = cnt;
+#pragma unroll
+    for (int o = 1; o < 32; o <<= 1) {
+        const int v = __shfl_up_sync(0xffffffffu, inc, o);
+        if (lane >= o) inc += v;
+    }
+    if (lane == 31) sched[warp] = inc;
+    __syncthreads();
+    int pre = inc - cnt, total = 0;
+    for (int w = 0; w < nwarps; ++w) {
+        const int v = sched[w];
+        total += v;
+        if (w < warp) pre += v;
+    }
+    int begin, end;
+    wgrad_split_bounds(total, split, splits, begin, end);
+    if (begin < end && pre <= begin && begin < pre + cnt) {
+        int c = c0, run = pre;
+        for (;; ++c) {
+            const int n = popc32(geom.live(c));
+            if (begin < run + n) break;
+            run += n;
+        }
+        sched[16] = c;
+        sched[17] = begin - run;
+    }
+    __syncthreads();
+    WgradRange r{0, 0, end - begin};
+    if (r.count > 0) {
+        r.c_begin = sched[16];
+        r.skip = sched[17];
+    }
+    return r;
+}
 
 __device__ __forceinline__ uint64_t make_desc_mn_sw128(uint32_t smem_addr, uint32_t lbo_bytes) {
     uint64_t d = 0;
@@ -575,14 +733,15 @@
 __global__ void __launch_bounds__(kWgradThreads, 1) conv_tc_wgrad_kernel(const __nv_bfloat16 *__restrict__ xb,
                                                                          const int *__restrict__ nbr, int n_out, int kvol,
                                                                          const __nv_bfloat16 *__restrict__ dyb, int cout,
-                                                                         int rows_per_split, int passes_per_cta,
-                                                                         float *__restrict__ partial) {
+                                                                         const uint32_t *__restrict__ tile_masks ,
+                                                                         int passes_per_cta, float *__restrict__ partial) {
     using W = WCfg<NPAD, ROWS>;
     constexpr int kOffsPerPass = 128 / CIN;
     constexpr int S = W::kStages;
     constexpr int kRowsW = ROWS, kATileW = W::kATile, kBTileW = W::kBTile, kIdxW = W::kIdx, kBBufsW = W::kBBufs;
     constexpr int kRowIters = ROWS / 32;
     extern __shared__ uint8_t smem_raw[];
+    __shared__ int sched[18];
     const uint32_t raw = smem_u32(smem_raw);
     const uint32_t base = (raw + 1023u) & ~1023u;
     const uint32_t b_base = base + S * kATileW;
@@ -601,9 +760,7 @@
     const int npass = min(passes_per_cta, total_passes - pass0);
     const int k0 = pass0 * kOffsPerPass;
     const int noffs = min(npass * kOffsPerPass, kvol - k0);
-    const int r_begin = split * rows_per_split;
-    const int r_end = min(n_out, r_begin + rows_per_split);
-    const int nchunks = r_end > r_begin ? (r_end - r_begin + kRowsW - 1) / kRowsW : 0;
+    const WgradGeom geom{tile_masks, kRowsW, kOffsPerPass, pass0, npass, (n_out + kRowsW - 1) / kRowsW};
 
     if (tid == 0) {
         for (int s = 0; s < S; ++s) {
@@ -627,34 +784,52 @@
         asm volatile("tcgen05.alloc.cta_group::1.sync.aligned.shared::cta.b32 [%0], %1;" ::"r"(tmem_slot), "r"(tmem_cols) : "memory");
         asm volatile("tcgen05.relinquish_alloc_permit.cta_group::1.sync.aligned;" ::: "memory");
     }
+    const WgradRange range = wgrad_block_range(geom, split, gridDim.x, sched);
     asm volatile("tcgen05.fence::before_thread_sync;" ::: "memory");
     __syncthreads();
     asm volatile("tcgen05.fence::after_thread_sync;" ::: "memory");
     const uint32_t tmem_base = *tmem_slot_ptr;
 
+    int chunk;
+    uint32_t passes;
     if (warp < 8) {
         const int p = tid & 7, rbase = tid >> 3;
         const uint32_t piece_off = (uint32_t)(rbase * 128 + ((p ^ (rbase & 7)) << 4));
         const int off_lo = CIN >= 64 ? 0 : p / (CIN / 8);
         const int ci_lo = CIN >= 64 ? p * 8 : (p % (CIN / 8)) * 8;
         constexpr int kLagW = W::kLag;
-        int g = 0, signalled = 0;
-        for (int rc = 0; rc < nchunks; ++rc) {
-            const int ib = rc & 1, use_i = rc >> 1;
-            const int bb = rc % kBBufsW, use_b = rc / kBBufsW;
-            const int row_base = r_begin + rc * kRowsW;
-            if (npass < kLagW) {
-                asm volatile("cp.async.wait_group 0;" ::: "memory");
-                asm volatile("fence.proxy.async.shared::cta;" ::: "memory");
-                __syncwarp();
-                if (lane == 0)
-                    for (; signalled < g; ++signalled) {
-                        if (signalled % npass == 0) mbar_arrive(b_full + 8 * ((signalled / npass) % kBBufsW));
-                        mbar_arrive(a_full + 8 * (signalled % S));
-                    }
-                signalled = g;
-            }
-            if (use_b > 0) mbar_wait(b_empty + 8 * bb, (use_b - 1) & 1);
+        int g = 0, signalled = 0, cc = 0, sig_chunks = 0;
+        uint32_t firsts = 0;
+        int end1 = 0, end2 = 0, end3 = 0;
+        auto signal_next = [&]() {
+            if (lane == 0) {
+                if (firsts & 1u) mbar_arrive(b_full + 8 * (sig_chunks % kBBufsW));
+                mbar_arrive(a_full + 8 * (signalled % S));
+            }
+            sig_chunks += firsts & 1u;
+            firsts >>= 1;
+            ++signalled;
+        };
+        auto drain = [&](int upto) {
+            const int in_flight = g - upto;
+            if (in_flight <= 0) asm volatile("cp.async.wait_group 0;" ::: "memory");
+            else if (in_flight == 1) asm volatile("cp.async.wait_group 1;" ::: "memory");
+            else asm volatile("cp.async.wait_group 2;" ::: "memory");
+            asm volatile("fence.proxy.async.shared::cta;" ::: "memory");
+            __syncwarp();
+            while (signalled < upto) signal_next();
+        };
+        WgradWarpWalk walk(geom, range);
+        uint32_t kbits;
+        while (walk.next(chunk, passes, kbits)) {
+            const int ib = cc & 1, use_i = cc >> 1;
+            const int bb = cc % kBBufsW, use_b = cc / kBBufsW;
+            const int row_base = chunk * kRowsW;
+            if (use_b > 0) {
+                const int need = kBBufsW == 2 ? end2 : end3;
+                if (signalled < need) drain(need);
+                mbar_wait(b_empty + 8 * bb, (use_b - 1) & 1);
+            }
             {
                 const uint32_t b_dst = b_base + bb * kBTileW + piece_off;
 #pragma unroll
@@ -664,14 +839,16 @@
                     for (int i = 0; i < kRowIters; ++i) {
                         const int row = row_base + rbase + 32 * i;
                         const uint32_t dst = b_dst + nb * (kRowsW * 128) + i * 4096;
-                        if (row < r_end && co < cout) cp_async_16(dst, dyb + (size_t)row * cout + co, 16u);
+                        if (row < n_out && co < cout) cp_async_16(dst, dyb + (size_t)row * cout + co, 16u);
                         else st_shared_zero16(dst);
                     }
                 }
             }
             mbar_wait(idx_full + 8 * ib, use_i & 1);
             const uint32_t idx_tile = idx_base + ib * kIdxW + 4 * rbase;
-            for (int ps = 0; ps < npass; ++ps, ++g) {
+            uint32_t first = 1u;
+            for (uint32_t pl = passes; pl; pl &= pl - 1, ++g) {
+                const int ps = __ffs(pl) - 1;
                 const int s = g % S, use = g / S;
                 if (use > 0) mbar_wait(a_empty + 8 * s, (use - 1) & 1);
                 const uint32_t a_dst = base + s * kATileW + piece_off;
@@ -679,12 +856,12 @@
                 for (int mb = 0; mb < 2; ++mb) {
                     const int koff = ps * kOffsPerPass + (CIN == 128 ? 0 : (CIN == 64 ? mb : mb * (kOffsPerPass / 2) + off_lo));
                     const int ci = CIN == 128 ? mb * 64 + ci_lo : ci_lo;
-                    const bool k_ok = koff < noffs;
+                    const bool k_live = koff < noffs && ((kbits >> koff) & 1u);
                     int src[kRowIters];
 #pragma unroll
                     for (int i = 0; i < kRowIters; ++i) {
                         src[i] = -1;
-                        if (k_ok) asm volatile("ld.shared.b32 %0, [%1];" : "=r"(src[i]) : "r"(idx_tile + 4 * (koff * kRowsW + 32 * i)));
+                        if (k_live) asm volatile("ld.shared.b32 %0, [%1];" : "=r"(src[i]) : "r"(idx_tile + 4 * (koff * kRowsW + 32 * i)));
                     }
 #pragma unroll
                     for (int i = 0; i < kRowIters; ++i) {
@@ -694,62 +871,64 @@
                     }
                 }
                 asm volatile("cp.async.commit_group;" ::: "memory");
+                firsts |= first << (g - signalled);
+                first = 0u;
                 if (g - signalled >= kLagW) {
                     asm volatile("cp.async.wait_group %0;" ::"n"(kLagW) : "memory");
                     asm volatile("fence.proxy.async.shared::cta;" ::: "memory");
                     __syncwarp();
-                    const int j = signalled;
-                    if (lane == 0) {
-                        if (j % npass == 0) mbar_arrive(b_full + 8 * ((j / npass) % kBBufsW));
-                        mbar_arrive(a_full + 8 * (j % S));
-                    }
-                    ++signalled;
+                    signal_next();
                 }
             }
             mbar_arrive(idx_empty + 8 * ib);
-        }
-        asm volatile("cp.async.wait_group 0;" ::: "memory");
-        asm volatile("fence.proxy.async.shared::cta;" ::: "memory");
-        __syncwarp();
-        if (lane == 0)
-            for (int j = signalled; j < g; ++j) {
-                if (j % npass == 0) mbar_arrive(b_full + 8 * ((j / npass) % kBBufsW));
-                mbar_arrive(a_full + 8 * (j % S));
-            }
+            end3 = end2;
+            end2 = end1;
+            end1 = g;
+            ++cc;
+        }
+        drain(g);
     } else if (warp == 8) {
-        if (nchunks > 0) {
-            constexpr uint32_t idesc = make_idesc_bf16(128, NPAD) | (1u << 15) | (1u << 16);
-            int g = 0;
-            uint32_t ready = 0;
-            for (int rc = 0; rc < nchunks; ++rc) {
-                const int ib = rc % kBBufsW;
-                mbar_wait(b_full + 8 * ib, (rc / kBBufsW) & 1);
-                const uint32_t b_tile = b_base + ib * kBTileW;
-                for (int ps = 0; ps < npass; ++ps, ++g) {
-                    const int s = g % S, use = g / S;
-                    if (!ready) mbar_wait(a_full + 8 * s, use & 1);
-                    ready = mbar_test(a_full + 8 * ((g + 1) % S), ((g + 1) / S) & 1);
-                    asm volatile("tcgen05.fence::after_thread_sync;" ::: "memory");
-                    const uint32_t a_tile = base + s * kATileW;
-                    if (elect_one()) {
-#pragma unroll
-                        const uint64_t ad0 = make_desc_mn_sw128(a_tile, kRowsW * 128), bd0 = make_desc_mn_sw128(b_tile, kRowsW * 128);
-                        umma_bf16(tmem_base + ps * NPAD, ad0, bd0, idesc, rc != 0);
-                        for (int j = 1; j < kRowsW / 16; ++j)
-                            umma_bf16(tmem_base + ps * NPAD, ad0 + 128 * j, bd0 + 128 * j, idesc, 1u);
-                        umma_commit(a_empty + 8 * s);
-                    }
-                    __syncwarp();
+        constexpr uint32_t idesc = make_idesc_bf16(128, NPAD) | (1u << 15) | (1u << 16);
+        int g = 0, cc = 0;
+        uint32_t ready = 0, touched = 0, kbits;
+        WgradWarpWalk walk(geom, range);
+        while (walk.next(chunk, passes, kbits)) {
+            const int bb = cc % kBBufsW;
+            mbar_wait(b_full + 8 * bb, (cc / kBBufsW) & 1);
+            const uint32_t b_tile = b_base + bb * kBTileW;
+            for (uint32_t pl = passes; pl; pl &= pl - 1, ++g) {
+                const int ps = __ffs(pl) - 1;
+                const int s = g % S, use = g / S;
+                if (!ready) mbar_wait(a_full + 8 * s, use & 1);
+                ready = mbar_test(a_full + 8 * ((g + 1) % S), ((g + 1) / S) & 1);
+                asm volatile("tcgen05.fence::after_thread_sync;" ::: "memory");
+                const uint32_t a_tile = base + s * kATileW;
+                const uint32_t accumulate = (touched >> ps) & 1u;
+                touched |= 1u << ps;
+                if (elect_one()) {
+                    const uint64_t ad0 = make_desc_mn_sw128(a_tile, kRowsW * 128), bd0 = make_desc_mn_sw128(b_tile, kRowsW * 128);
+                    umma_bf16(tmem_base + ps * NPAD, ad0, bd0, idesc, accumulate);
+#pragma unroll
+                    for (int j = 1; j < kRowsW / 16; ++j)
+                        umma_bf16(tmem_base + ps * NPAD, ad0 + 128 * j, bd0 + 128 * j, idesc, 1u);
+                    umma_commit(a_empty + 8 * s);
                 }
-                if (elect_one()) umma_commit(b_empty + 8 * ib);
                 __syncwarp();
             }
+            if (elect_one()) umma_commit(b_empty + 8 * bb);
+            __syncwarp();
+            ++cc;
+        }
+        if (touched) {
             if (elect_one()) umma_commit(accum_bar);
             __syncwarp();
         }
     } else if (warp < 13) {
         const int q = warp & 3;
-        if (nchunks > 0) {
+        uint32_t touched = 0, kbits;
+        WgradWarpWalk walk(geom, range);
+        while (walk.next(chunk, passes, kbits)) touched |= passes;
+        if (touched) {
             mbar_wait(accum_bar, 0);
             asm volatile("tcgen05.fence::after_thread_sync;" ::: "memory");
         }
@@ -758,9 +937,10 @@
             const int k = (pass0 + ps) * kOffsPerPass + m / CIN, ci = m % CIN;
             float *dst = partial + (((size_t)split * kvol + k) * CIN + ci) * cout;
             const uint32_t taddr = tmem_base + ((uint32_t)(q * 32) << 16) + ps * NPAD;
+            const bool has = (touched >> ps) & 1u;
             for (int n0 = 0; n0 < cout; n0 += 16) {
                 uint32_t v[16];
-                if (nchunks > 0) {
+                if (has) {
                     asm volatile(
                         "tcgen05.ld.sync.aligned.32x32b.x16.b32 {%0,%1,%2,%3,%4,%5,%6,%7,%8,%9,%10,%11,%12,%13,%14,%15}, [%16];"
                         : "=r"(v[0]), "=r"(v[1]), "=r"(v[2]), "=r"(v[3]), "=r"(v[4]), "=r"(v[5]), "=r"(v[6]), "=r"(v[7]),
@@ -781,14 +961,19 @@
         }
         asm volatile("tcgen05.fence::before_thread_sync;" ::: "memory");
     } else {
-        for (int rc = 0; rc < nchunks; ++rc) {
-            const int ib = rc & 1, use = rc >> 1;
+        int cc = 0;
+        WgradWarpWalk walk(geom, range);
+        uint32_t kbits;
+        while (walk.next(chunk, passes, kbits)) {
+            const int ib = cc & 1, use = cc >> 1;
             if (use > 0) mbar_wait(idx_empty + 8 * ib, (use - 1) & 1);
-            const uint32_t dst0 = idx_base + ib * kIdxW;
-            const int row_base = r_begin + rc * kRowsW;
-            load_table_slice<ROWS>(dst0, nbr + (size_t)k0 * n_out, n_out, row_base, r_end, noffs, lane);
+            uint32_t kmask = 0;
+            for (uint32_t pl = passes; pl; pl &= pl - 1) kmask |= ((1u << kOffsPerPass) - 1u) << ((__ffs(pl) - 1) * kOffsPerPass);
+            kmask &= kbits;
+            load_table_slice<ROWS>(idx_base + ib * kIdxW, nbr + (size_t)k0 * n_out, n_out, chunk * kRowsW, n_out, noffs, lane, kmask);
             cp_async_arrive_noinc(idx_full + 8 * ib);
             mbar_arrive(idx_full + 8 * ib);
+            ++cc;
         }
     }
     __syncthreads();
@@ -824,26 +1009,23 @@
 }
 
 struct WgradPlan {
-    int passes_per_cta, groups, splits, rows_per_split;
+    int passes_per_cta, groups, splits, rows;
     size_t xb_bytes, dyb_bytes, partial_bytes;
 };
 
 WgradPlan wgrad_plan(int n_in, int n_out, int kvol, int cin, int cout) {
     WgradPlan p;
     int npad = cout <= 64 ? 64 : 128;
-    const int kRowsW = npad == 64 ? 128 : 64;
+    p.rows = npad == 64 ? 128 : 64;
     int offs = 128 / cin;
     int total_passes = (kvol + offs - 1) / offs;
     p.passes_per_cta = total_passes < 512 / npad ? total_passes : 512 / npad;
     p.groups = (total_passes + p.passes_per_cta - 1) / p.passes_per_cta;
     int want = kNumSMs / p.groups;
     if (want < 1) want = 1;
-    int max_by_rows = (n_out + 4 * kRowsW - 1) / (4 * kRowsW);
+    int max_by_rows = (n_out + 4 * p.rows - 1) / (4 * p.rows);
     p.splits = want < max_by_rows ? want : max_by_rows;
     if (p.splits < 1) p.splits = 1;
-    int rps = (n_out + p.splits - 1) / p.splits;
-    p.rows_per_split = (rps + kRowsW - 1) / kRowsW * kRowsW;
-    if (p.rows_per_split < kRowsW) p.rows_per_split = kRowsW;
     p.xb_bytes = align_up((size_t)n_in * cin * 2 + 16, 256);
     p.dyb_bytes = align_up((size_t)n_out * cout * 2 + 16, 256);
     p.partial_bytes = align_up((size_t)p.splits * kvol * cin * cout * 4, 256);
@@ -862,8 +1044,8 @@
 }
 
 int conv_tc_wgrad(const float *x, const void *x_bf16, int n_in, int cin, const int32_t *nbr, int n_out, int kvol,
-                  const float *dy, const void *dy_bf16, int cout, float *dw_param, void *workspace, size_t workspace_bytes,
-                  cudaStream_t st) {
+                  const uint32_t *tile_masks, const float *dy, const void *dy_bf16, int cout, float *dw_param, void *workspace,
+                  size_t workspace_bytes, cudaStream_t st) {
     const int cin_real = cin;
     cin = pad16(cin);
     WgradPlan p = wgrad_plan(n_in, n_out, kvol, cin, cout);
@@ -903,7 +1085,7 @@
             TODA_CUDA_OK(cudaFuncSetAttribute(conv_tc_wgrad_kernel<CI, NP, RW>, cudaFuncAttributeMaxDynamicSharedMemorySize, smem)); \
             attr_set = true;                                                                                               \
         }                                                                                                                  \
-        conv_tc_wgrad_kernel<CI, NP, RW><<<grid, kWgradThreads, smem, st>>>(xb, nbr, n_out, kvol, dyb, cout, p.rows_per_split,  \
+        conv_tc_wgrad_kernel<CI, NP, RW><<<grid, kWgradThreads, smem, st>>>(xb, nbr, n_out, kvol, dyb, cout, tile_masks,      \
                                                                            p.passes_per_cta, partial);                      \
     } while (0)
     const bool wide = cout > 64;
@@ -921,3 +1103,26 @@
     TODA_LAUNCH_OK();
     return TODA_OK;
 }
+
+extern "C" int toda_wgrad_schedule(const uint32_t *masks, int n_out, int kvol, int cin, int cout, int split, int group,
+                                   int32_t *geometry, int32_t *items, int cap) {
+    TODA_CHECK_ARG(n_out >= 0 && conv_tc_wgrad_supported(cin, cout, kvol) && geometry && (items || cap == 0) && cap >= 0,
+                   "wgrad_schedule: bad args");
+    cin = pad16(cin);
+    const WgradPlan p = wgrad_plan(0, n_out, kvol, cin, cout);
+    geometry[0] = p.splits;
+    geometry[1] = p.groups;
+    geometry[2] = p.passes_per_cta;
+    geometry[3] = p.rows;
+    TODA_CHECK_ARG(split >= 0 && split < p.splits && group >= 0 && group < p.groups, "wgrad_schedule: no CTA (%d, %d)", split, group);
+    const int offs = 128 / cin, total_passes = (kvol + offs - 1) / offs, pass0 = group * p.passes_per_cta;
+    const int npass = total_passes - pass0 < p.passes_per_cta ? total_passes - pass0 : p.passes_per_cta;
+    const WgradGeom geom{masks, p.rows, offs, pass0, npass, (n_out + p.rows - 1) / p.rows};
+    WgradWalk walk(geom, wgrad_host_range(geom, split, p.splits));
+    int n = 0, chunk;
+    uint32_t passes;
+    while (walk.next(chunk, passes))
+        for (; passes; passes &= passes - 1, ++n)
+            if (n < cap) items[n] = chunk * 8 + __builtin_ctz(passes);
+    return n;
+}
diff --git a/toda_b200/csrc/conv_x3.cu b/toda_b200/csrc/conv_x3.cu
--- a/toda_b200/csrc/conv_x3.cu
+++ b/toda_b200/csrc/conv_x3.cu
@@ -9,8 +9,8 @@
                 cudaStream_t st, const TilePlan *plan, const float *addend, const void *w_bf16);
 size_t conv_tc_fwd_workspace_bytes(int n_in, int cin, int cout, int kvol);
 int conv_tc_wgrad(const float *x, const void *x_bf16, int n_in, int cin, const int32_t *nbr, int n_out, int kvol,
-                  const float *dy, const void *dy_bf16, int cout, float *dw_param, void *workspace, size_t workspace_bytes,
-                  cudaStream_t st);
+                  const uint32_t *tile_masks, const float *dy, const void *dy_bf16, int cout, float *dw_param, void *workspace,
+                  size_t workspace_bytes, cudaStream_t st);
 size_t conv_tc_wgrad_workspace_bytes(int n_in, int n_out, int kvol, int cin, int cout);
 
 namespace {
@@ -120,8 +120,8 @@
     return 2 * l.x_bytes + 2 * l.dy_bytes + 3 * l.t_bytes + l.inner + 256;
 }
 
-int conv_x3_wgrad(const float *x, int n_in, int cin, const int32_t *nbr, int n_out, int kvol, const float *dy, int cout, float *dw_param,
-                  void *workspace, size_t workspace_bytes, cudaStream_t st) {
+int conv_x3_wgrad(const float *x, int n_in, int cin, const int32_t *nbr, int n_out, int kvol, const uint32_t *tile_masks, const float *dy,
+                  int cout, float *dw_param, void *workspace, size_t workspace_bytes, cudaStream_t st) {
     const size_t need = conv_x3_wgrad_workspace_bytes(n_in, n_out, kvol, cin, cout);
     if (!workspace || workspace_bytes < need) {
         toda_set_error("spconv_wgrad(bf16x3): workspace %zu < required %zu bytes", workspace_bytes, need);
@@ -138,11 +138,11 @@
     TODA_LAUNCH_OK();
     split_rows_kernel<<<wave_grid((int64_t)n_out * cout, 256), 256, 0, st>>>(dy, n_out, cout, cout, dh, dl);
     TODA_LAUNCH_OK();
-    int rc = conv_tc_wgrad(x, xh, n_in, cp, nbr, n_out, kvol, dy, dh, cout, t1, inner, l.inner, st);
+    int rc = conv_tc_wgrad(x, xh, n_in, cp, nbr, n_out, kvol, tile_masks, dy, dh, cout, t1, inner, l.inner, st);
     if (rc) return rc;
-    rc = conv_tc_wgrad(x, xh, n_in, cp, nbr, n_out, kvol, dy, dl, cout, t2, inner, l.inner, st);
+    rc = conv_tc_wgrad(x, xh, n_in, cp, nbr, n_out, kvol, tile_masks, dy, dl, cout, t2, inner, l.inner, st);
     if (rc) return rc;
-    rc = conv_tc_wgrad(x, xl, n_in, cp, nbr, n_out, kvol, dy, dh, cout, t3, inner, l.inner, st);
+    rc = conv_tc_wgrad(x, xl, n_in, cp, nbr, n_out, kvol, tile_masks, dy, dh, cout, t3, inner, l.inner, st);
     if (rc) return rc;
     const size_t rows = (size_t)cout * kvol;
     sum3_unpad_kernel<<<wave_grid((int64_t)rows * cin, 256), 256, 0, st>>>(t1, t2, t3, rows, cp, cin, dw_param);
diff --git a/toda_b200/csrc/layer.cu b/toda_b200/csrc/layer.cu
--- a/toda_b200/csrc/layer.cu
+++ b/toda_b200/csrc/layer.cu
@@ -52,8 +52,8 @@
         if (rc) return rc;
     }
     if (p->need_dw) {
-        rc = toda_spconv_wgrad(p->x, p->x_bf16, p->n_in, p->cin, p->nbr_fwd, n, p->kvol, p->dy, p->dy_bf16, c, p->dw, p->wgrad_ws,
-                               p->wgrad_ws_bytes, p->precision, stream);
+        rc = toda_spconv_wgrad(p->x, p->x_bf16, p->n_in, p->cin, p->nbr_fwd, n, p->kvol, p->wgrad_masks, p->dy, p->dy_bf16, c, p->dw,
+                               p->wgrad_ws, p->wgrad_ws_bytes, p->precision, stream);
         if (rc) return rc;
     }
     if (p->need_db) {
diff --git a/toda_b200/csrc/table_slice.cuh b/toda_b200/csrc/table_slice.cuh
--- a/toda_b200/csrc/table_slice.cuh
+++ b/toda_b200/csrc/table_slice.cuh
@@ -3,18 +3,20 @@
 
 template <int ROWS>
 __device__ __forceinline__ void load_table_slice(uint32_t dst0, const int *__restrict__ nbr_k0, int n_out, int row_base, int r_end,
-                                                 int noffs, int lane) {
+                                                 int noffs, int lane, uint32_t kmask = ~0u) {
     const int *src = nbr_k0 + row_base + lane;
     uint32_t dst = dst0 + 4u * lane;
     if (row_base + ROWS <= r_end) {
 #pragma unroll 3
         for (int k = 0; k < noffs; ++k, src += n_out, dst += 4u * ROWS) {
+            if (!((kmask >> k) & 1u)) continue;
 #pragma unroll
             for (int j = 0; j < ROWS / 32; ++j)
                 asm volatile("cp.async.ca.shared.global [%0], [%1], 4;" ::"r"(dst + 128u * j), "l"(src + 32 * j) : "memory");
         }
     } else {
         for (int k = 0; k < noffs; ++k, src += n_out, dst += 4u * ROWS) {
+            if (!((kmask >> k) & 1u)) continue;
 #pragma unroll
             for (int j = 0; j < ROWS / 32; ++j) {
                 if (row_base + lane + 32 * j < r_end)
diff --git a/toda_b200/ops.py b/toda_b200/ops.py
--- a/toda_b200/ops.py
+++ b/toda_b200/ops.py
@@ -581,8 +581,9 @@
         ws = _workspace("wgrad", ws_bytes, dy.device)
         with _timed("conv_wgrad", n_in=rb.n_in, n_out=rb.n_out, cin=cin, cout=cout, kvol=rb.kvol, precision=precision,
                     rb=id(rb)):
-            _C.check(L.toda_spconv_wgrad(_p(x), _p(xb), rb.n_in, cin, _p(rb.nbr_fwd), rb.n_out, rb.kvol, _p(dy), _p(dyb),
-                                         cout, _p(dw), _p(ws), ws.numel(), precision, _stream()), "toda_spconv_wgrad")
+            _C.check(L.toda_spconv_wgrad(_p(x), _p(xb), rb.n_in, cin, _p(rb.nbr_fwd), rb.n_out, rb.kvol, _p(rb.tile_masks),
+                                         _p(dy), _p(dyb), cout, _p(dw), _p(ws), ws.numel(), precision, _stream()),
+                     "toda_spconv_wgrad")
         _count(2)
     if need_db:
         db = col_sum(dy)
@@ -846,7 +847,7 @@
         int(bool(need_dx)), _vp(nbr), _vp(wt), _vp(wtb), _vp(out_rows), _vp(masks),
         _vp(pl.lidx) if pl else None, _vp(pl.rows) if pl else None, _vp(pl.cnt) if pl else None, pl.ngroups if pl else 0,
         pl.cap if pl else 0, _vp(addend) if need_dx else None, _vp(dx),
-        int(bool(need_dw)), rb.nbr_fwd.data_ptr(), _vp(dw), _vp(wws), wws.numel() if wws is not None else 0,
+        int(bool(need_dw)), rb.nbr_fwd.data_ptr(), _vp(rb.tile_masks), _vp(dw), _vp(wws), wws.numel() if wws is not None else 0,
         int(bool(has_bias)), sp + 8 * cout, precision, _vp(ws), ws.numel() if ws is not None else 0)
     _C.check(L.toda_layer_bwd(ctypes.byref(args), _stream()), "toda_layer_bwd")
     _count(3 + (1 if need_dx else 0) + (2 if need_dw else 0) + (2 if has_bias else 0))
```

After: 403.2 (median of 6 runs). 1.01x the previous value.
